# sdecoder/AVX-sort-merge-joins

Measured on AMD Instinct MI355X. Metric: join throughput Mtuples/s (R⋈S) + achieved HBM GB/s, 128M⋈128M at 1/2/4/8 GPU, higher is better.
Workload: dtype int64; 1 GPU; sortmergejoin_multiway R=128000000 S=128000000 per GPU, 16-byte tuples, uniform, PK/FK keys 1..|R|, row-id payloads (48-bit intermediates); tuples_per_relation_per_gpu=128000000, tuples_per_relation_total=128000000, tuple_bytes=16, payload=rowid, distribution=uniform, parallelism=range-partition x1

## Files before the change

### avx-sort-merge-joins_amd/csrc/capi.hip

```cpp
#include <atomic>
#include <math.h>
#include <string.h>
#include <sys/time.h>

#include <algorithm>
#include <vector>

#include "../../include/smj.h"
#include "smj_common.hpp"
#include "smj_internal.hpp"

__global__ void k_setplan(smj::RangePlan* p, smj::RangePlan v) { *p = v; }

__global__ void __launch_bounds__(256)
k_join_begin(smj::RangePlan* p, smj::RangePlan v, int set_plan, unsigned long long* count,
             unsigned int* status, unsigned int* zero, uint32_t nzero) {
    if (threadIdx.x == 0) {
        if (set_plan) *p = v;
        *count = 0;
    }
    if (threadIdx.x < 4) status[threadIdx.x] = 0;
    for (uint32_t i = threadIdx.x; i < nzero; i += 256) zero[i] = 0;
}

// ... 1357 lines not shown
        (unsigned long long*)c.ws.scratch("api_cnt", sizeof(unsigned long long));
    const uint32_t T = joincfg->NTHREADS > 0 ? (uint32_t)joincfg->NTHREADS : 1;
    const uint32_t fan = joincfg->PARTFANOUT > 1 ? (uint32_t)joincfg->PARTFANOUT : 2;
    const uint32_t D = ceil_log2(fan);
    const uint32_t F = (1u << D) >= T ? (1u << D) : T;
    const uint32_t bits = ceil_log2(F);
    int64_t* hist = (int64_t*)c.ws.scratch("mp_hist", (size_t)T * F * 8);
    int64_t* off = (int64_t*)c.ws.scratch("mp_off", (size_t)T * F * 8);
    const DevBuf* rels[2] = {&r, &s};
    Tup* sorted[2] = {sR, sS};
    const uint64_t ns[2] = {nR, nS};
    static const char* pn[2] = {"mp_partR", "mp_partS"};
    std::vector<uint64_t> toff[2], tlen[2];
    for (int q = 0; q < 2; q++) {
        toff[q].assign(T, 0);
        tlen[q].assign(T, 0);
        if (ns[q] == 0) continue;
        Tup* part = (Tup*)c.ws.scratch(pn[q], ns[q] * sizeof(Tup));
        const uint64_t chunk = ns[q] / T;
        std::vector<uint64_t> c0(T), cl(T);
        for (uint32_t t = 0; t < T; t++) {
            c0[t] = t * chunk;
            cl[t] = t + 1 == T ? ns[q] - c0[t] : chunk;
            if (!cl[t]) continue;
            const uint64_t rchunk = t + 1 == T ? nR - (uint64_t)t * (nR / T) : nR / T;
            const int64_t sh = rchunk ? (int64_t)ceil(log2((double)(rchunk * T))) - (int64_t)bits - 1
                                      : 0;
            const uint32_t shift = sh > 0 ? (uint32_t)(sh < 63 ? sh : 63) : 0u;
            const uint32_t mask =
                shift < 32 ? (uint32_t)((((1ull << bits) - 1) << shift) & 0xffffffffull) : 0u;
            const Digit32 dig{mask, shift};
            stable_partition(&c.ws, rels[q]->d + c0[t], cl[t], part + c0[t], dig, bits, 0,
                             hist + (size_t)t * F, off + (size_t)t * F, c.st);
        }
        std::vector<int64_t> hh((size_t)T * F, 0), ho((size_t)T * F, 0);
        for (uint32_t t = 0; t < T; t++) {
            if (!cl[t]) continue;
            SMJ_CHECK(hipMemcpyAsync(hh.data() + (size_t)t * F, hist + (size_t)t * F, F * 8,
                                     hipMemcpyDeviceToHost, c.st));
            SMJ_CHECK(hipMemcpyAsync(ho.data() + (size_t)t * F, off + (size_t)t * F, F * 8,
                                     hipMemcpyDeviceToHost, c.st));
        }
        sync();
        std::vector<uint64_t> so((size_t)T * F), sl((size_t)T * F);
        for (uint32_t t = 0; t < T; t++)
            for (uint32_t j = 0; j < F; j++) {
                so[(size_t)t * F + j] = c0[t] + (uint64_t)ho[(size_t)t * F + j];
                sl[(size_t)t * F + j] = (uint64_t)hh[(size_t)t * F + j];
            }
        segmented_sort(&c.ws, part, so.data(), sl.data(), T * F, c.st);
        const uint32_t per = F / T;
        uint64_t o = 0;
        for (uint32_t t = 0; t < T; t++) {
            std::vector<const Tup*> runs;
            std::vector<uint64_t> lens;
            for (uint32_t j = t * per; j < (t + 1) * per; j++)
                for (uint32_t i = 0; i < T; i++) {
                    runs.push_back(part + so[(size_t)i * F + j]);
                    lens.push_back(sl[(size_t)i * F + j]);
                }
            uint64_t tot = 0;
            for (uint64_t x : lens) tot += x;
            toff[q][t] = o;
            tlen[q][t] = tot;
            if (tot) multiway_merge_tree(&c.ws, runs.data(), lens.data(), (uint32_t)runs.size(),
                                         sorted[q] + o, c.st);
            o += tot;
        }
    }
    unsigned long long* tcnt =
        (unsigned long long*)c.ws.scratch("mp_cnt", (size_t)T * sizeof(unsigned long long));
    SMJ_CHECK(hipMemsetAsync(tcnt, 0, (size_t)T * 8, c.st));
    for (uint32_t t = 0; t < T; t++)
        merge_join_count(sR + toff[0][t], tlen[0][t], sS + toff[1][t], tlen[1][t], tcnt + t,
                         c.st);
    std::vector<unsigned long long> h(T, 0);
    SMJ_CHECK(hipMemcpyAsync(h.data(), tcnt, (size_t)T * 8, hipMemcpyDeviceToHost, c.st));
    sync();
    (void)cnt;
    gettimeofday(&t1, NULL);
    result_t* res = (result_t*)malloc(sizeof(result_t));
    res->totalresults = 0;
    res->nthreads = joincfg->NTHREADS;
    res->resultlist = (threadresult_t*)calloc(T, sizeof(threadresult_t));
    for (uint32_t t = 0; t < T; t++) {
        res->totalresults += (int64_t)h[t];
        res->resultlist[t].nresults = (int64_t)h[t];
        res->resultlist[t].threadid = t;
        if (mat < 0 ? materialize_on() : mat > 0) {
            chainedtuplebuffer_t* cb = chainedtuplebuffer_init();
            materialize_append(sR + toff[0][t], tlen[0][t], sS + toff[1][t], tlen[1][t], cb);
            res->resultlist[t].results = cb;
        }
    }
    if (!getenv("SMJ_QUIET")) {
        double us = (t1.tv_sec - t0.tv_sec) * 1e6 + (t1.tv_usec - t0.tv_usec);
        fprintf(stderr, "NUM-TUPLES = %lld TOTAL-TIME-USECS = %.4lf ", (long long)nS, us);
        fprintf(stderr, "TUPLES-PER-SECOND = %.4lf ", nS / (us / 1e6));
        fflush(stderr);
    }
    return res;
}

result_t* sortmergejoin_multipass(relation_t* relR, relation_t* relS,
                                  joinconfig_t* joincfg) {
    return multipass_api(relR, relS, joincfg, -1);
}

result_t* smj_join(relation_t* relR, relation_t* relS, joinconfig_t* joincfg, int algo,
                   int materialize) {
    const int mat = materialize < 0 ? -1 : (materialize ? 1 : 0);
    switch (algo) {
        case 0: return join_api(relR, relS, joincfg, "m-way", mat);
        case 1: return multipass_api(relR, relS, joincfg, mat);
        case 2: return mpsm_api(relR, relS, joincfg, mat);
        default:
            fprintf(stderr, "[ERROR] smj_join: unknown algorithm %d\n", algo);
            return 0;
    }
}

int smj_tuple_bytes(void) { return (int)sizeof(Tup); }

const char* smj_device_name(void) {
    static char name[256] = {0};
    if (!name[0]) {
        Ctx& c = ctx();
        hipDeviceProp_t p;
        SMJ_CHECK(hipGetDeviceProperties(&p, c.device));
        snprintf(name, sizeof(name), "%s (%s)", p.name, p.gcnArchName);
    }
    return name;
}

smj_workspace* smj_workspace_create(void) {
    ctx();
    return (smj_workspace*)new Workspace();
}
void smj_workspace_destroy(smj_workspace* ws) { delete (Workspace*)ws; }

void smj_workspace_set_layouts(smj_workspace* ws, uint32_t off) {
    ((Workspace*)(ws ? ws : smj_context_workspace()))->layouts_off = off;
}

int smj_workspace_last_layout(smj_workspace* ws) {
    return ((Workspace*)(ws ? ws : smj_context_workspace()))->last_layout;
}

int smj_tilepass_occupancy(int layout, uint32_t d2_bits) {
    if (layout != SMJ_LAYOUT_USED_P48 && layout != SMJ_LAYOUT_USED_P32) return -1;
    return tilepass_occupancy(layout == SMJ_LAYOUT_USED_P32, d2_bits);
}

void smj_dev_partition(smj_workspace* ws, const tuple_t* in, uint64_t n,
                       tuple_t* out, uint32_t nbits, uint32_t shiftbits,
                       int padded, int64_t* hist_out, int64_t* off_out,
                       smj_stream_t stream) {
    const uint32_t mask = (uint32_t)(((1ull << nbits) - 1) << shiftbits);
    Digit32 dig{mask, shiftbits};
    stable_partition((Workspace*)ws, (const Tup*)in, n, (Tup*)out, dig, nbits,
                     padded, hist_out, off_out, (hipStream_t)stream);
}

void smj_dev_sort(smj_workspace* ws, const tuple_t* in, uint64_t n,
                  tuple_t* out, smj_stream_t stream) {
    device_sort((Workspace*)ws, (const Tup*)in, n, (Tup*)out,
                (hipStream_t)stream);
}

void smj_dev_merge2(const tuple_t* a, uint64_t na, const tuple_t* b,
                    uint64_t nb, tuple_t* out, smj_stream_t stream) {
    merge2(&ctx().ws, (const Tup*)a, na, (const Tup*)b, nb, (Tup*)out, (hipStream_t)stream);
}

void smj_dev_multiway_merge_host(smj_workspace* ws, const tuple_t* const* runs,
                                 const uint64_t* lens, uint32_t k,
                                 tuple_t* out, smj_stream_t stream) {
    multiway_merge((Workspace*)ws, (const Tup* const*)runs, lens, k, (Tup*)out,
                   (hipStream_t)stream);
}

void smj_dev_merge_join_count(const tuple_t* r, uint64_t nr, const tuple_t* s,
                              uint64_t ns, unsigned long long* count_dev,
                              smj_stream_t stream) {
    merge_join_count((const Tup*)r, nr, (const Tup*)s, ns, count_dev,
                     (hipStream_t)stream);
}

uint64_t smj_dev_materialize(smj_workspace* ws, const tuple_t* sortedR, uint64_t nR,
                             const tuple_t* sortedS, uint64_t nS, tuple_t* out,
                             uint64_t out_cap, smj_stream_t stream) {
    return materialize((Workspace*)ws, (const Tup*)sortedR, nR, (const Tup*)sortedS,
                       nS, (Tup*)out, out_cap, (hipStream_t)stream);
}

uint64_t smj_dev_join_pairs(smj_workspace* ws, const tuple_t* sortedR, uint64_t nR,
                            const tuple_t* sortedS, uint64_t nS, value_t* r_payload_out,
                            value_t* s_payload_out, intkey_t* key_out, uint64_t out_cap,
                            smj_stream_t stream) {
    return join_pairs((Workspace*)ws, (const Tup*)sortedR, nR, (const Tup*)sortedS, nS,
                      r_payload_out, s_payload_out, key_out, out_cap, (hipStream_t)stream);
}

uint64_t smj_dev_semi_join(smj_workspace* ws, const tuple_t* sortedR, uint64_t nR,
                           const tuple_t* sortedS, uint64_t nS, tuple_t* out,
                           uint64_t out_cap, int anti, smj_stream_t stream) {
    return semi_join((Workspace*)ws, (const Tup*)sortedR, nR, (const Tup*)sortedS, nS,
                     (Tup*)out, out_cap, anti, (hipStream_t)stream);
}

uint64_t smj_dev_band_join(smj_workspace* ws, const tuple_t* sortedR, uint64_t nR,
                           const tuple_t* sortedS, uint64_t nS, int64_t lo, int64_t hi,
                           value_t* r_payload_out, value_t* s_payload_out,
                           intkey_t* r_key_out, intkey_t* s_key_out, uint64_t out_cap,
                           smj_stream_t stream) {
    return band_join((Workspace*)ws, (const Tup*)sortedR, nR, (const Tup*)sortedS, nS, lo, hi,
                     r_payload_out, s_payload_out, r_key_out, s_key_out, out_cap,
                     (hipStream_t)stream);
}

void smj_dev_band_join_count(smj_workspace* ws, const tuple_t* sortedR, uint64_t nR,
                             const tuple_t* sortedS, uint64_t nS, int64_t lo, int64_t hi,
                             unsigned long long* count_dev, smj_stream_t stream) {
    band_join_count((Workspace*)ws, (const Tup*)sortedR, nR, (const Tup*)sortedS, nS, lo, hi,
                    count_dev, (hipStream_t)stream);
}

void smj_dev_join(smj_workspace* ws, const tuple_t* R, uint64_t nR,
                  const tuple_t* S, uint64_t nS, tuple_t* sortedR,
                  tuple_t* sortedS, uint32_t fanout_bits, int64_t key_min,
                  int64_t key_max, unsigned long long* count_dev,
                  smj_stream_t stream) {
    device_join((Workspace*)ws, (const Tup*)R, nR, (const Tup*)S, nS,
                (Tup*)sortedR, (Tup*)sortedS, fanout_bits, key_min, key_max,
                count_dev, (hipStream_t)stream);
}

__global__ void __launch_bounds__(256)
k_seg_tables(const int64_t* __restrict__ cnt, uint32_t nseg, uint32_t nb,
             uint64_t* __restrict__ seg_start, int64_t* __restrict__ seg_cnt,
             int64_t* __restrict__ bcount, uint64_t* __restrict__ bstart) {
    __shared__ uint32_t scr[5];
    __shared__ unsigned long long base;
    if (threadIdx.x == 0) base = 0;
    for (uint32_t b = threadIdx.x; b < nb; b += 256) {
        bcount[b] = 0;
        bstart[b] = 0;
    }
    __syncthreads();
    for (uint32_t s = 0; s < nseg; s++) {
        for (uint32_t b0 = 0; b0 < nb; b0 += 256) {
            const uint32_t b = b0 + threadIdx.x;
            const int64_t c = b < nb ? cnt[(size_t)s * nb + b] : 0;
            uint32_t tot;
            const uint32_t ex = block_exclusive_scan((uint32_t)c, scr, &tot);
            if (b < nb) {
                seg_start[(size_t)b * nseg + s] = base + ex;
                seg_cnt[(size_t)b * nseg + s] = c;
                bcount[b] += c;
            }
            __syncthreads();
            if (threadIdx.x == 0) base += tot;
            __syncthreads();
        }
    }
}

__global__ void __launch_bounds__(256)
k_seg_totals(const int64_t* __restrict__ cnt0, const int64_t* __restrict__ cnt1,
             uint32_t nseg, uint32_t nb, int64_t* __restrict__ bcount0,
             int64_t* __restrict__ bcount1, uint64_t* __restrict__ bstart0,
             uint64_t* __restrict__ bstart1) {
    const int64_t* cnt = blockIdx.x ? cnt1 : cnt0;
    int64_t* bcount = blockIdx.x ? bcount1 : bcount0;
    uint64_t* bstart = blockIdx.x ? bstart1 : bstart0;
    for (uint32_t b = threadIdx.x; b < nb; b += 256) {
        int64_t t = 0;
        for (uint32_t j = 0; j < nseg; j++) t += cnt[(size_t)b * nseg + j];
        bcount[b] = t;
        bstart[b] = 0;
    }
}

static void join_segmented_core(Workspace* ws, void* R, uint64_t nR, void* S, uint64_t nS,
                                uint64_t* const* ss, int64_t* const* sc, uint32_t nseg,
                                uint32_t bucket_bits, int64_t key_lo, int64_t key_hi,
                                uint32_t flags, tuple_t* sortedR, tuple_t* sortedS,
                                unsigned long long* count_dev, hipStream_t st,
                                const uint64_t* pstride = nullptr) {
    if (!(flags & SMJ_SEG_STAGE_R))
        SMJ_CHECK(hipMemsetAsync(count_dev, 0, sizeof(unsigned long long), st));
    uint32_t D1, D2, D2cap;
    choose_levels(nR > nS ? nR : nS, bucket_bits, &D1, &D2, &D2cap);
    const uint32_t tot_bits = D1 + D2;
    D1 = bucket_bits;
    D2 = tot_bits > D1 ? tot_bits - D1 : 0;
    if (D2 > kMaxD2) D2 = kMaxD2;
    D2cap = D2 + 2 < kMaxD2 ? D2 + 2 : (D2 > kMaxD2 ? D2 : kMaxD2);
    RangePlan hplan = make_plan(key_lo, key_hi, D1, D2, D2cap, kGroupD3Max);
    const bool p48 = pstride != nullptr;
    const bool packed = (flags & SMJ_SEG_PACKED) != 0 || p48;
    if (p48 && !LayP48::usable(hplan)) {
        fprintf(stderr, "[ERROR] smj_dev_join_segmented_planes: 48-bit words need "
                "1 <= s1 <= 32 (s1 = %u)\n", hplan.s1);
        abort();
    }
// ... 417 lines not shown
```

### avx-sort-merge-joins_amd/csrc/partition.hip

```cpp
#include <stdlib.h>
#include <string.h>

#include "smj_common.hpp"
#include "smj_internal.hpp"

namespace smj {

template <int THREADS, int ITEMS, class Digit>
__global__ void __launch_bounds__(THREADS)
k_hist(const Tup* __restrict__ in, uint64_t n, uint64_t chunk, Digit dig_arg,
       uint32_t nbins, uint32_t* __restrict__ counts, uint32_t nwg) {
    const auto dig = dig_arg.load();
    constexpr int TILE = THREADS * ITEMS;
    extern __shared__ __attribute__((aligned(16))) uint32_t lds_hist[];
    for (uint32_t d = threadIdx.x; d < nbins; d += THREADS) lds_hist[d] = 0;
    __syncthreads();
    const uint64_t beg = (uint64_t)blockIdx.x * chunk;
    uint64_t end = beg + chunk;
    if (end > n) end = n;
    for (uint64_t base = beg; base < end; base += TILE) {
        Tup v[ITEMS];
#pragma unroll
        for (int j = 0; j < ITEMS; j++) {
            const uint64_t i = base + (uint64_t)j * THREADS + threadIdx.x;
// ... 997 lines not shown
        if (sh_hist[d]) atomicAdd(&hist[d], sh_hist[d]);
}


#ifndef SMJ_SC_SEG
#define SMJ_SC_SEG 16
#endif
constexpr uint32_t kSegBytes = SMJ_SC_SEG;
constexpr uint32_t kRegionAlign = 128;
static_assert(kRegionAlign % kSegBytes == 0, "regions hold whole segments");

struct RegionRel {
    const unsigned int* sample[2];
    uint64_t* base[2];
    uint64_t* seg_start[2];
    unsigned long long* cursor[2];
    uint64_t* cap_end[2];
    int64_t* hist_out[2];
    int64_t* seg_cnt[2];
};

__global__ void __launch_bounds__(256)
k_regions(RegionRel R, uint32_t nbins, uint32_t stride, uint64_t slack, uint32_t elem_bytes) {
    const int r = blockIdx.x;
    const unsigned int* __restrict__ sample = R.sample[r];
    uint64_t* __restrict__ base = R.base[r];
    uint64_t* __restrict__ seg_start = R.seg_start[r];
    unsigned long long* __restrict__ cursor = R.cursor[r];
    uint64_t* __restrict__ cap_end = R.cap_end[r];
    __shared__ uint64_t sh[256];
    const uint64_t ALIGN = kRegionAlign / elem_bytes;
    const uint32_t per = (nbins + 255) / 256;
    const uint32_t b = threadIdx.x * per;
    auto cap = [&](uint32_t d) {
        const uint64_t est = (uint64_t)sample[d] * stride / kShards;
        return (est + est / 8 + slack + ALIGN - 1) / ALIGN * ALIGN;
    };
    uint64_t loc = 0;
    for (uint32_t k = 0; k < per; k++)
        if (b + k < nbins) loc += kShards * cap(b + k);
    sh[threadIdx.x] = loc;
    __syncthreads();
    if (threadIdx.x == 0) {
        uint64_t run = 0;
        for (int t = 0; t < 256; t++) {
            const uint64_t x = sh[t];
            sh[t] = run;
            run += x;
        }
    }
    __syncthreads();
    uint64_t ex = sh[threadIdx.x];
    for (uint32_t k = 0; k < per; k++) {
        const uint32_t d = b + k;
        if (d < nbins) {
            base[d] = ex;
            const uint64_t c = cap(d);
            for (uint32_t q = 0; q < kShards; q++) {
                seg_start[d * kShards + q] = ex;
                cursor[d * kShards + q] = ex;
                ex += c;
                cap_end[d * kShards + q] = ex;
            }
        }
    }
}

__global__ void __launch_bounds__(256)
k_regions_done(RegionRel R, uint32_t nbins, unsigned int* __restrict__ flag) {
    const int r = blockIdx.x;
    const uint64_t* __restrict__ seg_start = R.seg_start[r];
    const unsigned long long* __restrict__ cursor = R.cursor[r];
    const uint64_t* __restrict__ cap_end = R.cap_end[r];
    for (uint32_t d = threadIdx.x; d < nbins; d += 256) {
        int64_t tot = 0;
        for (uint32_t q = 0; q < kShards; q++) {
            const uint32_t i = d * kShards + q;
            const uint64_t e = cursor[i] < cap_end[i] ? cursor[i] : cap_end[i];
            const int64_t c = (int64_t)(e - seg_start[i]);
            R.seg_cnt[r][i] = c;
            tot += c;
            if (cursor[i] > cap_end[i]) atomicOr(flag, 1u);
        }
        R.hist_out[r][d] = tot;
    }
}

template <int THREADS, int ITEMS, class Digit>
__global__ void __launch_bounds__(THREADS)
k_shard_hist(const Tup* __restrict__ in, uint64_t n, uint64_t chunk, uint32_t split,
             Digit dig_arg, uint32_t nbins, unsigned int* __restrict__ counts) {
    const auto dig = dig_arg.load();
    extern __shared__ unsigned int lh[];
    for (uint32_t d = threadIdx.x; d < nbins; d += THREADS) lh[d] = 0;
    __syncthreads();
    const uint32_t c = blockIdx.x / split, s = blockIdx.x % split;
    const uint64_t sub = (chunk + split - 1) / split;
    const uint64_t beg = (uint64_t)c * chunk + (uint64_t)s * sub;
    const uint64_t end = min(min(beg + sub, (uint64_t)(c + 1) * chunk), n);
    constexpr int TILE = THREADS * ITEMS;
    for (uint64_t base = beg; base < end; base += TILE) {
        Tup v[ITEMS];
#pragma unroll
        for (int j = 0; j < ITEMS; j++) {
            const uint64_t i = base + (uint64_t)j * THREADS + threadIdx.x;
            v[j] = ld_stream(in + (i < end ? i : end - 1));
        }
#pragma unroll
        for (int j = 0; j < ITEMS; j++)
            if (base + (uint64_t)j * THREADS + threadIdx.x < end) atomicAdd(&lh[dig(v[j])], 1u);
    }
    __syncthreads();
    const uint32_t q = c % kShards;
    for (uint32_t d = threadIdx.x; d < nbins; d += THREADS)
        if (lh[d]) atomicAdd(&counts[(size_t)d * kShards + q], lh[d]);
}

__global__ void __launch_bounds__(1024)
k_regions_exact(RegionRel R, uint32_t nbins) {
    const int r = blockIdx.x;
    const unsigned int* __restrict__ cnt = R.sample[r];
    __shared__ uint32_t scr[1024 / 64 + 1];
    const uint32_t per = (nbins + 1023) / 1024;
    const uint32_t b = threadIdx.x * per;
    uint32_t loc = 0;
    for (uint32_t k = 0; k < per; k++)
        if (b + k < nbins)
            for (uint32_t q = 0; q < kShards; q++) loc += cnt[(size_t)(b + k) * kShards + q];
    uint32_t tot;
    uint64_t e = block_exclusive_scan(loc, scr, &tot);
    for (uint32_t k = 0; k < per; k++) {
        const uint32_t d = b + k;
        if (d >= nbins) break;
        R.base[r][d] = e;
        for (uint32_t q = 0; q < kShards; q++) {
            const size_t i = (size_t)d * kShards + q;
            R.seg_start[r][i] = e;
            R.cursor[r][i] = e;
            e += cnt[i];
            R.cap_end[r][i] = e;
        }
    }
}

template <int THREADS, int ITEMS, class OutT, uint32_t SB = sizeof(OutT)>
struct ScatterGeom {
    static constexpr uint32_t SEG = kSegBytes >= SB ? kSegBytes / SB : 1;
    static constexpr uint32_t TILE = THREADS * ITEMS;
    static __host__ __device__ constexpr uint32_t max_segs(uint32_t nbins) {
        return (TILE + nbins * (SEG - 1)) / SEG;
    }
    static __host__ __device__ constexpr size_t lds_bytes(uint32_t nbins) {
        return (size_t)TILE * sizeof(OutT) + (size_t)nbins * SEG * sizeof(OutT) +
               (size_t)nbins * (8 + 4 * 4) + ((size_t)max_segs(nbins) * 2 + 15) / 16 * 16 +
               (THREADS / 64 + 1) * 4;
    }
};

template <class P, class = void>
struct requires_quads : std::false_type {};
template <class P>
struct requires_quads<P, std::void_t<decltype(P::kQuads)>> : std::true_type {};
template <class Pack>
constexpr bool pack_quads() {
    if constexpr (requires_quads<Pack>::value) return Pack::kQuads;
    else return false;
}

template <int THREADS, int ITEMS, class Digit, class Pack, bool VEC>
__global__ void __launch_bounds__(THREADS)
k_scatter_res(const Tup* __restrict__ in, uint64_t n, uint64_t chunk, Digit dig_arg,
              uint32_t nbins, unsigned long long* __restrict__ cursor_all,
              const uint64_t* __restrict__ cap_end_all,
              void* __restrict__ out, uint64_t ostride, Pack pk,
              unsigned int* __restrict__ bad_flag) {
    typedef typename Pack::OutT OutT;
    typedef ScatterGeom<THREADS, ITEMS, OutT, Pack::kStoreBytes> Geo;
    constexpr uint32_t SEG = Geo::SEG;
    constexpr int TILE = (int)Geo::TILE;
    uint32_t bad = 0;
    const auto dig = dig_arg.load();
    const uint32_t shard = blockIdx.x % kShards;
    unsigned long long* cursor = cursor_all + shard;
    const uint64_t* cap_end = cap_end_all + shard;
    extern __shared__ __attribute__((aligned(16))) unsigned char lds_raw[];
    OutT* stage = reinterpret_cast<OutT*>(lds_raw);
    OutT* carry = stage + TILE;
    uint64_t* pos = reinterpret_cast<uint64_t*>(carry + (size_t)nbins * SEG);
    uint32_t* tstart = reinterpret_cast<uint32_t*>(pos + nbins);
    uint32_t* tfill = tstart + nbins;
    uint32_t* kc = tfill + nbins;
    uint32_t* segpre = kc + nbins;
    uint16_t* segown = reinterpret_cast<uint16_t*>(segpre + nbins);
    uint32_t* scr = reinterpret_cast<uint32_t*>(
        reinterpret_cast<unsigned char*>(segown) + ((size_t)Geo::max_segs(nbins) * 2 + 15) / 16 * 16);

    for (uint32_t d = threadIdx.x; d < nbins; d += THREADS) {
        tfill[d] = 0;
        kc[d] = 0;
    }
    const uint64_t beg = (uint64_t)blockIdx.x * chunk;
    uint64_t end = beg + chunk;
    if (end > n) end = n;
    const uint32_t d0 = threadIdx.x;
    const bool own = d0 < nbins;
    const uint64_t my_cap = own ? cap_end[(size_t)d0 * kShards] : 0;
    uint32_t my_kc = 0;

    static_assert(!VEC || (sizeof(Tup) == 8 && ITEMS % 2 == 0), "VEC: 8-byte tuples, ITEMS even");
    auto item_pos = [](int j) -> uint32_t {
        return VEC ? 2u * ((uint32_t)(j / 2) * THREADS + threadIdx.x) + (uint32_t)(j & 1)
                   : (uint32_t)j * THREADS + threadIdx.x;
    };
    auto load_tile = [&](Tup (&x)[ITEMS], uint64_t b0) {
#ifndef KEY_8B
        typedef unsigned long long V2 __attribute__((ext_vector_type(2)));
        if constexpr (VEC) {
            const V2* __restrict__ vin = reinterpret_cast<const V2*>(in);
            const uint64_t vl = end / 2 - 1;
#pragma unroll
            for (int p = 0; p < ITEMS / 2; p++) {
                const uint64_t vi = b0 / 2 + (uint64_t)p * THREADS + threadIdx.x;
#if SMJ_NT_LOADS
                const V2 y = __builtin_nontemporal_load(vin + (vi < vl ? vi : vl));
#else
                const V2 y = vin[vi < vl ? vi : vl];
#endif
                x[2 * p] = (Tup)y.x;
                x[2 * p + 1] = (Tup)y.y;
            }
        } else
#endif
        {
#pragma unroll
            for (int j = 0; j < ITEMS; j++) {
                const uint64_t i = b0 + (uint64_t)j * THREADS + threadIdx.x;
                x[j] = ld_stream(in + (i < end ? i : end - 1));
            }
        }
    };
    Tup v[ITEMS], nv[ITEMS];
    if (beg < end) load_tile(v, beg);
    __syncthreads();
    for (uint64_t base = beg; base < end; base += TILE) {
        const uint32_t tcount =
            (uint32_t)((end - base) < (uint64_t)TILE ? (end - base) : TILE);
        const uint64_t nb = base + TILE;
        __builtin_amdgcn_s_waitcnt(0x0f70);
        uint32_t dg[ITEMS];
#pragma unroll
        for (int j = 0; j < ITEMS; j++) {
            const uint32_t li = item_pos(j);
            dg[j] = li < tcount ? dig(v[j]) : 0xffffffffu;
            if (dg[j] != 0xffffffffu) atomicAdd(&tfill[dg[j]], 1u);
        }
        __syncthreads();
        const uint32_t c = own ? tfill[d0] : 0;
        const uint32_t T = my_kc + c;
        uint32_t Eown = T / SEG * SEG;
        uint32_t tot;
        const uint32_t ex = block_exclusive_scan(own ? (c | ((Eown / SEG) << 16)) : 0u, scr, &tot);
        const uint32_t nseg = tot >> 16;
        unsigned long long Pown = 0;
        if (own) {
            tstart[d0] = ex & 0xffffu;
            tfill[d0] = ex & 0xffffu;
            segpre[d0] = ex >> 16;
            for (uint32_t k = 0; k < Eown / SEG; k++) segown[(ex >> 16) + k] = (uint16_t)d0;
            if (Eown) Pown = atomicAdd(&cursor[(size_t)d0 * kShards], (unsigned long long)Eown);
        }
        load_tile(nv, nb);
        __syncthreads();
#pragma unroll
        for (int j = 0; j < ITEMS; j++)
            if (dg[j] != 0xffffffffu) stage[atomicAdd(&tfill[dg[j]], 1u)] = pk(v[j], bad);
        if (own) {
            const bool ovf = Eown && Pown + Eown > my_cap;
            pos[d0] = ovf ? ~0ull : Pown;
            if (ovf) Eown = 0;
        }
        __syncthreads();
        if constexpr (pack_quads<Pack>() && SEG == 4) {
            for (uint32_t sg = threadIdx.x; sg < nseg; sg += THREADS) {
                const uint32_t d = segown[sg];
                const uint32_t e = (sg - segpre[d]) * SEG;
                const uint32_t k = kc[d];
                const uint64_t p = pos[d];
                OutT x[4];
#pragma unroll
                for (uint32_t i = 0; i < 4; i++)
                    x[i] = e + i < k ? carry[d * SEG + e + i] : stage[tstart[d] + e + i - k];
                if (p != ~0ull) {
                    if ((p & 3) == 0) {
                        Pack::store4(out, ostride, p + e, x);
                    } else {
#pragma unroll
                        for (uint32_t i = 0; i < 4; i++) Pack::store(out, ostride, p + e + i, x[i]);
                    }
                }
            }
        } else if constexpr (Pack::kPairs) {
            constexpr uint32_t PS = SEG / 2;
            for (uint32_t q = threadIdx.x; q < nseg * PS; q += THREADS) {
                const uint32_t sg = q / PS;
                const uint32_t d = segown[sg];
                const uint32_t e = (sg - segpre[d]) * SEG + 2 * (q % PS);
                const uint32_t k = kc[d];
                const uint64_t p = pos[d];
                const OutT x0 = e < k ? carry[d * SEG + e] : stage[tstart[d] + e - k];
                const OutT x1 = e + 1 < k ? carry[d * SEG + e + 1] : stage[tstart[d] + e + 1 - k];
                if (p != ~0ull) {
                    if ((p & 1) == 0) {
                        Pack::store2(out, ostride, p + e, x0, x1);
                    } else {
                        Pack::store(out, ostride, p + e, x0);
                        Pack::store(out, ostride, p + e + 1, x1);
                    }
                }
            }
        } else {
            for (uint32_t q = threadIdx.x; q < nseg * SEG; q += THREADS) {
                const uint32_t sg = q / SEG;
                const uint32_t d = segown[sg];
                const uint32_t e = (sg - segpre[d]) * SEG + q % SEG;
                const uint32_t k = kc[d];
                const uint64_t p = pos[d];
                const OutT x = e < k ? carry[d * SEG + e] : stage[tstart[d] + e - k];
                if (p != ~0ull) Pack::store(out, ostride, p + e, x);
            }
        }
        __syncthreads();
        if (own) {
            uint32_t left = T - Eown;
            if (left > SEG - 1) left = SEG - 1;
            for (uint32_t e = Eown; e < Eown + left; e++)
                carry[d0 * SEG + (e - Eown)] =
                    e < my_kc ? carry[d0 * SEG + e] : stage[tstart[d0] + e - my_kc];
            my_kc = left;
            kc[d0] = left;
            tfill[d0] = 0;
        }
#pragma unroll
        for (int j = 0; j < ITEMS; j++) v[j] = nv[j];
        __syncthreads();
    }
    if (own) {
        const uint32_t d = d0;
        pos[d] = 0;
        if (kc[d]) {
            const uint64_t p = atomicAdd(&cursor[(size_t)d * kShards], (unsigned long long)kc[d]);
            pos[d] = p + kc[d] <= my_cap ? p : ~0ull;
        }
    }
    __syncthreads();
    for (uint32_t q = threadIdx.x; q < nbins * SEG; q += THREADS) {
        const uint32_t d = q / SEG, j = q % SEG;
        if (j < kc[d] && pos[d] != ~0ull) Pack::store(out, ostride, pos[d] + j, carry[q]);
    }
    if (bad_flag && bad) atomicOr(bad_flag, bad);
}

template <class Digit>
__global__ void k_padcopy(const Tup* __restrict__ in, uint64_t n, Digit dig_arg,
                          const uint64_t* __restrict__ ustart,
                          const uint64_t* __restrict__ pstart,
                          Tup* __restrict__ out) {
    const auto dig = dig_arg.load();
    uint64_t i = (uint64_t)blockIdx.x * blockDim.x + threadIdx.x;
    const uint64_t stride = (uint64_t)gridDim.x * blockDim.x;
    for (; i < n; i += stride) {
        Tup t = in[i];
        uint32_t d = dig(t);
        out[pstart[d] + (i - ustart[d])] = t;
    }
}

template <class Digit>
__global__ void k_hist_global(const Tup* __restrict__ in, uint64_t n, Digit dig_arg,
                              unsigned long long* __restrict__ hist) {
    const auto dig = dig_arg.load();
    uint64_t i = (uint64_t)blockIdx.x * blockDim.x + threadIdx.x;
    const uint64_t stride = (uint64_t)gridDim.x * blockDim.x;
    for (; i < n; i += stride) atomicAdd(&hist[dig(in[i])], 1ull);
}

struct LowBits {
    Digit32 inner;
    uint32_t lowbits;
    __device__ __forceinline__ LowBits load() const { return *this; }
    __device__ __forceinline__ uint32_t operator()(const Tup& t) const {
        return inner(t) & ((1u << lowbits) - 1u);
    }
};
struct HighBits {
    Digit32 inner;
    uint32_t lowbits;
    __device__ __forceinline__ HighBits load() const { return *this; }
    __device__ __forceinline__ uint32_t operator()(const Tup& t) const {
        return inner(t) >> lowbits;
    }
};

template <int THREADS, int ITEMS, bool STABLE, class Digit, class Pack = PackNone>
static void partition_hist_scatter(Workspace* ws, const Tup* in, uint64_t n,
                                   typename Pack::OutT* out, const Digit& dig, uint32_t dbits,
                                   int padded, uint64_t* starts_dev,
                                   int64_t* hist_out, int64_t* off_out,
                                   hipStream_t st, const Pack& pk = Pack(),
                                   unsigned int* bad_flag = nullptr) {
    constexpr int TILE = THREADS * ITEMS;
    const uint32_t nbins = 1u << dbits;
    uint64_t ntiles = (n + TILE - 1) / TILE;
    if (ntiles == 0) ntiles = 1;
    const uint32_t maxwg = 256 * 8;
    uint32_t nwg = (uint32_t)(ntiles < maxwg ? ntiles : maxwg);
    const uint64_t tiles_per_wg = (ntiles + nwg - 1) / nwg;
    const uint64_t chunk = tiles_per_wg * TILE;
    nwg = (uint32_t)((ntiles + tiles_per_wg - 1) / tiles_per_wg);

    uint32_t* counts = (uint32_t*)ws->scratch("pt_counts", (size_t)nbins * nwg * 4);
    uint64_t* totals = (uint64_t*)ws->scratch("pt_totals", (size_t)nbins * 8);
    {
        TraceScope ts(ws, "k_hist", st);
        hipLaunchKernelGGL((k_hist<THREADS, ITEMS, Digit>), dim3(nwg), dim3(THREADS),
                           nbins * sizeof(uint32_t), st, in, n, chunk, dig, nbins,
                           counts, nwg);
    }
    {
        TraceScope ts(ws, "k_scan", st);
        hipLaunchKernelGGL(k_scanrow, dim3(nbins), dim3(256), 0, st, counts, nwg,
                           totals);
        hipLaunchKernelGGL(k_scandig, dim3(1), dim3(256), 0, st, totals, nbins,
                           padded, starts_dev, hist_out, off_out);
    }
    if (n == 0) return;
    if constexpr (!STABLE) {
        const size_t ldsu = scatter_u_lds<THREADS, ITEMS>(nbins);
        set_lds_attr((const void*)k_scatter_u<THREADS, ITEMS, Digit, Pack>, 160 * 1024);
        if (ldsu > 160 * 1024) {
            fprintf(stderr, "[ERROR] smj: scatter LDS %zu > 160 KiB\n", ldsu);
            abort();
        }
        TraceScope ts(ws, "k_scatter", st);
        hipLaunchKernelGGL((k_scatter_u<THREADS, ITEMS, Digit, Pack>), dim3(nwg),
                           dim3(THREADS), ldsu, st, in, n, chunk, dig, nbins,
                           counts, nwg, starts_dev, out, pk, bad_flag);
        SMJ_CHECK(hipGetLastError());
        return;
    } else {
        typedef SwcGeom<512, 8> SG;
        if (nbins <= 4 * 512 && SG::lds_bytes(nbins) <= 160 * 1024) {
            set_lds_attr((const void*)k_scatter_swc<512, 8, Digit>, 160 * 1024);
            TraceScope ts(ws, "k_scatter", st);
            hipLaunchKernelGGL((k_scatter_swc<512, 8, Digit>), dim3(nwg), dim3(512),
                               SG::lds_bytes(nbins), st, in, n, chunk, dig, nbins, dbits,
                               counts, nwg, starts_dev, out);
            SMJ_CHECK(hipGetLastError());
            return;
        }
        const size_t lds = scatter_lds<THREADS, ITEMS>(nbins);
        set_lds_attr((const void*)k_scatter<THREADS, ITEMS, Digit>, 160 * 1024);
        if (lds > 160 * 1024) {
            fprintf(stderr, "[ERROR] smj: scatter LDS %zu > 160 KiB\n", lds);
            abort();
        }
        {
            TraceScope ts(ws, "k_scatter", st);
            hipLaunchKernelGGL((k_scatter<THREADS, ITEMS, Digit>), dim3(nwg),
                               dim3(THREADS), lds, st, in, n, chunk, dig, nbins, dbits,
                               counts, nwg, starts_dev, out);
        }
    }
    SMJ_CHECK(hipGetLastError());
}

static bool lds_order_ok(Workspace* ws, hipStream_t st) {
    static const bool ok = [&] {
        const uint64_t bad = lds_order_selfcheck(ws, st);
        if (bad)
            fprintf(stderr, "[WARN] smj: LDS atomics return %llu values out of lane order: "
                            "the stable partition uses ballot ranks\n",
                    (unsigned long long)bad);
        return bad == 0;
    }();
    return ok;
}

template <class Digit>
static void stable_partition_swp(Workspace* ws, const Tup* in, uint64_t n, Tup* out,
                                 const Digit& dig, uint32_t dbits, int padded,
                                 uint64_t* starts_dev, int64_t* hist_out, int64_t* off_out,
                                 hipStream_t st) {
    constexpr int THREADS = 512;
    constexpr int ITEMS = sizeof(Tup) == 16 ? 8 : 16;
    typedef SwaGeom<THREADS, ITEMS> G;
    const uint32_t nbins = 1u << dbits;
    uint64_t ntiles = (n + G::TILE - 1) / G::TILE;
    if (ntiles == 0) ntiles = 1;
    uint32_t nwg = (uint32_t)(ntiles < 256 ? ntiles : 256);
    const uint64_t tiles_per_wg = (ntiles + nwg - 1) / nwg;
    const uint64_t chunk = tiles_per_wg * G::TILE;
    nwg = (uint32_t)((ntiles + tiles_per_wg - 1) / tiles_per_wg);
    uint32_t* counts = (uint32_t*)ws->scratch("pt_counts", (size_t)nbins * nwg * 4);
    uint64_t* totals = (uint64_t*)ws->scratch("pt_totals", (size_t)nbins * 8);
    {
        TraceScope ts(ws, "k_hist", st);
        bool vec = false;
        if constexpr (sizeof(Tup) == 8) {
            vec = ((uintptr_t)in & 15) == 0 && (chunk & 1) == 0;
            if (vec)
                hipLaunchKernelGGL((k_hist_v<512, 8, Digit>), dim3(nwg), dim3(512),
                                   nbins * sizeof(uint32_t), st, in, n, chunk, dig, nbins,
                                   counts, nwg);
// ... 46 lines not shown
                               hipStream_t st) {
    if (dbits <= 10)
        partition_hist_scatter<512, 16, false>(ws, in, n, out, dig, dbits, 0, starts_dev,
                                               hist_out, nullptr, st);
    else
        partition_hist_scatter<256, 8, false>(ws, in, n, out, dig, dbits, 0, starts_dev,
                                              hist_out, nullptr, st);
}

void stable_partition(Workspace* ws, const Tup* in, uint64_t n, Tup* out,
                      const Digit32& dig, uint32_t dbits, int padded,
                      int64_t* hist_out, int64_t* off_out, hipStream_t st) {
    const uint32_t nbins = 1u << dbits;
    if (dbits <= kNarrowDigitBits) {
        uint64_t* starts = (uint64_t*)ws->scratch("pt_starts", (size_t)nbins * 8);
        stable_partition_narrow(ws, in, n, out, dig, dbits, padded, starts,
                                hist_out, off_out, st);
        return;
    }
    const uint32_t lowb = dbits / 2, highb = dbits - lowb;
    Tup* t1 = (Tup*)ws->scratch("pt_wide1", (n ? n : 1) * sizeof(Tup));
    Tup* t2 = (Tup*)ws->scratch("pt_wide2", (n ? n : 1) * sizeof(Tup));
    uint64_t* st1 = (uint64_t*)ws->scratch("pt_wst1", (1u << lowb) * 8);
    uint64_t* st2 = (uint64_t*)ws->scratch("pt_wst2", (1u << highb) * 8);
    LowBits lo{dig, lowb};
    HighBits hi{dig, lowb};
    stable_partition_narrow(ws, in, n, t1, lo, lowb, 0, st1, nullptr, nullptr, st);
    stable_partition_narrow(ws, t1, n, t2, hi, highb, 0, st2, nullptr, nullptr, st);
    unsigned long long* h = (unsigned long long*)ws->scratch("pt_whist", (size_t)nbins * 8);
    SMJ_CHECK(hipMemsetAsync(h, 0, (size_t)nbins * 8, st));
    if (n) hipLaunchKernelGGL(k_hist_global<Digit32>, dim3(1024), dim3(256), 0,
                              st, in, n, dig, h);
    uint64_t* ust = (uint64_t*)ws->scratch("pt_wust", (size_t)nbins * 8);
    uint64_t* pst = (uint64_t*)ws->scratch("pt_wpst", (size_t)nbins * 8);
    hipLaunchKernelGGL(k_scandig, dim3(1), dim3(256), 0, st,
                       (const uint64_t*)h, nbins, 0, ust, nullptr, nullptr);
    hipLaunchKernelGGL(k_scandig, dim3(1), dim3(256), 0, st,
                       (const uint64_t*)h, nbins, padded, pst, hist_out, off_out);
    if (n) hipLaunchKernelGGL(k_padcopy<Digit32>, dim3(2048), dim3(256), 0, st,
                              t2, n, dig, ust, pst, out);
    SMJ_CHECK(hipGetLastError());
}

void plan_partition(Workspace* ws, const Tup* in, uint64_t n, Tup* out,
                    const RangePlan* plan_dev, uint32_t dbits,
                    uint64_t* starts_dev, int64_t* hist_out, hipStream_t st) {
    PlanDigit1 dig{plan_dev};
    const uint32_t nbins = 1u << dbits;
    constexpr int THREADS = 512;
    constexpr int ITEMS = sizeof(Tup) == 16 ? 8 : 16;
    constexpr int TILE = THREADS * ITEMS;
    const size_t lds = scatter_wc_lds<THREADS, ITEMS>(nbins);
    if (sizeof(Tup) != 16 || dbits > 10 || lds > 160 * 1024) {
        unstable_partition(ws, in, n, out, dig, dbits, starts_dev, hist_out, st);
        return;
    }
    uint64_t ntiles = (n + TILE - 1) / TILE;
    if (ntiles == 0) ntiles = 1;
    const uint32_t maxwg = 256;
    uint32_t nwg = (uint32_t)(ntiles < maxwg ? ntiles : maxwg);
    const uint64_t tiles_per_wg = (ntiles + nwg - 1) / nwg;
    const uint64_t chunk = tiles_per_wg * TILE;
    nwg = (uint32_t)((ntiles + tiles_per_wg - 1) / tiles_per_wg);
    uint32_t* counts = (uint32_t*)ws->scratch("pt_counts", (size_t)nbins * nwg * 4);
    uint64_t* totals = (uint64_t*)ws->scratch("pt_totals", (size_t)nbins * 8);
    {
        TraceScope ts(ws, "k_hist", st);
        hipLaunchKernelGGL((k_hist<1024, 8, PlanDigit1>), dim3(nwg), dim3(1024),
                           nbins * sizeof(uint32_t), st, in, n, chunk, dig, nbins,
                           counts, nwg);
    }
    {
        TraceScope ts(ws, "k_scan", st);
        hipLaunchKernelGGL(k_scanrow, dim3(nbins), dim3(256), 0, st, counts, nwg,
                           totals);
        hipLaunchKernelGGL(k_scandig, dim3(1), dim3(256), 0, st, totals, nbins, 0,
                           starts_dev, hist_out, (int64_t*)nullptr);
    }
    if (n == 0) return;
    set_lds_attr((const void*)k_scatter_wc<THREADS, ITEMS, PlanDigit1>, 160 * 1024);
    TraceScope ts(ws, "k_scatter", st);
    hipLaunchKernelGGL((k_scatter_wc<THREADS, ITEMS, PlanDigit1>), dim3(nwg),
                       dim3(THREADS), lds, st, in, n, chunk, dig, nbins, counts,
                       nwg, starts_dev, out);
    SMJ_CHECK(hipGetLastError());
}

#ifdef KEY_8B
void plan_partition_packed(Workspace* ws, const Tup* in, uint64_t n, uint64_t* out,
                           const RangePlan* plan_dev, const RangePlan& pack_plan,
                           uint32_t dbits, uint64_t* starts_dev, int64_t* hist_out,
                           unsigned int* pack_bad, hipStream_t st) {
    PlanDigit1 dig{plan_dev};
    LayPacked::Pack pk;
    pk.bu = key_u(pack_plan.base);
    pk.span = pack_plan.span;
    pk.s1 = pack_plan.s1;
    if (dbits > 10)
        partition_hist_scatter<256, 8, false, PlanDigit1, LayPacked::Pack>(
            ws, in, n, out, dig, dbits, 0, starts_dev, hist_out, nullptr, st, pk, pack_bad);
    else
        partition_hist_scatter<512, 16, false, PlanDigit1, LayPacked::Pack>(
            ws, in, n, out, dig, dbits, 0, starts_dev, hist_out, nullptr, st, pk, pack_bad);
}
#endif

#ifndef SMJ_SC_THREADS
#define SMJ_SC_THREADS 1024
#endif
#ifndef SMJ_SC_ITEMS16
#define SMJ_SC_ITEMS16 4
#endif
#ifndef SMJ_SC_ITEMS16Q
#define SMJ_SC_ITEMS16Q 6
#endif
#ifndef SMJ_SC_ITEMS16P
#define SMJ_SC_ITEMS16P 8
#endif
#ifndef SMJ_SC_ITEMS8
#define SMJ_SC_ITEMS8 12
#endif
#ifndef SMJ_SC_ITEMS8W
#define SMJ_SC_ITEMS8W 16
#endif
#ifndef SMJ_SC_WG_PER_CU
#define SMJ_SC_WG_PER_CU 1
#endif
#ifndef SMJ_SAMPLE_STRIDE
#define SMJ_SAMPLE_STRIDE 128
#endif
static constexpr uint32_t kSampleStride = SMJ_SAMPLE_STRIDE;
#ifndef SMJ_SAMPLE_WG
#define SMJ_SAMPLE_WG 128
#endif
static constexpr uint32_t kSampleWg = SMJ_SAMPLE_WG;
static constexpr uint64_t kRegionSlack = 1024;

uint64_t sampled_capacity(uint64_t n, uint32_t dbits) {
    const uint64_t ALIGN = kRegionAlign / 4;
    return n + n / 8 + 5 * kSampleStride + 1 +
           ((uint64_t)1 << dbits) * kShards * (kRegionSlack + ALIGN);
}

static uint64_t scatter_chunk(uint64_t n, uint64_t tile, uint32_t* nwg_out) {
    const uint64_t ntiles = (n + tile - 1) / tile;
    const uint32_t maxwg = 256 * SMJ_SC_WG_PER_CU;
    uint32_t nwg = (uint32_t)(ntiles < maxwg ? ntiles : maxwg);
    const uint64_t tiles_per_wg = (ntiles + nwg - 1) / nwg;
    *nwg_out = (uint32_t)((ntiles + tiles_per_wg - 1) / tiles_per_wg);
    return tiles_per_wg * tile;
}

template <class Pack>
static int sampled_items(uint32_t nbins) {
    constexpr int THREADS = SMJ_SC_THREADS;
    constexpr int BIG = sizeof(Tup) == 16
        ? (sizeof(typename Pack::OutT) <= 8    ? SMJ_SC_ITEMS16P
           : sizeof(typename Pack::OutT) <= 12 ? SMJ_SC_ITEMS16Q
                                               : SMJ_SC_ITEMS16)
        : (sizeof(typename Pack::OutT) <= 4 ? SMJ_SC_ITEMS8W : SMJ_SC_ITEMS8);
    constexpr int SMALL = sizeof(Tup) == 16 ? 4 : 8;
    typedef typename Pack::OutT O;
    if (ScatterGeom<THREADS, BIG, O, Pack::kStoreBytes>::lds_bytes(nbins) <= 160 * 1024) return BIG;
    if (ScatterGeom<THREADS, SMALL, O, Pack::kStoreBytes>::lds_bytes(nbins) <= 160 * 1024)
        return SMALL;
    return 0;
}

template <int ITEMS, class Pack>
static bool sampled_scatter_t(Workspace* ws, const Tup* in, uint64_t n, void* out,
                              uint64_t ostride, const PlanDigit1& dig, uint32_t nbins,
                              unsigned long long* cursor, const uint64_t* cap_end,
                              const Pack& pk, unsigned int* bad_flag, hipStream_t st) {
    constexpr int THREADS = SMJ_SC_THREADS;
    constexpr int TILE = THREADS * ITEMS;
    const size_t lds = ScatterGeom<THREADS, ITEMS, typename Pack::OutT,
                                   Pack::kStoreBytes>::lds_bytes(nbins);
    if (lds > 160 * 1024) return false;
    uint32_t nwg = 0;
    const uint64_t chunk = scatter_chunk(n, TILE, &nwg);
    constexpr bool VEC_OK = sizeof(Tup) == 8 && ITEMS % 2 == 0;
    set_lds_attr((const void*)k_scatter_res<THREADS, ITEMS, PlanDigit1, Pack, false>, 160 * 1024);
    if constexpr (VEC_OK)
        set_lds_attr((const void*)k_scatter_res<THREADS, ITEMS, PlanDigit1, Pack, true>,
                     160 * 1024);
    TraceScope ts(ws, "k_scatter", st);
    bool vec = false;
    if constexpr (VEC_OK) {
        vec = n % 2 == 0 && chunk % 2 == 0 && ((uintptr_t)in & 15) == 0;
        if (vec)
            hipLaunchKernelGGL((k_scatter_res<THREADS, ITEMS, PlanDigit1, Pack, true>), dim3(nwg),
                               dim3(THREADS), lds, st, in, n, chunk, dig, nbins, cursor,
                               cap_end, out, ostride, pk, bad_flag);
    }
    if (!vec)
        hipLaunchKernelGGL((k_scatter_res<THREADS, ITEMS, PlanDigit1, Pack, false>), dim3(nwg),
                           dim3(THREADS), lds, st, in, n, chunk, dig, nbins, cursor,
                           cap_end, out, ostride, pk, bad_flag);
    return true;
}

template <class Pack>
static void sampled_scatter(Workspace* ws, const Tup* in, uint64_t n, void* out,
                            uint64_t ostride, const PlanDigit1& dig, uint32_t nbins,
                            unsigned long long* cursor, const uint64_t* cap_end,
                            const Pack& pk, unsigned int* bad_flag, hipStream_t st) {
    constexpr int THREADS = SMJ_SC_THREADS;
    if (nbins > (uint32_t)THREADS) {
        fprintf(stderr, "[ERROR] smj: sampled scatter needs <= %d partitions\n", THREADS);
        abort();
    }
    constexpr int BIG = sizeof(Tup) == 16
        ? (sizeof(typename Pack::OutT) <= 8    ? SMJ_SC_ITEMS16P
           : sizeof(typename Pack::OutT) <= 12 ? SMJ_SC_ITEMS16Q
                                               : SMJ_SC_ITEMS16)
        : (sizeof(typename Pack::OutT) <= 4 ? SMJ_SC_ITEMS8W : SMJ_SC_ITEMS8);
    constexpr int SMALL = sizeof(Tup) == 16 ? 4 : 8;
    const int items = sampled_items<Pack>(nbins);
    if (items == BIG && sampled_scatter_t<BIG>(ws, in, n, out, ostride, dig, nbins, cursor,
                                               cap_end, pk, bad_flag, st))
        return;
    if (items == SMALL && sampled_scatter_t<SMALL>(ws, in, n, out, ostride, dig, nbins,
                                                   cursor, cap_end, pk, bad_flag, st))
        return;
    fprintf(stderr, "[ERROR] smj: sampled scatter LDS exceeds 160 KiB (%u partitions)\n", nbins);
    abort();
}

void sampled_partition(Workspace* ws, int nrel, const Tup* const* in, const uint64_t* n,
                       void* const* out, const RangePlan* plan_dev, uint32_t dbits,
                       unsigned int* sample, uint64_t* const* starts_dev,
                       int64_t* const* hist_out, uint64_t* const* seg_start,
                       int64_t* const* seg_cnt, unsigned int* flag_dev, hipStream_t st,
                       const RangePlan* host_plan, bool packed, unsigned int* bad,
                       uint64_t p48_stride, bool p32, bool exact, bool p96) {
    PlanDigit1 dig{plan_dev};
    const uint32_t nbins = 1u << dbits;
    if (p96 && (sizeof(Tup) != 16 || !host_plan || !p48_stride || p32 || exact)) {
        fprintf(stderr, "[ERROR] smj: the 96-bit layout needs 16-byte tuples, the host plan "
                        "and a plane stride\n");
        abort();
    }
    if (exact && (p48_stride || p32)) {
        fprintf(stderr, "[ERROR] smj: exact shard regions take tuples or 64-bit words\n");
        abort();
    }
#ifndef KEY_8B
    packed = p48_stride != 0 || p32;
#endif
    if (p32 && (p48_stride || !packed)) {
        fprintf(stderr, "[ERROR] smj: the 32-bit layout is a packed one-plane layout\n");
        abort();
    }
    if (p48_stride && !packed) {
        fprintf(stderr, "[ERROR] smj: the 48-bit layout is a packed layout\n");
        abort();
    }
    if (packed && !host_plan) {
        fprintf(stderr, "[ERROR] smj: packed partition needs the host plan\n");
        abort();
    }
    static const char* cn[2] = {"sp_cursor0", "sp_cursor1"};
    static const char* en[2] = {"sp_capend0", "sp_capend1"};
    SampleRel S;
    RegionRel R;
    uint64_t nmax = 0;
    for (int r = 0; r < 2; r++) {
        const int rr = r < nrel ? r : 0;
        S.in[r] = in[rr];
        S.n[r] = n[rr];
        S.hist[r] = sample + (size_t)rr * nbins * (exact ? kShards : 1);
        R.sample[r] = S.hist[r];
        R.base[r] = starts_dev[rr];
        R.seg_start[r] = seg_start[rr];
        R.hist_out[r] = hist_out[rr];
        R.seg_cnt[r] = seg_cnt[rr];
        if (r < nrel) {
            R.cursor[r] = (unsigned long long*)ws->scratch(cn[r], (size_t)nbins * kShards * 8);
            R.cap_end[r] = (uint64_t*)ws->scratch(en[r], (size_t)nbins * kShards * 8);
            nmax = n[r] > nmax ? n[r] : nmax;
        } else {
            R.cursor[r] = R.cursor[0];
            R.cap_end[r] = R.cap_end[0];
        }
    }
    if (exact) {
        TraceScope ts(ws, "k_hist", st);
        for (int r = 0; r < nrel; r++) {
            if (!n[r]) continue;
            int items = 0;
#ifdef KEY_8B
            if (packed)
                items = sampled_items<LayPacked::Pack>(nbins);
            else
#endif
                items = sampled_items<PackRange>(nbins);
            if (!items) {
                fprintf(stderr, "[ERROR] smj: sampled scatter LDS exceeds 160 KiB (%u "
                        "partitions)\n", nbins);
                abort();
            }
            uint32_t nwg = 0;
            const uint64_t chunk = scatter_chunk(n[r], (uint64_t)SMJ_SC_THREADS * items, &nwg);
            constexpr int HI = sizeof(Tup) == 16 ? 8 : 16;
            const uint32_t split = 4;
            hipLaunchKernelGGL((k_shard_hist<1024, HI, PlanDigit1>), dim3(nwg * split),
                               dim3(1024), nbins * sizeof(unsigned int), st, in[r], n[r], chunk,
                               split, dig, nbins, S.hist[r]);
        }
        hipLaunchKernelGGL(k_regions_exact, dim3(nrel), dim3(1024), 0, st, R, nbins);
    } else {
        TraceScope ts(ws, "k_sample", st);
        const uint64_t npts = (nmax + 4 * kSampleStride - 1) / (4 * kSampleStride);
        uint32_t g = (uint32_t)((npts + 255) / 256);
        if (g > kSampleWg) g = kSampleWg;
        if (g == 0) g = 1;
        hipLaunchKernelGGL((k_sample_hist<PlanDigit1>), dim3(g, nrel), dim3(256),
                           nbins * sizeof(unsigned int), st, S, kSampleStride, dig, nbins);
        hipLaunchKernelGGL(k_regions, dim3(nrel), dim3(256), 0, st, R, nbins, kSampleStride,
                           kRegionSlack,
                           p96 ? (uint32_t)SMJ_P96_SEGB : p48_stride || p32 ? 4u : packed ? 8u
                                                                     : (uint32_t)sizeof(Tup));
    }
    for (int r = 0; r < nrel; r++) {
        if (!n[r]) continue;
        if (p32) {
            LayP32::Pack pk;
            pk.bu = key_u(host_plan->base);
            pk.span = host_plan->span;
            pk.s1 = host_plan->s1;
            sampled_scatter(ws, in[r], n[r], out[r], 0, dig, nbins, R.cursor[r], R.cap_end[r],
                            pk, bad, st);
            continue;
        }
#ifdef KEY_8B
        if (p96) {
            LayP96::Pack pk;
            pk.bu = key_u(host_plan->base);
            pk.span = host_plan->span;
            sampled_scatter(ws, in[r], n[r], out[r], p48_stride, dig, nbins, R.cursor[r],
                            R.cap_end[r], pk, bad, st);
            continue;
        }
#endif
        if (p48_stride) {
            LayP48::Pack pk;
            pk.bu = key_u(host_plan->base);
            pk.span = host_plan->span;
            pk.s1 = host_plan->s1;
            sampled_scatter(ws, in[r], n[r], out[r], p48_stride, dig, nbins, R.cursor[r],
                            R.cap_end[r], pk, bad, st);
            continue;
        }
#ifdef KEY_8B
        if (packed) {
            LayPacked::Pack pk;
            pk.bu = key_u(host_plan->base);
            pk.span = host_plan->span;
            pk.s1 = host_plan->s1;
            sampled_scatter(ws, in[r], n[r], out[r], 0, dig, nbins, R.cursor[r], R.cap_end[r],
                            pk, bad, st);
            continue;
        }
#endif
        PackRange pk{0ull, ~0ull};
        if (bad && host_plan) {
            pk.bu = key_u(host_plan->base);
            pk.span = host_plan->span;
        }
        sampled_scatter(ws, in[r], n[r], out[r], 0, dig, nbins, R.cursor[r], R.cap_end[r], pk,
                        bad && host_plan ? bad : (unsigned int*)nullptr, st);
    }
    hipLaunchKernelGGL(k_regions_done, dim3(nrel), dim3(256), 0, st, R, nbins, flag_dev);
    SMJ_CHECK(hipGetLastError());
}

__global__ void __launch_bounds__(1024)
k_lds_order(uint32_t K, uint32_t iters, unsigned long long* bad) {
    __shared__ uint32_t ctr[16][64];
// ... 63 lines not shown
```

### avx-sort-merge-joins_amd/csrc/smj_common.hpp

```cpp
#pragma once
#include <hip/hip_runtime.h>
#include <stdint.h>
#include <stdio.h>
#include <stdlib.h>

#define SMJ_CHECK(call)                                                        \
    do {                                                                       \
        hipError_t e_ = (call);                                                \
        if (e_ != hipSuccess) {                                                \
            fprintf(stderr, "[ERROR] smj: %s failed at %s:%d: %s\n", #call,    \
                    __FILE__, __LINE__, hipGetErrorString(e_));                \
            abort();                                                           \
        }                                                                      \
    } while (0)

#include <mutex>
#include <set>
#include <utility>

namespace smj {

inline void set_lds_attr(const void* kernel, int bytes) {
    static std::mutex mu;
    static std::set<std::pair<int, const void*>> done;
// ... 13 lines not shown
typedef uint64_t Tup;
#endif

constexpr int kTupBytes = sizeof(Tup);

#ifndef SMJ_NT_STORES
#define SMJ_NT_STORES 1
#endif
#ifndef SMJ_NT_LOADS
#define SMJ_NT_LOADS 0
#endif
#ifdef KEY_8B
typedef long long TupVec __attribute__((ext_vector_type(2)));
#endif
__device__ __forceinline__ void st_stream(Tup* p, const Tup& v) {
#if SMJ_NT_STORES
#ifdef KEY_8B
    TupVec x = {v.payload, v.key};
    __builtin_nontemporal_store(x, reinterpret_cast<TupVec*>(p));
#else
    __builtin_nontemporal_store(v, p);
#endif
#else
    *p = v;
#endif
}
__device__ __forceinline__ Tup ld_stream(const Tup* p) {
#if SMJ_NT_LOADS
#ifdef KEY_8B
    const TupVec x = __builtin_nontemporal_load(reinterpret_cast<const TupVec*>(p));
    Tup t;
    t.payload = x.x;
    t.key = x.y;
    return t;
#else
    return __builtin_nontemporal_load(p);
#endif
#else
    return *p;
#endif
}

__device__ __forceinline__ void st_w(uint64_t* p, uint64_t v) {
#if SMJ_NT_STORES
    __builtin_nontemporal_store(v, p);
#else
    *p = v;
#endif
}
#ifdef KEY_8B
__device__ __forceinline__ void st_w(Tup* p, const Tup& v) { st_stream(p, v); }
#endif

__device__ __forceinline__ Tup ld_nt(const Tup* p) {
#ifdef KEY_8B
    const TupVec x = __builtin_nontemporal_load(reinterpret_cast<const TupVec*>(p));
    Tup t;
    t.payload = x.x;
    t.key = x.y;
    return t;
#else
    return __builtin_nontemporal_load(p);
#endif
}

typedef const __attribute__((address_space(1))) uint64_t* GlobalU64Ptr;
__device__ __forceinline__ Tup ld_g(const Tup* p) {
#ifdef KEY_8B
    typedef const __attribute__((address_space(1))) TupVec* GV;
    const TupVec x = *(GV)p;
    Tup t;
    t.payload = x.x;
    t.key = x.y;
    return t;
#else
    return *(GlobalU64Ptr)p;
#endif
}

__device__ __forceinline__ void st_g(Tup* p, const Tup& v) {
#ifdef KEY_8B
    typedef __attribute__((address_space(1))) TupVec* GV;
    TupVec x = {v.payload, v.key};
    *(GV)p = x;
#else
    *(__attribute__((address_space(1))) uint64_t*)p = v;
#endif
}

__host__ __device__ __forceinline__ int64_t tup_key(const Tup& t) {
#ifdef KEY_8B
    return t.key;
#else
    return (int64_t)(int32_t)(uint32_t)(t >> 32);
#endif
}

__host__ __device__ __forceinline__ bool tup_less(const Tup& a, const Tup& b) {
#ifdef KEY_8B
    return (a.key < b.key) || (a.key == b.key && a.payload < b.payload);
#else
    return (int64_t)a < (int64_t)b;
#endif
}

__host__ __device__ __forceinline__ Tup tup_sel(bool c, const Tup& a, const Tup& b) {
#ifdef KEY_8B
    Tup r;
    r.payload = c ? a.payload : b.payload;
    r.key = c ? a.key : b.key;
    return r;
#else
    return c ? a : b;
#endif
}

__host__ __device__ __forceinline__ bool tup_eq(const Tup& a, const Tup& b) {
#ifdef KEY_8B
    return a.key == b.key && a.payload == b.payload;
#else
    return a == b;
#endif
}

__host__ __device__ __forceinline__ Tup tup_max_sentinel() {
#ifdef KEY_8B
    Tup t;
    t.payload = INT64_MAX;
    t.key = INT64_MAX;
    return t;
#else
    return (uint64_t)INT64_MAX;
#endif
}

__host__ __device__ __forceinline__ uint64_t key_u(int64_t k) {
    return (uint64_t)k ^ 0x8000000000000000ull;
}

struct RefDigit {
    uint32_t mask;
    uint32_t shift;
    __host__ __device__ __forceinline__ RefDigit load() const { return *this; }
    __device__ __forceinline__ uint32_t operator()(const Tup& t) const {
        uint64_t km1 = (uint64_t)(tup_key(t) - 1);
        return (uint32_t)((km1 & (uint64_t)mask) >> shift);
    }
};

constexpr uint32_t kBadPayload = 1;
constexpr uint32_t kBadRange = 2;
constexpr uint32_t kBadPayload48 = 4;
constexpr uint32_t kBadPayload32 = 8;

struct RangePlan {
    int64_t base;
    uint64_t span;
    uint32_t D1, D2, D3;
    uint32_t s1, s2, s3;
};

__host__ __device__ __forceinline__ uint64_t plan_rel(const RangePlan& p,
                                                      int64_t k) {
    uint64_t ku = key_u(k), bu = key_u(p.base);
    if (ku < bu) return 0;
    uint64_t r = ku - bu;
    return r > p.span ? p.span : r;
}

__host__ __device__ __forceinline__ uint32_t plan_d1(const RangePlan& p,
                                                     uint64_t rel) {
    uint64_t d = rel >> p.s1;
    uint64_t lim = (1ull << p.D1) - 1;
    return (uint32_t)(d > lim ? lim : d);
}

struct LayTup {
    typedef Tup W;
    static constexpr bool packed = false;
    typedef const W* CView;
    typedef W* View;
    __device__ static __forceinline__ CView cview(const void* b, uint64_t) {
        return static_cast<const W*>(b);
    }
    __device__ static __forceinline__ View view(void* b, uint64_t) { return static_cast<W*>(b); }
    __device__ static __forceinline__ uint64_t rel(const RangePlan& P, const W& w, uint32_t) {
        return plan_rel(P, tup_key(w));
    }
    __device__ static __forceinline__ bool clamped(const RangePlan& P, const W& w) {
        const uint64_t ku = key_u(tup_key(w)), bu = key_u(P.base);
        return ku < bu || ku - bu > P.span;
    }
    __device__ static __forceinline__ bool less(const W& a, const W& b) { return tup_less(a, b); }
    __device__ static __forceinline__ Tup unpack(const RangePlan&, const W& w, uint32_t) {
        return w;
    }
    __device__ static __forceinline__ uint32_t digit_fast(const W& w, uint32_t base_lo,
                                                          uint32_t, uint32_t sh, uint32_t mask) {
        return (((uint32_t)tup_key(w) - base_lo) >> sh) & mask;
    }
    __host__ static bool fast_ok(const RangePlan& P, uint32_t sh, uint32_t width) {
        return sh + width <= 32;
    }
    struct FastDigit {
        uint32_t base_lo, sh, mask;
        __device__ FastDigit(const RangePlan& P, uint32_t s, uint32_t width)
            : base_lo((uint32_t)P.base), sh(s), mask((1u << width) - 1) {}
        __device__ __forceinline__ uint32_t operator()(const W& w) const {
            return (((uint32_t)tup_key(w) - base_lo) >> sh) & mask;
        }
    };
    struct Unpack {
        __device__ Unpack(const RangePlan&, uint32_t) {}
        __device__ __forceinline__ Tup operator()(const W& w) const { return w; }
    };
    __device__ static __forceinline__ uint64_t same_key_id(const W& w) {
#ifdef KEY_8B
        return (uint64_t)w.payload;
#else
        return w;
#endif
    }
};

#ifdef KEY_8B
struct LayPacked {
    typedef uint64_t W;
    static constexpr bool packed = true;
    typedef const W* CView;
    typedef W* View;
    __device__ static __forceinline__ CView cview(const void* b, uint64_t) {
        return static_cast<const W*>(b);
    }
    __device__ static __forceinline__ View view(void* b, uint64_t) { return static_cast<W*>(b); }
    __device__ static __forceinline__ uint64_t rel(const RangePlan& P, const W& w, uint32_t b) {
        return ((uint64_t)b << P.s1) | (w >> (64 - P.s1));
    }
    __device__ static __forceinline__ bool clamped(const RangePlan&, const W&) { return false; }
    __device__ static __forceinline__ bool less(const W& a, const W& b) { return a < b; }
    __device__ static __forceinline__ uint64_t same_key_id(const W& w) { return w; }
    __device__ static __forceinline__ uint32_t digit_fast(const W& w, uint32_t, uint32_t s1,
                                                          uint32_t sh, uint32_t mask) {
        return (uint32_t)(w >> (64 - s1 + sh)) & mask;
    }
    __host__ static bool fast_ok(const RangePlan& P, uint32_t sh, uint32_t width) {
        return sh + width <= P.s1;
    }
    __device__ static __forceinline__ Tup unpack(const RangePlan& P, const W& w, uint32_t b) {
        Tup t;
        t.payload = (int64_t)(w & (~0ull >> P.s1));
        t.key = (int64_t)((key_u(P.base) + rel(P, w, b)) ^ 0x8000000000000000ull);
        return t;
    }
    struct FastDigit {
        uint32_t tsh, mask;
        __device__ FastDigit(const RangePlan& P, uint32_t s, uint32_t width)
            : tsh(64 - P.s1 + s), mask((1u << width) - 1) {}
        __device__ __forceinline__ uint32_t operator()(const W& w) const {
            return (uint32_t)(w >> tsh) & mask;
        }
    };
    struct Unpack {
        uint64_t kbu, pmask;
        uint32_t sh;
        __device__ Unpack(const RangePlan& P, uint32_t b)
            : kbu(key_u(P.base) + ((uint64_t)b << P.s1)), pmask(~0ull >> P.s1), sh(64 - P.s1) {}
        __device__ __forceinline__ Tup operator()(const W& w) const {
            Tup t;
            t.payload = (int64_t)(w & pmask);
            t.key = (int64_t)((kbu + (w >> sh)) ^ 0x8000000000000000ull);
            return t;
        }
    };
    struct Pack {
        typedef uint64_t OutT;
        uint64_t bu, span;
        uint32_t s1;
        __device__ __forceinline__ uint64_t operator()(const Tup& t, uint32_t& bad) const {
            const uint64_t ku = key_u(t.key);
            const uint64_t r = ku - bu;
            const uint32_t pb = 64 - s1;
            bad |= (ku < bu || r > span) ? kBadRange : 0u;
            bad |= ((uint64_t)t.payload >> pb) != 0 ? kBadPayload : 0u;
            return ((r & ((1ull << s1) - 1)) << pb) | (uint64_t)t.payload;
        }
        static constexpr uint32_t kStoreBytes = 8;
        __device__ static __forceinline__ void store(void* out, uint64_t, uint64_t i,
                                                     uint64_t x) {
            static_cast<uint64_t*>(out)[i] = x;
        }
        static constexpr bool kPairs = false;
        template <class X>
        __device__ static __forceinline__ void store2(void*, uint64_t, uint64_t, const X&,
                                                      const X&) {}
    };
    __host__ static bool usable(const RangePlan& P) { return P.s1 >= 1 && P.s1 <= 32; }
};
#endif

#ifndef SMJ_P96_SEGB
#define SMJ_P96_SEGB 8
#endif
#ifdef KEY_8B
struct __attribute__((packed, aligned(4))) P96W {
    int64_t pay;
    uint32_t rel;
};
static_assert(sizeof(P96W) == 12, "12-byte element");
typedef const __attribute__((address_space(1))) int64_t* G64c;
typedef __attribute__((address_space(1))) int64_t* G64;
typedef const __attribute__((address_space(1))) uint32_t* G32c96;
typedef __attribute__((address_space(1))) uint32_t* G32w96;
struct P96CView {
    G64c pay;
    G32c96 rel;
    __device__ __forceinline__ P96W operator[](uint64_t i) const {
        P96W w;
        w.pay = pay[i];
        w.rel = rel[i];
        return w;
    }
    __device__ __forceinline__ P96CView operator+(uint64_t k) const {
        return P96CView{pay + k, rel + k};
    }
};
struct P96View {
    G64 pay;
    G32w96 rel;
    __device__ __forceinline__ P96View operator+(uint64_t k) const {
        return P96View{pay + k, rel + k};
    }
};
__device__ __forceinline__ void st_w(const P96View& p, const P96W& w) {
#if SMJ_NT_STORES
    __builtin_nontemporal_store(w.pay, (int64_t*)p.pay);
    __builtin_nontemporal_store(w.rel, (uint32_t*)p.rel);
#else
    p.pay[0] = w.pay;
    p.rel[0] = w.rel;
#endif
}

struct LayP96 {
    typedef P96W W;
    static constexpr bool packed = true;
    typedef P96CView CView;
    typedef P96View View;
    __device__ static __forceinline__ CView cview(const void* b, uint64_t stride) {
        const int64_t* pay = static_cast<const int64_t*>(b);
        return CView{(G64c)pay, (G32c96)(const uint32_t*)(pay + stride)};
    }
    __device__ static __forceinline__ View view(void* b, uint64_t stride) {
        int64_t* pay = static_cast<int64_t*>(b);
        return View{(G64)pay, (G32w96)(uint32_t*)(pay + stride)};
    }
    __device__ static __forceinline__ uint64_t rel(const RangePlan&, const W& w, uint32_t) {
        return w.rel;
    }
    __device__ static __forceinline__ bool clamped(const RangePlan&, const W&) { return false; }
    __device__ static __forceinline__ bool less(const W& a, const W& b) {
        return a.rel < b.rel || (a.rel == b.rel && a.pay < b.pay);
    }
    __device__ static __forceinline__ uint64_t same_key_id(const W& w) {
        return (uint64_t)w.pay;
    }
    __device__ static __forceinline__ uint32_t digit_fast(const W& w, uint32_t, uint32_t,
                                                          uint32_t sh, uint32_t mask) {
        return (w.rel >> sh) & mask;
    }
    __host__ static bool fast_ok(const RangePlan&, uint32_t sh, uint32_t width) {
        return sh + width <= 32;
    }
    __device__ static __forceinline__ Tup unpack(const RangePlan& P, const W& w, uint32_t) {
        Tup t;
        t.payload = w.pay;
        t.key = (int64_t)((key_u(P.base) + w.rel) ^ 0x8000000000000000ull);
        return t;
    }
    struct FastDigit {
        uint32_t sh, mask;
        __device__ FastDigit(const RangePlan&, uint32_t s, uint32_t width)
            : sh(s), mask((1u << width) - 1) {}
        __device__ __forceinline__ uint32_t operator()(const W& w) const {
            return (w.rel >> sh) & mask;
        }
    };
    struct Unpack {
        uint64_t kbu;
        __device__ Unpack(const RangePlan& P, uint32_t) : kbu(key_u(P.base)) {}
        __device__ __forceinline__ Tup operator()(const W& w) const {
            Tup t;
            t.payload = w.pay;
            t.key = (int64_t)((kbu + w.rel) ^ 0x8000000000000000ull);
            return t;
        }
    };
    struct Pack {
        typedef P96W OutT;
        uint64_t bu, span;
        __device__ __forceinline__ P96W operator()(const Tup& t, uint32_t& bad) const {
            const uint64_t ku = key_u(t.key);
            const uint64_t r = ku - bu;
            bad |= (ku < bu || r > span) ? kBadRange : 0u;
            P96W w;
            w.pay = t.payload;
            w.rel = (uint32_t)r;
            return w;
        }
        static constexpr uint32_t kStoreBytes = SMJ_P96_SEGB;
        __device__ static __forceinline__ void store(void* out, uint64_t stride, uint64_t i,
                                                     const P96W& x) {
            int64_t* pay = static_cast<int64_t*>(out);
            ((G64)pay)[i] = x.pay;
            ((G32w96)(uint32_t*)(pay + stride))[i] = x.rel;
        }
        static constexpr bool kPairs = true;
        __device__ static __forceinline__ void store2(void* out, uint64_t stride, uint64_t i,
                                                      const P96W& x0, const P96W& x1) {
            typedef long long L2 __attribute__((ext_vector_type(2)));
            typedef uint32_t U2 __attribute__((ext_vector_type(2)));
            int64_t* pay = static_cast<int64_t*>(out);
            L2 p = {x0.pay, x1.pay};
            U2 r = {x0.rel, x1.rel};
            *(__attribute__((address_space(1))) L2*)(pay + i) = p;
            *(__attribute__((address_space(1))) U2*)((uint32_t*)(pay + stride) + i) = r;
        }
    };
    __host__ static bool usable(const RangePlan& P) { return P.span < (1ull << 32); }
};
#endif

typedef const __attribute__((address_space(1))) uint32_t* G32c;
typedef const __attribute__((address_space(1))) uint16_t* G16c;
typedef __attribute__((address_space(1))) uint32_t* G32;
typedef __attribute__((address_space(1))) uint16_t* G16;

struct P48CView {
    G32c lo;
    G16c hi;
    __device__ __forceinline__ uint64_t operator[](uint64_t i) const {
        return (uint64_t)lo[i] | ((uint64_t)hi[i] << 32);
    }
    __device__ __forceinline__ P48CView operator+(uint64_t k) const {
        return P48CView{lo + k, hi + k};
    }
};

struct P48View {
    G32 lo;
    G16 hi;
    __device__ __forceinline__ uint64_t operator[](uint64_t i) const {
        return (uint64_t)lo[i] | ((uint64_t)hi[i] << 32);
    }
    __device__ __forceinline__ P48View operator+(uint64_t k) const {
        return P48View{lo + k, hi + k};
    }
};

__device__ __forceinline__ void st_w(const P48View& p, uint64_t v) {
#if SMJ_NT_STORES
    __builtin_nontemporal_store((uint32_t)v, p.lo);
    __builtin_nontemporal_store((uint16_t)(v >> 32), p.hi);
#else
    p.lo[0] = (uint32_t)v;
    p.hi[0] = (uint16_t)(v >> 32);
#endif
}

struct LayP48 {
    typedef uint64_t W;
    static constexpr bool packed = true;
    typedef P48CView CView;
    typedef P48View View;
    __device__ static __forceinline__ CView cview(const void* b, uint64_t stride) {
        const uint32_t* lo = static_cast<const uint32_t*>(b);
        return CView{(G32c)lo, (G16c)(const uint16_t*)(lo + stride)};
    }
    __device__ static __forceinline__ View view(void* b, uint64_t stride) {
        uint32_t* lo = static_cast<uint32_t*>(b);
        return View{(G32)lo, (G16)(uint16_t*)(lo + stride)};
    }
    __device__ static __forceinline__ uint64_t rel(const RangePlan& P, const W& w, uint32_t b) {
        return ((uint64_t)b << P.s1) | (w >> (48 - P.s1));
    }
    __device__ static __forceinline__ bool clamped(const RangePlan&, const W&) { return false; }
    __device__ static __forceinline__ bool less(const W& a, const W& b) { return a < b; }
    __device__ static __forceinline__ uint64_t same_key_id(const W& w) { return w; }
    __device__ static __forceinline__ uint32_t digit_fast(const W& w, uint32_t, uint32_t s1,
                                                          uint32_t sh, uint32_t mask) {
        return (uint32_t)(w >> (48 - s1 + sh)) & mask;
    }
    __host__ static bool fast_ok(const RangePlan& P, uint32_t sh, uint32_t width) {
        return sh + width <= P.s1;
    }
    __device__ static __forceinline__ Tup unpack(const RangePlan& P, const W& w, uint32_t b) {
        const uint64_t pay = w & (~0ull >> (16 + P.s1));
        const int64_t key = (int64_t)((key_u(P.base) + rel(P, w, b)) ^ 0x8000000000000000ull);
#ifdef KEY_8B
        Tup t;
        t.payload = (int64_t)pay;
        t.key = key;
        return t;
#else
        return ((uint64_t)(uint32_t)key << 32) | pay;
#endif
    }
    struct FastDigit {
        uint32_t tsh, mask;
        __device__ FastDigit(const RangePlan& P, uint32_t s, uint32_t width)
            : tsh(48 - P.s1 + s), mask((1u << width) - 1) {}
        __device__ __forceinline__ uint32_t operator()(const W& w) const {
            return (uint32_t)(w >> tsh) & mask;
        }
    };
    struct Unpack {
        uint64_t kbu, pmask;
        uint32_t sh;
        __device__ Unpack(const RangePlan& P, uint32_t b)
            : kbu(key_u(P.base) + ((uint64_t)b << P.s1)), pmask(~0ull >> (16 + P.s1)),
              sh(48 - P.s1) {}
        __device__ __forceinline__ Tup operator()(const W& w) const {
#ifdef KEY_8B
            Tup t;
            t.payload = (int64_t)(w & pmask);
            t.key = (int64_t)((kbu + (w >> sh)) ^ 0x8000000000000000ull);
            return t;
#else
            const uint32_t key = (uint32_t)kbu + (uint32_t)(w >> sh);
            return ((uint64_t)key << 32) | (uint32_t)(w & pmask);
#endif
        }
    };
    struct Pack {
        typedef uint64_t OutT;
        uint64_t bu, span;
        uint32_t s1;
        __device__ __forceinline__ uint64_t operator()(const Tup& t, uint32_t& bad) const {
            const uint64_t ku = key_u(tup_key(t));
            const uint64_t r = ku - bu;
            const uint32_t pb = 48 - s1;
#ifdef KEY_8B
            const uint64_t pay = (uint64_t)t.payload;
#else
            const uint64_t pay = (uint32_t)t;
#endif
            bad |= (ku < bu || r > span) ? kBadRange : 0u;
            bad |= (pay >> (64 - s1)) != 0 ? kBadPayload : 0u;
            bad |= (pay >> pb) != 0 ? kBadPayload48 : 0u;
            return ((r & ((1ull << s1) - 1)) << pb) | (pay & ((1ull << pb) - 1));
        }
        static constexpr uint32_t kStoreBytes = 4;
        __device__ static __forceinline__ void store(void* out, uint64_t stride, uint64_t i,
                                                     uint64_t x) {
            uint32_t* lo = static_cast<uint32_t*>(out);
            ((G32)lo)[i] = (uint32_t)x;
            ((G16)(uint16_t*)(lo + stride))[i] = (uint16_t)(x >> 32);
        }
        static constexpr bool kPairs = true;
        __device__ static __forceinline__ void store2(void* out, uint64_t stride, uint64_t i,
                                                      uint64_t x0, uint64_t x1) {
            typedef uint32_t U2 __attribute__((ext_vector_type(2)));
            typedef uint16_t H2 __attribute__((ext_vector_type(2)));
            uint32_t* lo = static_cast<uint32_t*>(out);
            const U2 l = {(uint32_t)x0, (uint32_t)x1};
            const H2 h = {(uint16_t)(x0 >> 32), (uint16_t)(x1 >> 32)};
            *(__attribute__((address_space(1))) U2*)(lo + i) = l;
            *(__attribute__((address_space(1))) H2*)((uint16_t*)(lo + stride) + i) = h;
        }
    };
    __host__ static bool usable(const RangePlan& P) { return P.s1 >= 1 && P.s1 <= 32; }
};

struct P32CView {
    G32c p;
    __device__ __forceinline__ uint32_t operator[](uint64_t i) const { return p[i]; }
    __device__ __forceinline__ P32CView operator+(uint64_t k) const { return P32CView{p + k}; }
};
struct P32View {
    G32 p;
    __device__ __forceinline__ uint32_t operator[](uint64_t i) const { return p[i]; }
    __device__ __forceinline__ P32View operator+(uint64_t k) const { return P32View{p + k}; }
};
__device__ __forceinline__ void st_w(const P32View& v, uint32_t x) {
#if SMJ_NT_STORES
    __builtin_nontemporal_store(x, v.p);
#else
    v.p[0] = x;
#endif
}

struct LayP32 {
    typedef uint32_t W;
    static constexpr bool packed = true;
    typedef P32CView CView;
    typedef P32View View;
    __device__ static __forceinline__ CView cview(const void* b, uint64_t) {
        return CView{(G32c) static_cast<const uint32_t*>(b)};
    }
    __device__ static __forceinline__ View view(void* b, uint64_t) {
        return View{(G32) static_cast<uint32_t*>(b)};
    }
    __device__ static __forceinline__ uint64_t rel(const RangePlan& P, const W& w, uint32_t b) {
        return ((uint64_t)b << P.s1) | (uint64_t)(w >> (32 - P.s1));
    }
    __device__ static __forceinline__ bool clamped(const RangePlan&, const W&) { return false; }
    __device__ static __forceinline__ bool less(const W& a, const W& b) { return a < b; }
    __device__ static __forceinline__ uint64_t same_key_id(const W& w) { return w; }
    __device__ static __forceinline__ uint32_t digit_fast(const W& w, uint32_t, uint32_t s1,
                                                          uint32_t sh, uint32_t mask) {
        return (w >> (32 - s1 + sh)) & mask;
    }
    __host__ static bool fast_ok(const RangePlan& P, uint32_t sh, uint32_t width) {
        return sh + width <= P.s1;
    }
    __device__ static __forceinline__ Tup unpack(const RangePlan& P, const W& w, uint32_t b) {
        const uint32_t pay = w & (0xffffffffu >> P.s1);
        const int64_t key = (int64_t)((key_u(P.base) + rel(P, w, b)) ^ 0x8000000000000000ull);
#ifdef KEY_8B
        Tup t;
        t.payload = (int64_t)pay;
        t.key = key;
        return t;
#else
        return ((uint64_t)(uint32_t)key << 32) | pay;
#endif
    }
    struct FastDigit {
        uint32_t tsh, mask;
        __device__ FastDigit(const RangePlan& P, uint32_t s, uint32_t width)
            : tsh(32 - P.s1 + s), mask((1u << width) - 1) {}
        __device__ __forceinline__ uint32_t operator()(const W& w) const {
            return (w >> tsh) & mask;
        }
    };
    struct Unpack {
        uint64_t kbu;
        uint32_t pmask, sh;
        __device__ Unpack(const RangePlan& P, uint32_t b)
            : kbu(key_u(P.base) + ((uint64_t)b << P.s1)), pmask(0xffffffffu >> P.s1),
              sh(32 - P.s1) {}
        __device__ __forceinline__ Tup operator()(const W& w) const {
#ifdef KEY_8B
            Tup t;
            t.payload = (int64_t)(w & pmask);
            t.key = (int64_t)((kbu + (w >> sh)) ^ 0x8000000000000000ull);
            return t;
#else
            const uint32_t key = (uint32_t)kbu + (w >> sh);
            return ((uint64_t)key << 32) | (w & pmask);
#endif
        }
    };
    struct Pack {
        typedef uint32_t OutT;
        uint64_t bu, span;
        uint32_t s1;
        __device__ __forceinline__ uint32_t operator()(const Tup& t, uint32_t& bad) const {
            const uint64_t ku = key_u(tup_key(t));
            const uint64_t r = ku - bu;
#ifdef KEY_8B
            const uint64_t pay = (uint64_t)t.payload;
#else
            const uint64_t pay = (uint32_t)t;
#endif
            bad |= (ku < bu || r > span) ? kBadRange : 0u;
            bad |= (pay >> (64 - s1)) != 0 ? kBadPayload : 0u;
            bad |= (pay >> (48 - s1)) != 0 ? kBadPayload48 : 0u;
            bad |= (pay >> (32 - s1)) != 0 ? kBadPayload32 : 0u;
            return ((uint32_t)r << (32 - s1)) | ((uint32_t)pay & (0xffffffffu >> s1));
        }
        static constexpr uint32_t kStoreBytes = 4;
        __device__ static __forceinline__ void store(void* out, uint64_t, uint64_t i, uint32_t x) {
#if SMJ_NT_STORES
            __builtin_nontemporal_store(x, (G32) static_cast<uint32_t*>(out) + i);
#else
            ((G32) static_cast<uint32_t*>(out))[i] = x;
#endif
        }
#ifndef SMJ_P32_QUADS
#define SMJ_P32_QUADS 1
#endif
        static constexpr bool kQuads = SMJ_P32_QUADS;
        __device__ static __forceinline__ void store4(void* out, uint64_t, uint64_t i,
                                                      const uint32_t (&x)[4]) {
            typedef uint32_t U4 __attribute__((ext_vector_type(4)));
            const U4 v = {x[0], x[1], x[2], x[3]};
            __attribute__((address_space(1))) U4* p =
                (__attribute__((address_space(1))) U4*)(static_cast<uint32_t*>(out) + i);
#if SMJ_NT_STORES
            __builtin_nontemporal_store(v, p);
#else
            *p = v;
#endif
        }
        static constexpr bool kPairs = true;
        __device__ static __forceinline__ void store2(void* out, uint64_t, uint64_t i, uint32_t x0,
                                                      uint32_t x1) {
            typedef uint32_t U2 __attribute__((ext_vector_type(2)));
            const U2 v = {x0, x1};
            __attribute__((address_space(1))) U2* p =
                (__attribute__((address_space(1))) U2*)(static_cast<uint32_t*>(out) + i);
#if SMJ_NT_STORES
            __builtin_nontemporal_store(v, p);
#else
            *p = v;
#endif
        }
    };
    __host__ static bool usable(const RangePlan& P) { return P.s1 >= 1 && P.s1 <= 31; }
};

typedef const __attribute__((address_space(1))) uint8_t* G8c;
typedef __attribute__((address_space(1))) uint8_t* G8;
struct P40CView {
    G32c lo;
    G8c hi;
    uint64_t gbits;
    __device__ __forceinline__ uint64_t operator[](uint64_t i) const {
        return (uint64_t)lo[i] | ((uint64_t)hi[i] << 32) | gbits;
    }
    __device__ __forceinline__ P40CView operator+(uint64_t k) const {
        return P40CView{lo + k, hi + k, gbits};
    }
};
struct P40View {
    G32 lo;
    G8 hi;
    __device__ __forceinline__ P40View operator+(uint64_t k) const { return P40View{lo + k, hi + k}; }
};
__device__ __forceinline__ void st_w(const P40View& p, uint64_t v) {
#if SMJ_NT_STORES
    __builtin_nontemporal_store((uint32_t)v, p.lo);
    __builtin_nontemporal_store((uint8_t)(v >> 32), p.hi);
#else
    p.lo[0] = (uint32_t)v;
    p.hi[0] = (uint8_t)(v >> 32);
#endif
}
struct LayP40 : LayP48 {
    typedef P40CView CView;
    typedef P40View View;
    __device__ static __forceinline__ CView cview(const void* b, uint64_t hoff) {
        return CView{(G32c) static_cast<const uint32_t*>(b),
                     (G8c)(static_cast<const uint8_t*>(b) + hoff), 0ull};
    }
    __device__ static __forceinline__ View view(void* b, uint64_t hoff) {
        return View{(G32) static_cast<uint32_t*>(b), (G8)(static_cast<uint8_t*>(b) + hoff)};
    }
    __host__ static bool holds(const RangePlan& P) { return P.D2 >= 8; }
};
template <class V>
__device__ __forceinline__ V with_group(const V& v, uint32_t, const RangePlan&) {
    return v;
}
__device__ __forceinline__ P40CView with_group(const P40CView& v, uint32_t g, const RangePlan& P) {
    return P40CView{v.lo, v.hi, (uint64_t)g << (48 - P.D2)};
}

struct PackNone {
    typedef Tup OutT;
    __device__ __forceinline__ Tup operator()(const Tup& t, uint32_t&) const { return t; }
    static constexpr uint32_t kStoreBytes = sizeof(Tup);
    __device__ static __forceinline__ void store(void* out, uint64_t, uint64_t i, const Tup& x) {
        static_cast<Tup*>(out)[i] = x;
    }
    static constexpr bool kPairs = false;
    template <class X>
    __device__ static __forceinline__ void store2(void*, uint64_t, uint64_t, const X&,
                              const X&) {}
};

struct PackRange {
    typedef Tup OutT;
    uint64_t bu, span;
    __device__ __forceinline__ Tup operator()(const Tup& t, uint32_t& bad) const {
        const uint64_t ku = key_u(tup_key(t));
        bad |= (ku < bu || ku - bu > span) ? kBadRange : 0u;
        return t;
    }
    static constexpr uint32_t kStoreBytes = sizeof(Tup);
    __device__ static __forceinline__ void store(void* out, uint64_t, uint64_t i, const Tup& x) {
        static_cast<Tup*>(out)[i] = x;
    }
    static constexpr bool kPairs = false;
    template <class X>
    __device__ static __forceinline__ void store2(void*, uint64_t, uint64_t, const X&,
                              const X&) {}
};

__host__ __device__ __forceinline__ uint32_t plan_d2(const RangePlan& p,
                                                     uint64_t rel,
                                                     uint32_t d1) {
    uint64_t v = rel >> p.s2;
    uint64_t lo = (uint64_t)d1 << p.D2;
    uint64_t lim = (1ull << p.D2) - 1;
    if (v < lo) return 0;
    v -= lo;
    return (uint32_t)(v > lim ? lim : v);
}

__host__ __device__ __forceinline__ uint32_t plan_d3(const RangePlan& p,
                                                     uint64_t rel,
                                                     uint32_t d12) {
    uint64_t v = rel >> p.s3;
    uint64_t lo = (uint64_t)d12 << p.D3;
    uint64_t lim = (1ull << p.D3) - 1;
    if (v < lo) return 0;
    v -= lo;
    return (uint32_t)(v > lim ? lim : v);
}

__host__ __device__ inline RangePlan make_plan(int64_t kmin, int64_t kmax,
                                               uint32_t D1, uint32_t D2,
                                               uint32_t D2cap, uint32_t D3max) {
    RangePlan p;
    p.base = kmin;
    uint64_t width = (kmax >= kmin) ? (key_u(kmax) - key_u(kmin)) : 0;
    uint32_t L = 0;
    while (L < 64 && (width >> L) != 0) L++;
    p.span = (L >= 64) ? ~0ull : ((1ull << L) - 1);
    p.D1 = D1;
    p.s1 = L > D1 ? L - D1 : 0;
    p.D2 = D2 < p.s1 ? D2 : p.s1;
    uint32_t s2 = p.s1 - p.D2;
    if (s2 > D3max && p.D2 < D2cap) {
        uint32_t extra = s2 - D3max;
        if (extra > D2cap - p.D2) extra = D2cap - p.D2;
        p.D2 += extra;
        s2 -= extra;
    }
    p.s2 = s2;
    p.D3 = s2 < D3max ? s2 : D3max;
    p.s3 = s2 - p.D3;
    return p;
}

__device__ __forceinline__ int lane_id() { return threadIdx.x & 63; }

__device__ __forceinline__ uint64_t lanemask_lt() {
    int l = lane_id();
    return l == 0 ? 0ull : (~0ull >> (64 - l));
}

template <typename T>
__device__ __forceinline__ T wave_sum(T v) {
#pragma unroll
    for (int o = 32; o > 0; o >>= 1) v += __shfl_xor(v, o, 64);
    return v;
}

__device__ __forceinline__ uint32_t block_exclusive_scan(uint32_t v,
                                                         uint32_t* scratch,
                                                         uint32_t* total) {
    const int lane = lane_id();
    const int wid = threadIdx.x >> 6;
    const int nw = blockDim.x >> 6;
    uint32_t x = v;
#pragma unroll
    for (int o = 1; o < 64; o <<= 1) {
        uint32_t y = __shfl_up(x, o, 64);
        if (lane >= o) x += y;
    }
    if (lane == 63) scratch[wid] = x;
    __syncthreads();
    if (threadIdx.x == 0) {
        uint32_t run = 0;
        for (int w = 0; w < nw; w++) {
            uint32_t t = scratch[w];
            scratch[w] = run;
            run += t;
        }
        scratch[nw] = run;
    }
    __syncthreads();
    uint32_t res = scratch[wid] + x - v;
    if (total) *total = scratch[nw];
    __syncthreads();
    return res;
}

__host__ __device__ __forceinline__ uint64_t align_tuples(uint64_t n) {
    const uint64_t tpl = 64 / sizeof(Tup);
    return (n + tpl - 1) & ~(tpl - 1);
}

}
```

### avx-sort-merge-joins_amd/csrc/smj_internal.hpp

```cpp
#pragma once
#include <sched.h>

#include <chrono>
#include <map>
#include <mutex>
#include <string>
#include <vector>

#include <hip/hip_ext.h>

#include "smj_common.hpp"

namespace smj {

constexpr uint32_t kNarrowDigitBits = 12;
constexpr uint32_t kMaxD2 = 10;

typedef RefDigit Digit32;

__device__ __forceinline__ uint32_t uniform32(uint32_t x) {
    return __builtin_amdgcn_readfirstlane(x);
}
__device__ __forceinline__ uint64_t uniform64(uint64_t x) {
    return ((uint64_t)__builtin_amdgcn_readfirstlane((uint32_t)(x >> 32)) << 32) |
// ... 142 lines not shown
    struct TraceRec {
        const char* name;
        hipEvent_t a, b;
    };
    bool trace_on = false;
    std::string trace_only;
    std::vector<TraceRec> trace;
    size_t trace_n = 0;
    bool traced(const char* name) const {
        return trace_on && (trace_only.empty() || trace_only == name);
    }
    int trace_begin(const char* name, hipStream_t st) {
        if (!traced(name)) return -1;
        if (trace_n == trace.size()) {
            TraceRec r;
            SMJ_CHECK(hipEventCreate(&r.a));
            SMJ_CHECK(hipEventCreate(&r.b));
            trace.push_back(r);
        }
        trace[trace_n].name = name;
        SMJ_CHECK(hipEventRecord(trace[trace_n].a, st));
        return (int)trace_n++;
    }
    void trace_end(int idx, hipStream_t st) {
        if (idx >= 0) SMJ_CHECK(hipEventRecord(trace[idx].b, st));
    }
    bool trace_ext(const char* name, hipEvent_t* a, hipEvent_t* b) {
        if (!traced(name)) return false;
        if (trace_n == trace.size()) {
            TraceRec r;
            SMJ_CHECK(hipEventCreate(&r.a));
            SMJ_CHECK(hipEventCreate(&r.b));
            trace.push_back(r);
        }
        trace[trace_n].name = name;
        *a = trace[trace_n].a;
        *b = trace[trace_n].b;
        trace_n++;
        return true;
    }

    ~Workspace() {
        for (auto& r : trace) {
            (void)hipEventDestroy(r.a);
            (void)hipEventDestroy(r.b);
        }
        for (auto& kv : bufs) (void)hipFree(kv.second.first);
        for (auto& kv : pinned) (void)hipHostFree(kv.second.first);
        if (ev_init)
            for (auto& e : ev) (void)hipEventDestroy(e);
    }
};

struct TraceScope {
    Workspace* ws;
    hipStream_t st;
    int idx;
    TraceScope(Workspace* w, const char* name, hipStream_t s)
        : ws(w), st(s), idx(w ? w->trace_begin(name, s) : -1) {}
    ~TraceScope() {
        if (ws) ws->trace_end(idx, st);
    }
};

template <typename... KArgs, typename... Args>
inline void traced_launch(Workspace* ws, const char* name, void (*kernel)(KArgs...),
                          dim3 grid, dim3 block, uint32_t shmem, hipStream_t st,
                          Args... args) {
    hipEvent_t a, b;
    if (ws && ws->trace_ext(name, &a, &b))
        hipExtLaunchKernelGGL(kernel, grid, block, shmem, st, a, b, 0u, (KArgs)args...);
    else
        hipLaunchKernelGGL(kernel, grid, block, shmem, st, (KArgs)args...);
}

uint32_t glibc_rand_at(uint32_t seed, uint64_t k);
void gen_nonunique_ref(Workspace* ws, Tup* out, uint64_t n, uint64_t first, uint64_t total,
                       int64_t maxid, uint32_t seed, uint64_t skip, hipStream_t st);
void gen_zipf_ref(Workspace* ws, Tup* out, uint64_t n, uint64_t first, uint64_t maxid,
                  double theta, uint32_t seed, uint64_t skip, hipStream_t st);

void xsend(const int64_t* start, const int64_t* cnt, const unsigned int* flags, uint32_t F,
           uint32_t K, uint32_t G, uint32_t U, int64_t* msg, int64_t* chunk, hipStream_t st);
void xrecv(const int64_t* msg, const int64_t* chunk, uint32_t G, uint32_t rank, uint32_t mine,
           uint32_t K, uint32_t nb, uint64_t cap, int64_t* tstart, int64_t* tcnt,
           int64_t* summary, hipStream_t st);
void hist_tables(const int64_t* hist, uint32_t F, uint32_t K, int64_t* start, int64_t* cnt,
                 hipStream_t st);

void stable_partition(Workspace* ws, const Tup* in, uint64_t n, Tup* out,
                      const Digit32& dig, uint32_t dbits, int padded,
                      int64_t* hist_out, int64_t* off_out, hipStream_t st);
void plan_partition(Workspace* ws, const Tup* in, uint64_t n, Tup* out,
                    const RangePlan* plan_dev, uint32_t dbits,
                    uint64_t* starts_dev, int64_t* hist_out, hipStream_t st);
#ifdef KEY_8B
void plan_partition_packed(Workspace* ws, const Tup* in, uint64_t n, uint64_t* out,
                           const RangePlan* plan_dev, const RangePlan& pack_plan,
                           uint32_t dbits, uint64_t* starts_dev, int64_t* hist_out,
                           unsigned int* pack_bad, hipStream_t st);
#endif
uint64_t sampled_capacity(uint64_t n, uint32_t dbits);
#ifndef SMJ_SHARDS
#define SMJ_SHARDS 8
#endif
constexpr uint32_t kShards = SMJ_SHARDS;
void sampled_partition(Workspace* ws, int nrel, const Tup* const* in, const uint64_t* n,
                       void* const* out, const RangePlan* plan_dev, uint32_t dbits,
                       unsigned int* sample, uint64_t* const* starts_dev,
                       int64_t* const* hist_out, uint64_t* const* seg_start,
                       int64_t* const* seg_cnt, unsigned int* flag_dev, hipStream_t st,
                       const RangePlan* host_plan = nullptr, bool packed = false,
                       unsigned int* bad = nullptr, uint64_t p48_stride = 0,
                       bool p32 = false, bool exact = false, bool p96 = false);
void hist_memcpy(Workspace* ws, const Tup* in, uint64_t n, Tup* out,
                 uint32_t dbits, hipStream_t st);
uint64_t lds_order_selfcheck(Workspace* ws, hipStream_t st);

extern const uint32_t kGroupTarget;
extern const uint32_t kTileTuples;
extern const uint32_t kGroupD3Max;
struct BucketSortArgs {
    const void* part[2];
    const uint64_t* bstart[2];
    const int64_t* bcount[2];
    const uint64_t* seg_start[2] = {nullptr, nullptr};
    const int64_t* seg_cnt[2] = {nullptr, nullptr};
    uint32_t nseg = kShards;
    void* tmp[2];
    Tup* out[2];
    uint64_t n[2];
    int nrel;
    uint32_t nbuckets;
    const RangePlan* plan_dev;
    unsigned long long* count_dev;
    const unsigned int* part_flag = nullptr;
    const RangePlan* host_plan = nullptr;
    bool packed = false;
    bool p48 = false;
    uint64_t pstride[2] = {0, 0};
    bool p32 = false;
    bool p96 = false;
    unsigned int* status = nullptr;
    const unsigned int* pack_bad = nullptr;
    uint32_t* status_out = nullptr;
    bool digit_fast = true;
    uint32_t stage = 7;
    hipEvent_t ev_tile = nullptr;
    hipEvent_t ev_bucket = nullptr;
    hipEvent_t ev_ovf = nullptr;
};
bool bucket_sort(Workspace* ws, const BucketSortArgs& a, hipStream_t st);
int tilepass_occupancy(bool p32, uint32_t d2);

void plan_from_sample(Workspace* ws, const Tup* const* rels,
                      const uint64_t* ns, int nrel, uint32_t D1, uint32_t D2,
                      uint32_t D2cap, int64_t hint_min, int64_t hint_max,
                      RangePlan* plan_dev, hipStream_t st);

void segmented_sort(Workspace* ws, Tup* data, const uint64_t* seg_off_host,
                    const uint64_t* seg_len_host, uint32_t nseg, hipStream_t st);
void merge2(Workspace* ws, const Tup* a, uint64_t na, const Tup* b, uint64_t nb, Tup* out,
            hipStream_t st);
void merge_join_count(const Tup* r, uint64_t nr, const Tup* s, uint64_t ns,
                      unsigned long long* count_dev, hipStream_t st);
void merge_join_count_batch(Workspace* ws, const Tup* const* r, const uint64_t* nr,
                            const Tup* const* s, const uint64_t* ns, uint32_t k,
                            unsigned long long* count_dev, hipStream_t st);
void multiway_merge(Workspace* ws, const Tup* const* runs_host,
                    const uint64_t* lens_host, uint32_t k, Tup* out,
                    hipStream_t st);
void multiway_merge_tree(Workspace* ws, const Tup* const* runs_host,
                         const uint64_t* lens_host, uint32_t k, Tup* out,
                         hipStream_t st);

uint64_t materialize(Workspace* ws, const Tup* R, uint64_t nR, const Tup* S,
                     uint64_t nS, Tup* out, uint64_t out_cap, hipStream_t st);
uint64_t join_pairs(Workspace* ws, const Tup* R, uint64_t nR, const Tup* S, uint64_t nS,
                    void* r_out, void* s_out, void* key_out, uint64_t out_cap,
                    hipStream_t st);
uint64_t semi_join(Workspace* ws, const Tup* R, uint64_t nR, const Tup* S, uint64_t nS,
                   Tup* out, uint64_t out_cap, int anti, hipStream_t st);
void mat_scan(Workspace* ws, const uint64_t* cnt, uint64_t ntiles, uint64_t* base,
              uint64_t* ibase, uint64_t* tot, hipStream_t st);

uint64_t band_join(Workspace* ws, const Tup* R, uint64_t nR, const Tup* S, uint64_t nS,
                   int64_t lo, int64_t hi, void* r_out, void* s_out, void* r_key_out,
                   void* s_key_out, uint64_t out_cap, hipStream_t st);
void band_join_count(Workspace* ws, const Tup* R, uint64_t nR, const Tup* S, uint64_t nS,
                     int64_t lo, int64_t hi, unsigned long long* count_dev, hipStream_t st);

void gen_pk(Tup* out, uint64_t n, uint64_t first, uint64_t total,
            uint64_t seed, hipStream_t st);
void gen_fk(Tup* out, uint64_t n, uint64_t first, uint64_t total,
            uint64_t maxid, uint64_t seed, hipStream_t st);
void gen_zipf(Workspace* ws, Tup* out, uint64_t n, uint64_t first,
              uint64_t maxid, double theta, uint64_t seed, hipStream_t st);

}
```

### avx-sort-merge-joins_amd/smj/__init__.py

```python
from __future__ import annotations

import ctypes as C
import os

import numpy as np

try:
    import torch
except Exception:
    torch = None

PKG = os.path.dirname(os.path.abspath(__file__))
ROOT = os.path.dirname(PKG)
LIBDIR = os.environ.get("SMJ_LIB_DIR") or os.path.join(ROOT, "lib")
TUPLE8 = np.dtype([("payload", "<i4"), ("key", "<i4")])
TUPLE16 = np.dtype([("payload", "<i8"), ("key", "<i8")])

REFERENCE_SYMBOLS = [
    "partition_relation", "partition_relation_optimized",
    "partition_relation_optimized_V2", "histogram_memcpy_bench",
    "avxsort_tuples", "avxsort_int64", "avxsort_int32",
    "avxsortmultiway_tuples", "avxsortmultiway_int64",
    "scalarsort_tuples", "scalarsort_int64", "scalarsort_int32",
    "avx_merge_tuples", "avx_merge_int64", "scalar_merge_tuples",
    "scalar_merge_int64", "avx_multiway_merge", "scalar_multiway_merge",
    "scalar_multiway_merge_modulo", "scalar_multiway_merge_bitand",
    "merge_join", "merge_join_interpolation", "print_timing", "sortmergejoin_multiway",
    "sortmergejoin_multipass", "sortmergejoin_mpsm", "sortmergejoin_initrun",
    "chainedtuplebuffer_init", "chainedtuplebuffer_free", "chainedtuplebuffer_tuples",
    "cb_next_writepos", "write_result_relation", "radix_cluster", "is_sorted_helper",
    "check_sorted",
]
DEVICE_SYMBOLS = [
    "smj_tuple_bytes", "smj_device_name", "smj_workspace_create",
    "smj_workspace_destroy", "smj_dev_partition", "smj_dev_sort",
    "smj_dev_merge2", "smj_dev_multiway_merge_host", "smj_dev_merge_join_count",
    "smj_dev_join", "smj_join_phase_ms", "smj_dev_gen_pk", "smj_dev_gen_fk",
    "smj_dev_gen_zipf", "smj_dev_synchronize", "smj_dev_partition_range",
    "smj_trace_enable", "smj_trace_reset", "smj_trace_only", "smj_trace_read", "smj_dev_join_segmented",
    "smj_dev_partition_range_packed", "smj_dev_materialize", "smj_selfcheck_lds_order",
    "smj_set_materialize", "smj_dev_join_segmented_tables", "smj_dev_partition_range_sampled",
    "smj_sampled_capacity", "smj_sampled_shards", "smj_context_workspace",
    "smj_dev_gen_nonunique", "smj_dev_gen_zipf_ref", "smj_glibc_rand",
    "smj_dev_xsend", "smj_dev_xrecv", "smj_join", "smj_dev_partition_range_planes",
    "smj_dev_join_segmented_planes", "smj_mgpu_join", "smj_mgpu_release",
    "smj_inregister_sort_keyval32", "smj_workspace_set_layouts", "smj_mgpu_unique_id",
    "smj_mgpu_comm_init", "smj_mgpu_rank_join", "smj_mgpu_comm_destroy", "smj_mgpu_rank_sorted",
    "smj_mgpu_comm_workspace", "smj_workspace_last_layout", "smj_mgpu_join_slices",
    "smj_mgpu_last_stats", "smj_mgpu_last_sorted", "smj_mgpu_group_workspace",
    "smj_dev_partition_range_shards", "smj_tilepass_occupancy",
    "smj_dev_join_pairs", "smj_dev_semi_join",
    "smj_dev_band_join", "smj_dev_band_join_count",
]


def lib_path(width: int) -> str:
    return os.path.join(LIBDIR, "libsmj_hip.so" if width == 8 else "libsmj_hip_k8.so")


def build(jobs: int = 8) -> None:
    import subprocess
    subprocess.check_call(["make", "-C", ROOT, f"-j{jobs}"])


class Relation(C.Structure):
    _fields_ = [("tuples", C.c_void_p), ("num_tuples", C.c_uint64)]


class JoinConfig(C.Structure):
    _fields_ = [("NTHREADS", C.c_int), ("PARTFANOUT", C.c_int),
                ("SCALARSORT", C.c_int), ("SCALARMERGE", C.c_int),
                ("MWAYMERGEBUFFERSIZE", C.c_int), ("NUMASTRATEGY", C.c_int)]


class ThreadResult(C.Structure):
    _fields_ = [("nresults", C.c_int64), ("results", C.c_void_p),
                ("threadid", C.c_uint32)]


class Result(C.Structure):
    _fields_ = [("totalresults", C.c_int64),
                ("resultlist", C.POINTER(ThreadResult)), ("nthreads", C.c_int)]


class MgpuStats(C.Structure):
    _fields_ = [("layout", C.c_int), ("pbits", C.c_uint32), ("attempts", C.c_int),
                ("replans", C.c_int), ("sent_bytes", C.c_uint64), ("recv_bytes", C.c_uint64),
                ("key_min", C.c_int64), ("key_max", C.c_int64), ("ms", C.c_double),
                ("partition_ms", C.c_double), ("tables_ms", C.c_double),
                ("wait_ms", C.c_double), ("join_ms", C.c_double), ("reduce_ms", C.c_double),
                ("busy_ms", C.c_double), ("rows_ms", C.c_double)]

    def as_dict(self):
        d = {f: getattr(self, f) for f, _ in self._fields_}
        d["layout"] = MG_LAYOUTS[d["layout"]]
        return d


LAYOUT_NO_P48, LAYOUT_NO_PACKED, LAYOUT_NO_SAMPLED, LAYOUT_SAMPLE_PLAN = 1, 2, 4, 8
LAYOUT_NO_P32, LAYOUT_NO_P96 = 16, 32
LAYOUTS_USED = ("tuples", "words", "p48", "p32", "p96")
MG_COPY, MG_NOPLANES, MG_ONECALL, MG_SAMPLED, MG_EXACT = 1, 2, 4, 8, 16
MG_LAYOUTS = ("tuples", "words", "planes")


class MgpuComm:

    def __init__(self, lib, handle):
        self.lib, self.h = lib, handle

    def join(self, R, S, flags=0, key_range=None, guess_max=0):
        L = self.lib
        nR, nS = C.c_uint64(), C.c_uint64()
        st = MgpuStats()
        kmin, kmax = key_range if key_range is not None else (1, 0)
        torch.cuda.current_stream(R.device).synchronize()
        c = L.lib.smj_mgpu_rank_join(self.h, R.data_ptr(), R.shape[0], S.data_ptr(),
                                     S.shape[0], flags, kmin, kmax, guess_max, None,
                                     C.byref(nR), None, C.byref(nS), C.byref(st))
        stats = st.as_dict()
        self.n = (nR.value, nS.value)
        return int(c), nR.value, nS.value, stats

    def sorted(self):
        sR, sS = self.lib.empty(self.n[0]), self.lib.empty(self.n[1])
        self.lib.lib.smj_mgpu_rank_sorted(self.h, sR.data_ptr() if self.n[0] else None,
                                          sS.data_ptr() if self.n[1] else None)
        return sR, sS

    def close(self):
        if self.h:
            self.lib.lib.smj_mgpu_comm_destroy(self.h)
            self.h = None


class ChainedTupleBuffer(C.Structure):
    _fields_ = [("tuples", C.c_void_p), ("numtuples", C.c_uint64),
                ("capacity", C.c_uint64)]


_P = C.c_void_p
_U64 = C.c_uint64
_I64 = C.c_int64
_U32 = C.c_uint32


_HIP = None


def _hip_copy(dst: int, src: int, nbytes: int) -> None:
    global _HIP
    if _HIP is None:
        _HIP = C.CDLL("libamdhip64.so")
        _HIP.hipMemcpy.argtypes = [C.c_void_p, C.c_void_p, C.c_size_t, C.c_int]
        _HIP.hipMemcpy.restype = C.c_int
    rc = _HIP.hipMemcpy(dst, src, nbytes, 4)
    if rc != 0:
        raise RuntimeError(f"hipMemcpy failed: {rc}")


def _ptr(a):
    return a.ctypes.data


class Library:
    def __init__(self, width: int = 16, path: str | None = None):
        assert width in (8, 16)
        self.width = width
        self.dtype = TUPLE8 if width == 8 else TUPLE16
        self.path = path or lib_path(width)
        if not os.path.exists(self.path):
            raise FileNotFoundError(
                f"{self.path} missing: build it with `make -C {ROOT}` "
                "(there is no CPU fallback)")
        self.lib = C.CDLL(self.path)
        L = self.lib
        sig = {
            "partition_relation": (None, [_P, _P, _P, C.c_int, C.c_int]),
            "partition_relation_optimized": (None, [_P, _P, _P, _U32, _U32]),
            "partition_relation_optimized_V2": (None, [_P, _P, _P, _U32, _U32]),
            "histogram_memcpy_bench": (None, [_P, _P, _P, _U32]),
            "avxsort_tuples": (None, [_P, _P, _U64]),
            "avxsort_int64": (None, [_P, _P, _U64]),
            "avxsort_int32": (None, [_P, _P, _U64]),
            "avxsortmultiway_tuples": (None, [_P, _P, _U64]),
            "avxsortmultiway_int64": (None, [_P, _P, _U64]),
            "scalarsort_tuples": (None, [_P, _P, _U64]),
            "scalarsort_int64": (None, [_P, _P, _U64]),
            "scalarsort_int32": (None, [_P, _P, _U64]),
            "avx_merge_tuples": (_U64, [_P, _P, _P, _U64, _U64]),
            "avx_merge_int64": (_U64, [_P, _P, _P, _U64, _U64]),
            "scalar_merge_tuples": (_U64, [_P, _P, _P, _U64, _U64]),
            "scalar_merge_int64": (_U64, [_P, _P, _P, _U64, _U64]),
            "avx_multiway_merge": (_U64, [_P, _P, _U32, _P, _U32]),
            "scalar_multiway_merge": (_U64, [_P, _P, _U32, _P, _U32]),
            "merge_join": (_U64, [_P, _P, _U64, _U64, _P]),
            "sortmergejoin_multiway": (C.POINTER(Result), [_P, _P, _P]),
            "sortmergejoin_multipass": (C.POINTER(Result), [_P, _P, _P]),
            "sortmergejoin_mpsm": (C.POINTER(Result), [_P, _P, _P]),
            "chainedtuplebuffer_init": (C.POINTER(ChainedTupleBuffer), []),
            "chainedtuplebuffer_free": (None, [_P]),
            "chainedtuplebuffer_tuples": (_U64, [_P]),
            "cb_next_writepos": (_P, [_P]),
            "write_result_relation": (None, [_P, C.c_char_p]),
            "smj_set_materialize": (None, [C.c_int]),
            "smj_join": (C.POINTER(Result), [_P, _P, _P, C.c_int, C.c_int]),
            "radix_cluster": (None, [_P, _P, _P, C.c_int, C.c_int]),
            "is_sorted_helper": (C.c_int, [_P, _U64]),
            "check_sorted": (None, [_P, _P, _U64, _U64, C.c_int]),
            "smj_tuple_bytes": (C.c_int, []),
            "smj_device_name": (C.c_char_p, []),
            "smj_workspace_create": (_P, []),
            "smj_workspace_destroy": (None, [_P]),
            "smj_dev_partition": (None, [_P, _P, _U64, _P, _U32, _U32, C.c_int, _P, _P, _P]),
            "smj_dev_sort": (None, [_P, _P, _U64, _P, _P]),
            "smj_dev_merge2": (None, [_P, _U64, _P, _U64, _P, _P]),
            "smj_dev_multiway_merge_host": (None, [_P, _P, _P, _U32, _P, _P]),
            "smj_dev_merge_join_count": (None, [_P, _U64, _P, _U64, _P, _P]),
            "smj_dev_join": (None, [_P, _P, _U64, _P, _U64, _P, _P, _U32, _I64, _I64, _P, _P]),
            "smj_join_phase_ms": (None, [_P, _P]),
            "smj_dev_gen_pk": (None, [_P, _U64, _U64, _U64, _U64, C.c_int, _P]),
            "smj_dev_gen_fk": (None, [_P, _U64, _U64, _U64, _U64, _U64, _P]),
            "smj_dev_gen_zipf": (None, [_P, _P, _U64, _U64, _U64, C.c_double, _U64, _P]),
            "smj_dev_synchronize": (None, [_P]),
            "smj_dev_partition_range": (None, [_P, _P, _U64, _P, _U32, _I64, _I64, _P, _P]),
            "smj_dev_join_segmented": (None, [_P, _P, _U64, _P, _P, _U64, _P, _U32, _U32,
                                              _I64, _I64, _U32, _P, _P, _P, _P]),
            "smj_dev_partition_range_packed": (C.c_int, [_P, _P, _U64, _P, _U32, _I64, _I64,
                                                         _P, _P, _P]),
            "smj_dev_join_segmented_tables": (None, [_P, _P, _U64, _P, _P, _P, _U64, _P, _P,
                                                     _U32, _U32, _I64, _I64, _U32, _P, _P,
                                                     _P, _P]),
            "smj_dev_partition_range_sampled": (C.c_int, [_P, _P, _U64, _P, _U32, _I64, _I64,
                                                          C.c_int, _P, _P, _P, _P]),
            "smj_dev_partition_range_shards": (C.c_int, [_P, _P, _U64, _P, _U32, _I64, _I64,
                                                         C.c_int, _P, _P, _P, _P]),
            "smj_dev_partition_range_planes": (C.c_int, [_P, _P, _U64, _P, _U64, _U32, _I64,
                                                         _I64, _P, _P, _P, _P]),
            "smj_dev_join_segmented_planes": (None, [_P, _P, _U64, _U64, _P, _P, _P, _U64,
                                                     _U64, _P, _P, _U32, _U32, _I64, _I64,
                                                     _U32, _P, _P, _P, _P]),
            "smj_sampled_capacity": (_U64, [_U64, _U32]),
            "smj_sampled_shards": (_U32, []),
            "smj_dev_materialize": (_U64, [_P, _P, _U64, _P, _U64, _P, _U64, _P]),
            "smj_dev_join_pairs": (_U64, [_P, _P, _U64, _P, _U64, _P, _P, _P, _U64, _P]),
            "smj_dev_semi_join": (_U64, [_P, _P, _U64, _P, _U64, _P, _U64, C.c_int, _P]),
            "smj_dev_band_join": (_U64, [_P, _P, _U64, _P, _U64, _I64, _I64, _P, _P, _P, _P,
                                         _U64, _P]),
            "smj_dev_band_join_count": (None, [_P, _P, _U64, _P, _U64, _I64, _I64, _P, _P]),
            "smj_selfcheck_lds_order": (_U64, [_P, _P]),
            "smj_context_workspace": (_P, []),
            "smj_dev_gen_nonunique": (None, [_P, _P, _U64, _U64, _U64, _I64, _U32, _U64, _P]),
            "smj_dev_gen_zipf_ref": (None, [_P, _P, _U64, _U64, _U64, C.c_double, _U32, _U64,
                                            _P]),
            "smj_glibc_rand": (_U32, [_U32, _U64]),
            "smj_dev_xsend": (None, [_P, _P, _P, _U32, _U32, _U32, _U32, _P, _P, _P]),
            "smj_dev_xrecv": (None, [_P, _P, _U32, _U32, _U32, _U32, _U32, _U64, _P, _P, _P,
                                     _P]),
            "smj_mgpu_join": (_I64, [_P, _U64, _P, _U64, C.c_int, _U32, _I64, _I64, _P, _P,
                                     _P, _P]),
            "smj_mgpu_release": (None, []),
            "smj_mgpu_join_slices": (_I64, [_P, _P, _P, _P, C.c_int, _U32, _I64, _I64, _P, _P]),
            "smj_mgpu_last_stats": (C.c_int, [C.c_int, _P]),
            "smj_mgpu_group_workspace": (_P, [C.c_int]),
            "smj_mgpu_last_sorted": (C.c_int, [C.c_int, _P, _P, _P, _P]),
            "smj_mgpu_unique_id": (C.c_int, [_P, C.c_int]),
            "smj_mgpu_comm_init": (_P, [_P, C.c_int, C.c_int]),
            "smj_mgpu_rank_join": (_I64, [_P, _P, _U64, _P, _U64, _U32, _I64, _I64, _U64,
                                          _P, _P, _P, _P, _P]),
            "smj_mgpu_comm_destroy": (None, [_P]),
            "smj_mgpu_rank_sorted": (None, [_P, _P, _P]),
            "smj_mgpu_comm_workspace": (_P, [_P]),
            "smj_inregister_sort_keyval32": (None, [_P, _P, _U64]),
            "smj_workspace_set_layouts": (None, [_P, _U32]),
            "smj_workspace_last_layout": (C.c_int, [_P]),
            "smj_tilepass_occupancy": (C.c_int, [C.c_int, _U32]),
            "smj_trace_enable": (None, [_P, C.c_int]),
            "smj_trace_reset": (None, [_P]),
            "smj_trace_only": (None, [_P, C.c_char_p]),
            "smj_trace_read": (C.c_int, [_P, C.c_char_p, C.c_int, _P, _P, C.c_int]),
        }
        for name, (res, args) in sig.items():
            try:
                f = getattr(L, name)
            except AttributeError:
                if os.environ.get("SMJ_LIB_DIR"):
                    continue
                raise
            f.restype = res
            f.argtypes = args
        got = L.smj_tuple_bytes()
        assert got == width, f"{self.path} built for {got}-byte tuples"
        self._ws = None

    def _rel(self, a: np.ndarray) -> Relation:
        return Relation(a.ctypes.data, len(a))

    def _parts(self, fan: int):
        rels = (Relation * fan)()
        ptrs = (C.POINTER(Relation) * fan)(*[C.pointer(rels[i]) for i in range(fan)])
        return rels, ptrs

    def partition(self, t: np.ndarray, nbits: int, shift: int, variant: int = 1):
        fan = 1 << nbits
        t = np.ascontiguousarray(t, dtype=self.dtype)
        out = np.zeros(len(t) + fan * 64 // self.width, self.dtype)
        rin, rout = self._rel(t), self._rel(out)
        rout.num_tuples = len(t)
        rels, ptrs = self._parts(fan)
        fn = [self.lib.partition_relation, self.lib.partition_relation_optimized,
              self.lib.partition_relation_optimized_V2][variant]
        fn(C.cast(ptrs, _P), C.byref(rin), C.byref(rout), nbits, shift)
        base = out.ctypes.data
        cnt = np.array([rels[i].num_tuples for i in range(fan)], np.int64)
        off = np.array([(rels[i].tuples - base) // self.width for i in range(fan)], np.int64)
        return out, cnt, off

    def radix_cluster(self, t: np.ndarray, shift: int, bits: int, hist=None):
        t = np.ascontiguousarray(t, dtype=self.dtype)
        h = np.zeros(1 << bits, np.int32) if hist is None else \
            np.ascontiguousarray(hist, dtype=np.int32).copy()
        out = np.zeros(len(t) + int(h.sum()), self.dtype)
        rin, rout = self._rel(t), self._rel(out)
        self.lib.radix_cluster(C.byref(rout), C.byref(rin), _ptr(h), shift, bits)
        return out, h

    def is_sorted_helper(self, t: np.ndarray) -> int:
        t = np.ascontiguousarray(t, dtype=self.dtype)
        return int(self.lib.is_sorted_helper(_ptr(t) if len(t) else None, len(t)))

    def avxsort_tuples(self, t: np.ndarray, fn: str = "avxsort_tuples") -> np.ndarray:
        a = np.ascontiguousarray(t, dtype=self.dtype).copy()
        b = np.zeros_like(a)
        pa, pb = C.c_void_p(a.ctypes.data), C.c_void_p(b.ctypes.data)
        getattr(self.lib, fn)(C.byref(pa), C.byref(pb), len(a))
        res = b if pb.value == b.ctypes.data else a
        return res.copy()

    def sort_int(self, v: np.ndarray, fn: str = "avxsort_int64") -> np.ndarray:
        dt = np.int32 if fn.endswith("int32") else np.int64
        a = np.ascontiguousarray(v, dtype=dt).copy()
        b = np.zeros_like(a)
        pa, pb = C.c_void_p(a.ctypes.data), C.c_void_p(b.ctypes.data)
        getattr(self.lib, fn)(C.byref(pa), C.byref(pb), len(a))
        return (b if pb.value == b.ctypes.data else a).copy()

    def inregister_sort_keyval32(self, items: np.ndarray) -> np.ndarray:
        a = np.ascontiguousarray(items, dtype=np.int64)
        out = np.zeros_like(a)
        self.lib.smj_inregister_sort_keyval32(_ptr(a), _ptr(out), len(a) // 16)
        return out

    def merge_int64(self, a, b, fn="avx_merge_int64") -> np.ndarray:
        a = np.ascontiguousarray(a, dtype=np.int64)
        b = np.ascontiguousarray(b, dtype=np.int64)
        out = np.zeros(len(a) + len(b), np.int64)
        n = getattr(self.lib, fn)(_ptr(a), _ptr(b), _ptr(out), len(a), len(b))
        assert n == len(out)
        return out

    def avx_merge_tuples(self, a, b, fn="avx_merge_tuples") -> np.ndarray:
        a = np.ascontiguousarray(a, dtype=self.dtype)
        b = np.ascontiguousarray(b, dtype=self.dtype)
        out = np.zeros(len(a) + len(b), self.dtype)
        n = getattr(self.lib, fn)(_ptr(a), _ptr(b), _ptr(out), len(a), len(b))
        assert n == len(out)
        return out

    def avx_multiway_merge(self, runs, fn="avx_multiway_merge"):
        runs = [np.ascontiguousarray(r, dtype=self.dtype) for r in runs]
        k = len(runs)
        total = sum(len(r) for r in runs)
        out = np.zeros(total, self.dtype)
        rels = (Relation * k)(*[Relation(r.ctypes.data, len(r)) for r in runs])
        ptrs = (C.POINTER(Relation) * k)(*[C.pointer(rels[i]) for i in range(k)])
        fifo = np.zeros(1 << 16, self.dtype)
        n = getattr(self.lib, fn)(_ptr(out), C.cast(ptrs, _P), k, _ptr(fifo), len(fifo))
        consumed = all(rels[i].num_tuples == 0 and
                       rels[i].tuples == runs[i].ctypes.data + len(runs[i]) * self.width
                       for i in range(k))
        return out, int(n), consumed

    def merge_join(self, r, s) -> int:
        r = np.ascontiguousarray(r, dtype=self.dtype)
        s = np.ascontiguousarray(s, dtype=self.dtype)
        return int(self.lib.merge_join(_ptr(r), _ptr(s), len(r), len(s), None))

    def _take_buffer(self, cb) -> np.ndarray:
        n = int(self.lib.chainedtuplebuffer_tuples(cb))
        if n == 0:
            return np.zeros(0, self.dtype)
        b = C.cast(cb, C.POINTER(ChainedTupleBuffer)).contents
        raw = C.string_at(b.tuples, n * self.width)
        return np.frombuffer(raw, dtype=self.dtype).copy()

    def merge_join_materialize(self, r, s, prefix=None):
        r = np.ascontiguousarray(r, dtype=self.dtype)
        s = np.ascontiguousarray(s, dtype=self.dtype)
        cb = self.lib.chainedtuplebuffer_init()
        try:
            for t in (prefix if prefix is not None else []):
                p = self.lib.cb_next_writepos(cb)
                C.memmove(p, np.array([t], self.dtype).ctypes.data, self.width)
            n = int(self.lib.merge_join(_ptr(r), _ptr(s), len(r), len(s), cb))
            return n, self._take_buffer(cb)
        finally:
            self.lib.chainedtuplebuffer_free(cb)

    def mgpu_join(self, R, S, nranks=0, flags=0, key_range=None, sorted_out=True):
        dev = not isinstance(R, np.ndarray)
        if dev:
            for t in (R, S):
                torch.cuda.current_stream(t.device).synchronize()
            nR, nS = R.shape[0], S.shape[0]
            pR, pS = R.data_ptr(), S.data_ptr()
            sR = R.new_empty(R.shape) if sorted_out else None
            sS = S.new_empty(S.shape) if sorted_out else None
            qR = sR.data_ptr() if sorted_out else None
            qS = sS.data_ptr() if sorted_out else None
        else:
            R = np.ascontiguousarray(R, dtype=self.dtype)
            S = np.ascontiguousarray(S, dtype=self.dtype)
            nR, nS = len(R), len(S)
            pR, pS = (_ptr(R) if nR else None), (_ptr(S) if nS else None)
            sR = np.zeros(nR, self.dtype) if sorted_out else None
            sS = np.zeros(nS, self.dtype) if sorted_out else None
            qR = _ptr(sR) if sorted_out and nR else None
            qS = _ptr(sS) if sorted_out and nS else None
        G = nranks
        if G <= 0:
            import torch as _t
            G = _t.cuda.device_count()
        counts = np.zeros(2 * G, np.uint64)
        st = MgpuStats()
        kmin, kmax = key_range if key_range is not None else (1, 0)
        c = self.lib.smj_mgpu_join(pR, nR, pS, nS, G, flags, kmin, kmax, qR, qS,
                                   _ptr(counts), C.byref(st))
        return int(c), sR, sS, counts.reshape(G, 2), st.as_dict()

    def mgpu_join_slices(self, Rs, Ss, flags=0, key_range=None):
        G = len(Rs)
        assert G == len(Ss) and G >= 1
        for t in list(Rs) + list(Ss):
            torch.cuda.current_stream(t.device).synchronize()
        P, U = C.c_void_p * G, C.c_uint64 * G
        pR = P(*[t.data_ptr() if t.shape[0] else None for t in Rs])
        pS = P(*[t.data_ptr() if t.shape[0] else None for t in Ss])
        nR = U(*[t.shape[0] for t in Rs])
        nS = U(*[t.shape[0] for t in Ss])
        counts = np.zeros(2 * G, np.uint64)
        st = MgpuStats()
        kmin, kmax = key_range if key_range is not None else (1, 0)
        c = self.lib.smj_mgpu_join_slices(pR, nR, pS, nS, G, flags, kmin, kmax, _ptr(counts),
                                          C.byref(st))
        return int(c), counts.reshape(G, 2), [self.mgpu_last_stats(g) for g in range(G)]

    def mgpu_last_stats(self, rank):
        st = MgpuStats()
        if self.lib.smj_mgpu_last_stats(rank, C.byref(st)) != 0:
            raise IndexError(f"no rank {rank} in the last multi-GPU join")
        return st.as_dict()

    def mgpu_last_sorted(self, rank, device):
        pR, pS = C.c_void_p(), C.c_void_p()
        nR, nS = C.c_uint64(), C.c_uint64()
        if self.lib.smj_mgpu_last_sorted(rank, C.byref(pR), C.byref(nR), C.byref(pS),
                                         C.byref(nS)) != 0:
            raise IndexError(f"no rank {rank} in the last multi-GPU join")
        out = []
        for p, n in ((pR, nR.value), (pS, nS.value)):
            t = self.empty(n, device=device)
            if n:
                _hip_copy(t.data_ptr(), p.value, n * self.width)
            out.append(t)
        return tuple(out)

    def mgpu_comm(self, nranks, rank, group=None):
        import torch.distributed as dist
        idb = np.zeros(128, np.uint8)
        if rank == 0:
            n = self.lib.smj_mgpu_unique_id(_ptr(idb), len(idb))
            assert n == 128, n
        if nranks > 1:
            t = torch.from_numpy(idb.astype(np.int64))
            if dist.get_backend(group) == "nccl":
                t = t.cuda()
            dist.broadcast(t, src=dist.get_global_rank(group, 0) if group is not None else 0,
                           group=group)
            idb = t.cpu().numpy().astype(np.uint8)
        c = self.lib.smj_mgpu_comm_init(_ptr(idb), nranks, rank)
        return MgpuComm(self, c)

    def sortmergejoin_multiway(self, R, S, nthreads=1, fanout=128, mpsm=False,
                               algo=None, materialize=False, persist=None):
        R = np.ascontiguousarray(R, dtype=self.dtype)
        S = np.ascontiguousarray(S, dtype=self.dtype)
        cfg = JoinConfig(nthreads, fanout, int(self.width == 16), int(self.width == 16),
                         20 << 20, 2)
        rr, rs = self._rel(R), self._rel(S)
        algo = algo or ("mpsm" if mpsm else "m-way")
        code = {"m-way": 0, "m-pass": 1, "mpsm": 2}[algo]
        res = self.lib.smj_join(C.byref(rr), C.byref(rs), C.byref(cfg), code,
                                1 if (materialize or persist) else 0)
        if not res:
            return None
        total = int(res.contents.totalresults)
        out = None
        if materialize or persist:
            if persist:
                self.lib.write_result_relation(C.cast(res, _P), os.fsencode(persist))
            lists = [res.contents.resultlist[i].results for i in range(max(nthreads, 1))]
            out = np.concatenate([self._take_buffer(cb) for cb in lists if cb] or
                                 [np.zeros(0, self.dtype)])
            for cb in lists:
                self.lib.chainedtuplebuffer_free(cb)
        libc = C.CDLL(None)
        libc.free.argtypes = [C.c_void_p]
        libc.free(res.contents.resultlist)
        libc.free(C.cast(res, C.c_void_p))
        return total if out is None else (total, out)

    @property
    def ws(self):
        if self._ws is None:
            self._ws = self.lib.smj_workspace_create()
        return self._ws

    def set_layouts(self, off: int = 0):
        self.lib.smj_workspace_set_layouts(self.ws, off)

    def reset_workspace(self):
        if self._ws is not None:
            import torch
            torch.cuda.synchronize()
            self.lib.smj_workspace_destroy(self._ws)
            self._ws = None

    def last_layout(self, api: bool = False) -> str:
        f = getattr(self.lib, "smj_workspace_last_layout", None)
        if f is None or f.restype is not C.c_int:
            return "unknown"
        k = f(None if api else self.ws)
        return LAYOUTS_USED[k] if k >= 0 else "none"

    def tilepass_occupancy(self, layout: str = "p48", d2_bits: int = 10) -> int:
        return int(self.lib.smj_tilepass_occupancy(LAYOUTS_USED.index(layout), d2_bits))

    @staticmethod
    def stream_ptr():
        return torch.cuda.current_stream().cuda_stream

    def empty(self, n: int, device="cuda"):
        dt = torch.int32 if self.width == 8 else torch.int64
        return torch.empty((max(n, 1), 2), dtype=dt, device=device)[:n]

    def to_device(self, a: np.ndarray):
        v = np.ascontiguousarray(a, dtype=self.dtype).view(
            np.int32 if self.width == 8 else np.int64).reshape(-1, 2)
        return torch.from_numpy(v.copy()).cuda()

    def to_host(self, t) -> np.ndarray:
        return t.cpu().numpy().reshape(-1).view(self.dtype).copy()

    def dev_gen_pk(self, out, first, total, seed, with_payload=True):
        self.lib.smj_dev_gen_pk(out.data_ptr(), out.shape[0], first, total, seed,
                                int(with_payload), self.stream_ptr())

    def dev_gen_fk(self, out, first, total, maxid, seed):
        self.lib.smj_dev_gen_fk(out.data_ptr(), out.shape[0], first, total, maxid,
                                seed, self.stream_ptr())

    def dev_gen_zipf(self, out, first, maxid, theta, seed):
        self.lib.smj_dev_gen_zipf(self.ws, out.data_ptr(), out.shape[0], first, maxid,
                                  theta, seed, self.stream_ptr())

    def dev_gen_nonunique(self, out, first, total, maxid, seed, skip=0):
        self.lib.smj_dev_gen_nonunique(self.ws, out.data_ptr(), out.shape[0], first, total,
                                       maxid, seed, skip, self.stream_ptr())

    def dev_gen_zipf_ref(self, out, first, maxid, theta, seed, skip=0):
        self.lib.smj_dev_gen_zipf_ref(self.ws, out.data_ptr(), out.shape[0], first, maxid,
                                      theta, seed, skip, self.stream_ptr())

    def dev_xsend(self, start, cnt, flags, world, msg, chunk, used=0):
        F, K = start.shape
        self.lib.smj_dev_xsend(start.data_ptr(), cnt.data_ptr(), flags.data_ptr(), F, K, world,
                               used, msg.data_ptr(), chunk.data_ptr(), self.stream_ptr())

    def dev_xrecv(self, msg, chunk, world, rank, mine, K, tstart, tcnt, cap, summary):
        self.lib.smj_dev_xrecv(msg.data_ptr(), chunk.data_ptr(), world, rank, mine, K,
                               tstart.shape[0], cap, tstart.data_ptr(), tcnt.data_ptr(),
                               summary.data_ptr(), self.stream_ptr())

    def glibc_rand(self, seed, k):
        return int(self.lib.smj_glibc_rand(seed, k))

    def dev_sort(self, inp, out):
        self.lib.smj_dev_sort(self.ws, inp.data_ptr(), inp.shape[0], out.data_ptr(),
                              self.stream_ptr())

    def dev_partition(self, inp, out, nbits, shift, padded, hist, off):
        self.lib.smj_dev_partition(self.ws, inp.data_ptr(), inp.shape[0], out.data_ptr(),
                                   nbits, shift, int(padded), hist.data_ptr(),
                                   off.data_ptr(), self.stream_ptr())

    def dev_merge2(self, a, b, out):
        self.lib.smj_dev_merge2(a.data_ptr(), a.shape[0], b.data_ptr(), b.shape[0],
                                out.data_ptr(), self.stream_ptr())

    def dev_merge_join_count(self, r, s, count):
        self.lib.smj_dev_merge_join_count(r.data_ptr(), r.shape[0], s.data_ptr(),
                                          s.shape[0], count.data_ptr(), self.stream_ptr())

    @staticmethod
    def run_table(runs):
        k = len(runs)
        ptrs = (C.c_void_p * k)(*[r.data_ptr() for r in runs])
        lens = (C.c_uint64 * k)(*[r.shape[0] for r in runs])
        return C.cast(ptrs, _P), C.cast(lens, _P), k, (ptrs, lens)

    def dev_multiway_merge(self, runs, out):
        ptrs, lens, k, _keep = runs if isinstance(runs, tuple) else self.run_table(runs)
        self.lib.smj_dev_multiway_merge_host(self.ws, ptrs, lens, k, out.data_ptr(),
                                             self.stream_ptr())

    def dev_materialize(self, sortedR, sortedS, out=None):
        cap = 0 if out is None else out.shape[0]
        return int(self.lib.smj_dev_materialize(
            self.ws, sortedR.data_ptr(), sortedR.shape[0], sortedS.data_ptr(),
            sortedS.shape[0], out.data_ptr() if cap else None, cap, self.stream_ptr()))

    def _column(self, t, cap, what):
        dt = torch.int32 if self.width == 8 else torch.int64
        assert t.dim() == 1 and t.dtype == dt and t.is_contiguous() and t.is_cuda, what
        assert t.shape[0] >= cap, f"{what} holds fewer than the {cap} of r_out"
        return t.data_ptr() if cap else None

    def dev_join_pairs(self, sortedR, sortedS, r_out=None, s_out=None, key_out=None):
        cap = 0 if r_out is None else r_out.shape[0]
        assert (s_out is None) == (r_out is None), "r_out and s_out go together"
        assert r_out is not None or key_out is None, "key_out needs r_out and s_out"
        rp = self._column(r_out, cap, "r_out") if r_out is not None else None
        sp = self._column(s_out, cap, "s_out") if s_out is not None else None
        kp = self._column(key_out, cap, "key_out") if key_out is not None else None
        return int(self.lib.smj_dev_join_pairs(
            self.ws, sortedR.data_ptr(), sortedR.shape[0], sortedS.data_ptr(),
            sortedS.shape[0], rp, sp, kp, cap, self.stream_ptr()))

    def dev_semi_join(self, sortedR, sortedS, out=None, anti=False):
        cap = 0 if out is None else out.shape[0]
        return int(self.lib.smj_dev_semi_join(
            self.ws, sortedR.data_ptr(), sortedR.shape[0], sortedS.data_ptr(),
            sortedS.shape[0], out.data_ptr() if cap else None, cap, int(bool(anti)),
            self.stream_ptr()))

    def join_index(self, R, S, key_range=None, with_keys=False):
        dt = torch.int32 if self.width == 8 else torch.int64
        sR, sS = self.empty(R.shape[0]), self.empty(S.shape[0])
        count = torch.zeros(1, dtype=torch.int64, device=R.device)
        kmin, kmax = key_range if key_range is not None else (1, 0)
        self.dev_join(R, S, sR, sS, count, 10, kmin, kmax)
        total = int(count.item())
        cols = [torch.empty(total, dtype=dt, device=R.device)
                for _ in range(3 if with_keys else 2)]
        if total:
            got = self.dev_join_pairs(sR, sS, *cols)
            assert got == total, (got, total)
        return tuple(cols)

    @staticmethod
    def _band(lo, hi):
        lo, hi = int(lo), int(hi)
        for v in (lo, hi):
            assert -(1 << 63) <= v < (1 << 63), "lo and hi are int64"
        return lo, hi

    def dev_band_join(self, sortedR, sortedS, lo, hi, r_out=None, s_out=None,
                      r_key_out=None, s_key_out=None):
        lo, hi = self._band(lo, hi)
        cap = 0 if r_out is None else r_out.shape[0]
        assert (s_out is None) == (r_out is None), "r_out and s_out go together"
        assert r_out is not None or (r_key_out is None and s_key_out is None), \
            "key columns need r_out and s_out"
        ptrs = [self._column(t, cap, what) if t is not None else None
                for t, what in ((r_out, "r_out"), (s_out, "s_out"),
                                (r_key_out, "r_key_out"), (s_key_out, "s_key_out"))]
        return int(self.lib.smj_dev_band_join(
            self.ws, sortedR.data_ptr(), sortedR.shape[0], sortedS.data_ptr(),
            sortedS.shape[0], lo, hi, *ptrs, cap, self.stream_ptr()))

    def dev_band_join_count(self, sortedR, sortedS, lo, hi, count):
        lo, hi = self._band(lo, hi)
        self.lib.smj_dev_band_join_count(
            self.ws, sortedR.data_ptr(), sortedR.shape[0], sortedS.data_ptr(),
            sortedS.shape[0], lo, hi, count.data_ptr(), self.stream_ptr())

    def band_join(self, R, S, lo, hi, with_keys=False):
        dt = torch.int32 if self.width == 8 else torch.int64
        total = 0
        if R.shape[0] and S.shape[0]:
# ... 124 lines not shown
```

### include/smj.h

```cpp
#ifndef SMJ_H
#define SMJ_H

#include <stdint.h>
#include <stddef.h>
#include <stdio.h>
#include <inttypes.h>
#include <sys/time.h>
#include <pthread.h>

#ifdef __cplusplus
extern "C" {
#endif

#ifndef TYPES_H
#define TYPES_H
#ifdef KEY_8B
typedef int64_t intkey_t;
typedef int64_t value_t;
#else
typedef int32_t intkey_t;
typedef int32_t value_t;
#endif

typedef struct tuple_t        tuple_t;
// ... 136 lines not shown
    tuple_t * tuples;
    uint64_t  numtuples;
    uint64_t  capacity;
} chainedtuplebuffer_t;
chainedtuplebuffer_t * chainedtuplebuffer_init(void);
void chainedtuplebuffer_free(chainedtuplebuffer_t * cb);
uint64_t chainedtuplebuffer_tuples(chainedtuplebuffer_t * cb);
tuple_t * cb_next_writepos(chainedtuplebuffer_t * cb);
#endif

uint64_t merge_join(tuple_t * rtuples, tuple_t * stuples, const uint64_t numR,
                    const uint64_t numS, void * output);

void smj_set_materialize(int on);

result_t * smj_join(relation_t * relR, relation_t * relS, joinconfig_t * joincfg,
                    int algo, int materialize);

void write_result_relation(result_t * result, const char * filename);

#ifndef SMJ_COMPAT_HIDE_PRINT_TIMING
void print_timing(uint64_t numtuples, struct timeval * start,
                  struct timeval * end, FILE * out);
#endif

int is_sorted_helper(int64_t * items, uint64_t nitems);

void check_sorted(int64_t * R, int64_t * S, uint64_t nR, uint64_t nS, int my_tid);

uint64_t merge_join_interpolation(tuple_t * rtuples, tuple_t * stuples,
                                  const uint64_t numR, const uint64_t numS,
                                  void * output);

#ifndef SMJ_ARG_T
#define SMJ_ARG_T
typedef struct arg_t arg_t;
typedef struct relationpair_t relationpair_t;
struct arg_t {
    tuple_t *  relR;
    tuple_t *  relS;
    tuple_t *  tmp_partR;
    tuple_t *  tmp_partS;
    tuple_t *  tmp_sortR;
    tuple_t *  tmp_sortS;
    int32_t numR;
    int32_t numS;
    int32_t my_tid;
    int     nthreads;
    joinconfig_t * joincfg;
    pthread_barrier_t * barrier;
    int64_t result;
    relationpair_t ** threadrelchunks;
    tuple_t ** sharedmergebuffer;
    uint32_t ** histR;
    tuple_t * tmpRglobal;
    uint64_t totalR;
#ifdef JOIN_MATERIALIZE
    threadresult_t * threadresult;
#endif
    struct timeval start, end;
    uint64_t part, sort, mergedelta, merge, join;
} __attribute__((aligned(CACHE_LINE_SIZE)));
struct relationpair_t {
    relation_t R;
    relation_t S;
};
#endif

result_t * sortmergejoin_initrun(relation_t * relR, relation_t * relS,
                                 joinconfig_t * joincfg,
                                 void * (*jointhread)(void *));

result_t * sortmergejoin_multiway(relation_t * relR, relation_t * relS,
                                  joinconfig_t * joincfg);

result_t * sortmergejoin_multipass(relation_t * relR, relation_t * relS,
                                   joinconfig_t * joincfg);

result_t * sortmergejoin_mpsm(relation_t * relR, relation_t * relS,
                              joinconfig_t * joincfg);

#define SMJ_MG_COPY     1u
#define SMJ_MG_NOPLANES 2u
#define SMJ_MG_ONECALL  4u
#define SMJ_MG_SAMPLED  8u
#define SMJ_MG_EXACT   16u
typedef struct smj_mgpu_stats {
    int      layout;
    uint32_t pbits;
    int      attempts;
    int      replans;
    uint64_t sent_bytes;
    uint64_t recv_bytes;
    int64_t  key_min;
    int64_t  key_max;
    double   ms;
    double   partition_ms;
    double   tables_ms;
    double   wait_ms;
    double   join_ms;
    double   reduce_ms;
    double   busy_ms;
    double   rows_ms;
} smj_mgpu_stats;
int64_t smj_mgpu_join(const tuple_t * R, uint64_t nR, const tuple_t * S, uint64_t nS,
                      int nranks, uint32_t flags, int64_t key_min, int64_t key_max,
                      tuple_t * sortedR, tuple_t * sortedS, uint64_t * rank_counts,
                      smj_mgpu_stats * stats);
int64_t smj_mgpu_join_slices(const tuple_t * const * R, const uint64_t * nR,
                             const tuple_t * const * S, const uint64_t * nS, int nranks,
                             uint32_t flags, int64_t key_min, int64_t key_max,
                             uint64_t * rank_counts, smj_mgpu_stats * stats);
int smj_mgpu_last_stats(int rank, smj_mgpu_stats * out);
int smj_mgpu_last_sorted(int rank, tuple_t ** sortedR, uint64_t * nR, tuple_t ** sortedS,
                         uint64_t * nS);
struct smj_workspace * smj_mgpu_group_workspace(int rank);
void smj_mgpu_release(void);

typedef struct smj_mgpu_comm smj_mgpu_comm;
int smj_mgpu_unique_id(void * out, int cap);
smj_mgpu_comm * smj_mgpu_comm_init(const void * id, int nranks, int rank);
int64_t smj_mgpu_rank_join(smj_mgpu_comm * comm, const tuple_t * R, uint64_t nR,
                           const tuple_t * S, uint64_t nS, uint32_t flags,
                           int64_t key_min, int64_t key_max, uint64_t guess_max,
                           tuple_t ** sortedR, uint64_t * nR_out, tuple_t ** sortedS,
                           uint64_t * nS_out, smj_mgpu_stats * stats);
void smj_mgpu_rank_sorted(smj_mgpu_comm * comm, tuple_t * outR, tuple_t * outS);
struct smj_workspace * smj_mgpu_comm_workspace(smj_mgpu_comm * comm);
void smj_mgpu_comm_destroy(smj_mgpu_comm * comm);

typedef void * smj_stream_t;

int smj_tuple_bytes(void);
const char * smj_device_name(void);

typedef struct smj_workspace smj_workspace;
smj_workspace * smj_workspace_create(void);
void smj_workspace_destroy(smj_workspace * ws);

#define SMJ_LAYOUT_NO_P48      1u
#define SMJ_LAYOUT_NO_PACKED   2u
#define SMJ_LAYOUT_NO_SAMPLED  4u
#define SMJ_LAYOUT_SAMPLE_PLAN 8u
#define SMJ_LAYOUT_NO_P32     16u
#define SMJ_LAYOUT_NO_P96     32u
void smj_workspace_set_layouts(smj_workspace * ws, uint32_t off);
#define SMJ_LAYOUT_USED_TUPLES 0
#define SMJ_LAYOUT_USED_WORDS  1
#define SMJ_LAYOUT_USED_P48    2
#define SMJ_LAYOUT_USED_P32    3
#define SMJ_LAYOUT_USED_P96    4
int smj_workspace_last_layout(smj_workspace * ws);
int smj_tilepass_occupancy(int layout, uint32_t d2_bits);

void smj_dev_partition(smj_workspace * ws, const tuple_t * in, uint64_t n,
                       tuple_t * out, uint32_t nbits, uint32_t shiftbits,
                       int padded, int64_t * hist_out, int64_t * off_out,
                       smj_stream_t stream);

void smj_dev_sort(smj_workspace * ws, const tuple_t * in, uint64_t n,
                  tuple_t * out, smj_stream_t stream);

void smj_dev_merge2(const tuple_t * a, uint64_t na, const tuple_t * b,
                    uint64_t nb, tuple_t * out, smj_stream_t stream);

void smj_dev_multiway_merge_host(smj_workspace * ws,
                                 const tuple_t * const * runs,
                                 const uint64_t * lens, uint32_t k,
                                 tuple_t * out, smj_stream_t stream);

void smj_dev_merge_join_count(const tuple_t * r, uint64_t nr,
                              const tuple_t * s, uint64_t ns,
                              unsigned long long * count_dev,
                              smj_stream_t stream);

uint64_t smj_dev_materialize(smj_workspace * ws, const tuple_t * sortedR,
                             uint64_t nR, const tuple_t * sortedS, uint64_t nS,
                             tuple_t * out, uint64_t out_cap, smj_stream_t stream);

uint64_t smj_dev_join_pairs(smj_workspace * ws, const tuple_t * sortedR, uint64_t nR,
                            const tuple_t * sortedS, uint64_t nS, value_t * r_payload_out,
                            value_t * s_payload_out, intkey_t * key_out ,
                            uint64_t out_cap, smj_stream_t stream);

uint64_t smj_dev_semi_join(smj_workspace * ws, const tuple_t * sortedR, uint64_t nR,
                           const tuple_t * sortedS, uint64_t nS, tuple_t * out,
                           uint64_t out_cap, int anti, smj_stream_t stream);

uint64_t smj_dev_band_join(smj_workspace * ws, const tuple_t * sortedR, uint64_t nR,
                           const tuple_t * sortedS, uint64_t nS, int64_t lo, int64_t hi,
                           value_t * r_payload_out, value_t * s_payload_out,
                           intkey_t * r_key_out ,
                           intkey_t * s_key_out ,
                           uint64_t out_cap, smj_stream_t stream);

void smj_dev_band_join_count(smj_workspace * ws, const tuple_t * sortedR, uint64_t nR,
                             const tuple_t * sortedS, uint64_t nS, int64_t lo, int64_t hi,
                             unsigned long long * count_dev, smj_stream_t stream);

void smj_dev_join(smj_workspace * ws, const tuple_t * R, uint64_t nR,
                  const tuple_t * S, uint64_t nS, tuple_t * sortedR,
                  tuple_t * sortedS, uint32_t fanout_bits, int64_t key_min,
                  int64_t key_max, unsigned long long * count_dev,
                  smj_stream_t stream);

void smj_join_phase_ms(smj_workspace * ws, float * ms5);

void smj_dev_gen_pk(tuple_t * out, uint64_t n, uint64_t first, uint64_t total,
                    uint64_t seed, int with_payload, smj_stream_t stream);
void smj_dev_gen_fk(tuple_t * out, uint64_t n, uint64_t first, uint64_t total,
                    uint64_t maxid, uint64_t seed, smj_stream_t stream);
void smj_dev_gen_zipf(smj_workspace * ws, tuple_t * out, uint64_t n,
                      uint64_t first, uint64_t maxid, double theta,
                      uint64_t seed, smj_stream_t stream);

void smj_dev_gen_nonunique(smj_workspace * ws, tuple_t * out, uint64_t n, uint64_t first,
                           uint64_t total, int64_t maxid, uint32_t seed, uint64_t skip,
                           smj_stream_t stream);
void smj_dev_gen_zipf_ref(smj_workspace * ws, tuple_t * out, uint64_t n, uint64_t first,
                          uint64_t maxid, double theta, uint32_t seed, uint64_t skip,
                          smj_stream_t stream);
uint32_t smj_glibc_rand(uint32_t seed, uint64_t k);

void smj_dev_synchronize(smj_stream_t stream);

void smj_dev_partition_range(smj_workspace * ws, const tuple_t * in, uint64_t n,
                             tuple_t * out, uint32_t nbits, int64_t key_min,
                             int64_t key_max, int64_t * hist_out,
                             smj_stream_t stream);

int smj_dev_partition_range_packed(smj_workspace * ws, const tuple_t * in, uint64_t n,
                                   uint64_t * out, uint32_t nbits, int64_t key_min,
                                   int64_t key_max, int64_t * hist_out,
                                   unsigned int * bad_flag, smj_stream_t stream);

#define SMJ_SEG_PACKED 1u
#define SMJ_SEG_STAGE_R 2u
#define SMJ_SEG_STAGE_REST 4u
void smj_dev_join_segmented(smj_workspace * ws, void * R, uint64_t nR,
                            const int64_t * segR, void * S, uint64_t nS,
                            const int64_t * segS, uint32_t nseg,
                            uint32_t bucket_bits, int64_t key_lo, int64_t key_hi,
                            uint32_t flags, tuple_t * sortedR, tuple_t * sortedS,
                            unsigned long long * count_dev, smj_stream_t stream);

void smj_dev_join_segmented_tables(smj_workspace * ws, void * R, uint64_t nR,
                                   const int64_t * startR, const int64_t * cntR,
                                   void * S, uint64_t nS, const int64_t * startS,
                                   const int64_t * cntS, uint32_t nseg,
                                   uint32_t bucket_bits, int64_t key_lo, int64_t key_hi,
                                   uint32_t flags, tuple_t * sortedR, tuple_t * sortedS,
                                   unsigned long long * count_dev, smj_stream_t stream);

void smj_dev_join_segmented_planes(smj_workspace * ws, void * R, uint64_t strideR,
                                   uint64_t nR, const int64_t * startR,
                                   const int64_t * cntR, void * S, uint64_t strideS,
                                   uint64_t nS, const int64_t * startS,
                                   const int64_t * cntS, uint32_t nseg,
                                   uint32_t bucket_bits, int64_t key_lo, int64_t key_hi,
                                   uint32_t flags, tuple_t * sortedR, tuple_t * sortedS,
                                   unsigned long long * count_dev, smj_stream_t stream);

int smj_dev_partition_range_sampled(smj_workspace * ws, const tuple_t * in, uint64_t n,
                                    void * out, uint32_t nbits, int64_t key_min,
                                    int64_t key_max, int packed, int64_t * seg_start,
                                    int64_t * seg_cnt, unsigned int * flags,
                                    smj_stream_t stream);
int smj_dev_partition_range_planes(smj_workspace * ws, const tuple_t * in, uint64_t n,
                                   void * out, uint64_t stride, uint32_t nbits,
                                   int64_t key_min, int64_t key_max, int64_t * seg_start,
                                   int64_t * seg_cnt, unsigned int * flags,
                                   smj_stream_t stream);
int smj_dev_partition_range_shards(smj_workspace * ws, const tuple_t * in, uint64_t n,
                                   void * out, uint32_t nbits, int64_t key_min,
                                   int64_t key_max, int packed, int64_t * seg_start,
                                   int64_t * seg_cnt, unsigned int * flags,
                                   smj_stream_t stream);
uint64_t smj_sampled_capacity(uint64_t n, uint32_t nbits);
uint32_t smj_sampled_shards(void);

void smj_dev_xsend(const int64_t * start, const int64_t * cnt, const unsigned int * flags,
                   uint32_t F, uint32_t K, uint32_t world, uint32_t used, int64_t * msg,
                   int64_t * chunk, smj_stream_t stream);
void smj_dev_xrecv(const int64_t * msg, const int64_t * chunk, uint32_t world, uint32_t rank,
                   uint32_t mine, uint32_t K, uint32_t nbuckets, uint64_t cap,
                   int64_t * tstart, int64_t * tcnt, int64_t * summary, smj_stream_t stream);

uint64_t smj_selfcheck_lds_order(smj_workspace * ws, smj_stream_t stream);

smj_workspace * smj_context_workspace(void);

void smj_trace_enable(smj_workspace * ws, int on);
void smj_trace_reset(smj_workspace * ws);
void smj_trace_only(smj_workspace * ws, const char * name);
int smj_trace_read(smj_workspace * ws, char * names, int cap, float * ms_sum,
                   int * launches, int max);

#ifdef __cplusplus
}
#endif
#endif
```

Before: 88180 Mtuples/s.

## Software-pipeline range scatter kernel with prefetch, double-buffered fill counters and quad stores

Restructures the KEY_8B range-scatter kernel so the next tile's loads are issued while the current tile is histogrammed, staged and written out. Non-owner waves prefetch early and owner waves after their atomic reservation, with an explicit vmcnt wait. The per-bin fill counters are double-buffered so one barrier can be dropped, and digits are packed into 16-bit pairs to save registers. Pack error checks move into an accumulator reduced once at the end, and a 4-wide store path is added for the p48 layout. This adds register pressure, inline asm and more LDS, and a query API reports scatter tile size and resource use.

```diff
diff --git a/avx-sort-merge-joins_amd/csrc/capi.hip b/avx-sort-merge-joins_amd/csrc/capi.hip
--- a/avx-sort-merge-joins_amd/csrc/capi.hip
+++ b/avx-sort-merge-joins_amd/csrc/capi.hip
@@ -1533,6 +1533,17 @@
     return tilepass_occupancy(layout == SMJ_LAYOUT_USED_P32, d2_bits);
 }
 
+uint32_t smj_scatter_tile(int layout, uint32_t nbins) {
+    return (uint32_t)scatter_query(layout, nbins, 0, nullptr, nullptr);
+}
+
+int smj_scatter_resources(int layout, uint32_t nbins, int vec, int* num_regs,
+                          int* scratch_bytes) {
+    if (!num_regs || !scratch_bytes) return -1;
+    ctx();
+    return scatter_query(layout, nbins, vec, num_regs, scratch_bytes) ? 0 : -1;
+}
+
 void smj_dev_partition(smj_workspace* ws, const tuple_t* in, uint64_t n,
                        tuple_t* out, uint32_t nbits, uint32_t shiftbits,
                        int padded, int64_t* hist_out, int64_t* off_out,
diff --git a/avx-sort-merge-joins_amd/csrc/partition.hip b/avx-sort-merge-joins_amd/csrc/partition.hip
--- a/avx-sort-merge-joins_amd/csrc/partition.hip
+++ b/avx-sort-merge-joins_amd/csrc/partition.hip
@@ -1173,7 +1173,7 @@
     }
     static __host__ __device__ constexpr size_t lds_bytes(uint32_t nbins) {
         return (size_t)TILE * sizeof(OutT) + (size_t)nbins * SEG * sizeof(OutT) +
-               (size_t)nbins * (8 + 4 * 4) + ((size_t)max_segs(nbins) * 2 + 15) / 16 * 16 +
+               (size_t)nbins * (8 + 5 * 4) + ((size_t)max_segs(nbins) * 2 + 15) / 16 * 16 +
                (THREADS / 64 + 1) * 4;
     }
 };
@@ -1188,6 +1188,145 @@
     else return false;
 }
 
+template <class Geo, class OutT>
+struct ScatterLds {
+    OutT* stage;
+    OutT* carry;
+    uint64_t* pos;
+    uint32_t *tstart, *tfill_a, *tfill_b, *kc, *segpre, *scr;
+    uint16_t* segown;
+    __device__ __forceinline__ ScatterLds(unsigned char* raw, uint32_t nbins) {
+        stage = reinterpret_cast<OutT*>(raw);
+        carry = stage + Geo::TILE;
+        pos = reinterpret_cast<uint64_t*>(carry + (size_t)nbins * Geo::SEG);
+        tstart = reinterpret_cast<uint32_t*>(pos + nbins);
+        tfill_a = tstart + nbins;
+        tfill_b = tfill_a + nbins;
+        kc = tfill_b + nbins;
+        segpre = kc + nbins;
+        segown = reinterpret_cast<uint16_t*>(segpre + nbins);
+        scr = reinterpret_cast<uint32_t*>(reinterpret_cast<unsigned char*>(segown) +
+                                          ((size_t)Geo::max_segs(nbins) * 2 + 15) / 16 * 16);
+    }
+};
+
+template <int THREADS, int ITEMS, bool VEC>
+__device__ __forceinline__ void scatter_load_tile(Tup (&x)[ITEMS],
+                                                  const unsigned char* __restrict__ cin,
+                                                  uint32_t clen, uint32_t r0) {
+#ifndef KEY_8B
+    typedef unsigned long long V2 __attribute__((ext_vector_type(2)));
+    if constexpr (VEC) {
+        const uint32_t vl = clen / 2 - 1;
+#pragma unroll
+        for (int p = 0; p < ITEMS / 2; p++) {
+            const uint32_t vi = r0 / 2 + (uint32_t)p * THREADS + threadIdx.x;
+            const V2* q = reinterpret_cast<const V2*>(cin + (vi < vl ? vi : vl) * 16u);
+#if SMJ_NT_LOADS
+            const V2 y = __builtin_nontemporal_load(q);
+#else
+            const V2 y = *q;
+#endif
+            x[2 * p] = (Tup)y.x;
+            x[2 * p + 1] = (Tup)y.y;
+        }
+    } else
+#endif
+    {
+#pragma unroll
+        for (int j = 0; j < ITEMS; j++) {
+            const uint32_t i = r0 + (uint32_t)j * THREADS + threadIdx.x;
+            x[j] = ld_stream(reinterpret_cast<const Tup*>(
+                cin + (i < clen ? i : clen - 1) * (uint32_t)sizeof(Tup)));
+        }
+    }
+}
+
+template <int THREADS, class Pack, class Geo>
+__device__ __forceinline__ void scatter_store_segments(
+    const ScatterLds<Geo, typename Pack::OutT>& L, uint32_t nseg, void* __restrict__ out,
+    uint64_t ostride) {
+    typedef typename Pack::OutT OutT;
+    constexpr uint32_t SEG = Geo::SEG;
+    const OutT* stage = L.stage;
+    const OutT* carry = L.carry;
+    const uint64_t* pos = L.pos;
+    const uint32_t *tstart = L.tstart, *kc = L.kc, *segpre = L.segpre;
+    const uint16_t* segown = L.segown;
+    if constexpr (pack_quads<Pack>() && SEG == 4) {
+        for (uint32_t sg = threadIdx.x; sg < nseg; sg += THREADS) {
+            const uint32_t d = segown[sg];
+            const uint32_t e = (sg - segpre[d]) * SEG;
+            const uint32_t k = kc[d];
+            const uint64_t p = pos[d];
+            OutT x[4];
+#pragma unroll
+            for (uint32_t i = 0; i < 4; i++)
+                x[i] = e + i < k ? carry[d * SEG + e + i] : stage[tstart[d] + e + i - k];
+            if (p != ~0ull) {
+                if ((p & 3) == 0) {
+                    Pack::store4(out, ostride, p + e, x);
+                } else {
+#pragma unroll
+                    for (uint32_t i = 0; i < 4; i++) Pack::store(out, ostride, p + e + i, x[i]);
+                }
+            }
+        }
+    } else if constexpr (Pack::kPairs) {
+        constexpr uint32_t PS = SEG / 2;
+        for (uint32_t q = threadIdx.x; q < nseg * PS; q += THREADS) {
+            const uint32_t sg = q / PS;
+            const uint32_t d = segown[sg];
+            const uint32_t e = (sg - segpre[d]) * SEG + 2 * (q % PS);
+            const uint32_t k = kc[d];
+            const uint64_t p = pos[d];
+            const OutT x0 = e < k ? carry[d * SEG + e] : stage[tstart[d] + e - k];
+            const OutT x1 = e + 1 < k ? carry[d * SEG + e + 1] : stage[tstart[d] + e + 1 - k];
+            if (p != ~0ull) {
+                if ((p & 1) == 0) {
+                    Pack::store2(out, ostride, p + e, x0, x1);
+                } else {
+                    Pack::store(out, ostride, p + e, x0);
+                    Pack::store(out, ostride, p + e + 1, x1);
+                }
+            }
+        }
+    } else {
+        for (uint32_t q = threadIdx.x; q < nseg * SEG; q += THREADS) {
+            const uint32_t sg = q / SEG;
+            const uint32_t d = segown[sg];
+            const uint32_t e = (sg - segpre[d]) * SEG + q % SEG;
+            const uint32_t k = kc[d];
+            const uint64_t p = pos[d];
+            const OutT x = e < k ? carry[d * SEG + e] : stage[tstart[d] + e - k];
+            if (p != ~0ull) Pack::store(out, ostride, p + e, x);
+        }
+    }
+}
+
+template <int THREADS, class Pack, class Geo>
+__device__ __forceinline__ void scatter_flush(const ScatterLds<Geo, typename Pack::OutT>& L,
+                                              uint32_t nbins, bool own,
+                                              unsigned long long* cursor_d0, uint64_t cap,
+                                              void* __restrict__ out, uint64_t ostride) {
+    constexpr uint32_t SEG = Geo::SEG;
+    if (own) {
+        const uint32_t d = threadIdx.x;
+        L.pos[d] = 0;
+        if (L.kc[d]) {
+            const uint64_t p = atomicAdd(cursor_d0, (unsigned long long)L.kc[d]);
+            L.pos[d] = p + L.kc[d] <= cap ? p : ~0ull;
+        }
+    }
+    __syncthreads();
+    for (uint32_t q = threadIdx.x; q < nbins * SEG; q += THREADS) {
+        const uint32_t d = q / SEG, j = q % SEG;
+        if (j < L.kc[d] && L.pos[d] != ~0ull)
+            Pack::store(out, ostride, L.pos[d] + j, L.carry[q]);
+    }
+}
+
+#ifdef KEY_8B
 template <int THREADS, int ITEMS, class Digit, class Pack, bool VEC>
 __global__ void __launch_bounds__(THREADS)
 k_scatter_res(const Tup* __restrict__ in, uint64_t n, uint64_t chunk, Digit dig_arg,
@@ -1199,25 +1338,24 @@
     typedef ScatterGeom<THREADS, ITEMS, OutT, Pack::kStoreBytes> Geo;
     constexpr uint32_t SEG = Geo::SEG;
     constexpr int TILE = (int)Geo::TILE;
-    uint32_t bad = 0;
+    PackAcc acc;
     const auto dig = dig_arg.load();
     const uint32_t shard = blockIdx.x % kShards;
     unsigned long long* cursor = cursor_all + shard;
     const uint64_t* cap_end = cap_end_all + shard;
     extern __shared__ __attribute__((aligned(16))) unsigned char lds_raw[];
-    OutT* stage = reinterpret_cast<OutT*>(lds_raw);
-    OutT* carry = stage + TILE;
-    uint64_t* pos = reinterpret_cast<uint64_t*>(carry + (size_t)nbins * SEG);
-    uint32_t* tstart = reinterpret_cast<uint32_t*>(pos + nbins);
-    uint32_t* tfill = tstart + nbins;
-    uint32_t* kc = tfill + nbins;
-    uint32_t* segpre = kc + nbins;
-    uint16_t* segown = reinterpret_cast<uint16_t*>(segpre + nbins);
-    uint32_t* scr = reinterpret_cast<uint32_t*>(
-        reinterpret_cast<unsigned char*>(segown) + ((size_t)Geo::max_segs(nbins) * 2 + 15) / 16 * 16);
+    const ScatterLds<Geo, OutT> L(lds_raw, nbins);
+    OutT* const stage = L.stage;
+    OutT* const carry = L.carry;
+    uint64_t* const pos = L.pos;
+    uint32_t *const tstart = L.tstart, *const kc = L.kc, *const segpre = L.segpre;
+    uint32_t* const scr = L.scr;
+    uint16_t* const segown = L.segown;
+    uint32_t *const tfill_a = L.tfill_a, *const tfill_b = L.tfill_b;
 
     for (uint32_t d = threadIdx.x; d < nbins; d += THREADS) {
-        tfill[d] = 0;
+        tfill_a[d] = 0;
+        tfill_b[d] = 0;
         kc[d] = 0;
     }
     const uint64_t beg = (uint64_t)blockIdx.x * chunk;
@@ -1233,32 +1371,170 @@
         return VEC ? 2u * ((uint32_t)(j / 2) * THREADS + threadIdx.x) + (uint32_t)(j & 1)
                    : (uint32_t)j * THREADS + threadIdx.x;
     };
+    const unsigned char* __restrict__ cin = reinterpret_cast<const unsigned char*>(in + beg);
+    const uint32_t clen = beg < end ? (uint32_t)(end - beg) : 1u;
+    auto load_tile = [&](Tup (&x)[ITEMS], uint32_t r0) {
+        scatter_load_tile<THREADS, ITEMS, VEC>(x, cin, clen, r0);
+    };
+    const uint32_t wid = __builtin_amdgcn_readfirstlane(threadIdx.x >> 6);
+    const uint32_t own_waves = (nbins + 63) / 64;
+    const bool own_wave = wid < own_waves;
+    constexpr uint32_t NLOADS = VEC ? ITEMS / 2 : ITEMS;
+    static_assert(NLOADS < 64, "the vmcnt field holds 6 bits");
+    Tup v[ITEMS];
+    if (beg < end) load_tile(v, 0);
+    uint32_t pend_e = 0;
+    auto take_carry = [&]() {
+        const uint32_t okc = kc[d0], ots = tstart[d0];
+        for (uint32_t e = pend_e; e < pend_e + my_kc; e++)
+            carry[d0 * SEG + (e - pend_e)] =
+                e < okc ? carry[d0 * SEG + e] : stage[ots + e - okc];
+        kc[d0] = my_kc;
+    };
+    uint32_t tsel = 0;
+    __syncthreads();
+    for (uint32_t base = 0; beg < end && base < clen; base += TILE) {
+        const uint32_t tcount = clen - base < (uint32_t)TILE ? clen - base : (uint32_t)TILE;
+        const uint32_t nb = base + TILE;
+        uint32_t* const tfill = tsel ? tfill_b : tfill_a;
+        uint32_t* const tnext = tsel ? tfill_a : tfill_b;
+        __builtin_amdgcn_s_waitcnt(0x0f70);
+        constexpr uint32_t kNoDigit = 0xffffu;
+        uint32_t dgp[(ITEMS + 1) / 2];
+        OutT w[ITEMS];
+#pragma unroll
+        for (int j = 0; j < ITEMS; j++) {
+            const uint32_t d = item_pos(j) < tcount ? dig(v[j]) : kNoDigit;
+            dgp[j / 2] = (j & 1) ? (dgp[j / 2] | (d << 16)) : d;
+            w[j] = pk.pack(v[j], acc);
+        }
+        auto digit = [&](int j) -> uint32_t {
+            return (j & 1) ? dgp[j / 2] >> 16 : dgp[j / 2] & 0xffffu;
+        };
+        if (!own_wave) load_tile(v, nb);
+#pragma unroll
+        for (int j = 0; j < ITEMS; j++) {
+            const uint32_t d = digit(j);
+            if (d != kNoDigit) atomicAdd(&tfill[d], 1u);
+        }
+        __syncthreads();
+        const uint32_t c = own ? tfill[d0] : 0;
+        const uint32_t T = my_kc + c;
+        uint32_t Eown = T / SEG * SEG;
+        const uint32_t sv = own ? (c | ((Eown / SEG) << 16)) : 0u;
+        uint32_t sx = sv;
+        if (own_wave) {
+            const int lane = lane_id();
+#pragma unroll
+            for (int o = 1; o < 64; o <<= 1) {
+                const uint32_t y = __shfl_up(sx, o, 64);
+                if (lane >= o) sx += y;
+            }
+            if (lane == 63) scr[wid] = sx;
+        }
+        __syncthreads();
+        uint32_t ex = sx - sv, tot = 0;
+        for (uint32_t k = 0; k < own_waves; k++) {
+            const uint32_t t = scr[k];
+            ex += k < wid ? t : 0u;
+            tot += t;
+        }
+        const uint32_t nseg = tot >> 16;
+        unsigned long long Pown = 0;
+        auto owner_phase = [&]() {
+            take_carry();
+            tnext[d0] = 0;
+            tstart[d0] = ex & 0xffffu;
+            tfill[d0] = ex & 0xffffu;
+            segpre[d0] = ex >> 16;
+            for (uint32_t k = 0; k < Eown / SEG; k++) segown[(ex >> 16) + k] = (uint16_t)d0;
+            if (Eown)
+                asm volatile("global_atomic_add_x2 %0, %1, %2, off sc0"
+                             : "=&v"(Pown)
+                             : "v"(&cursor[(size_t)d0 * kShards]), "v"((unsigned long long)Eown)
+                             : "memory");
+        };
+        auto stage_items = [&]() {
+#pragma unroll
+            for (int j = 0; j < ITEMS; j++) {
+                const uint32_t d = digit(j);
+                if (d != kNoDigit) stage[atomicAdd(&tfill[d], 1u)] = w[j];
+            }
+        };
+        auto owner_close = [&]() {
+            const bool ovf = Eown && Pown + Eown > my_cap;
+            pos[d0] = ovf ? ~0ull : Pown;
+            if (ovf) Eown = 0;
+            uint32_t left = T - Eown;
+            if (left > SEG - 1) left = SEG - 1;
+            pend_e = Eown;
+            my_kc = left;
+        };
+        if (own) owner_phase();
+        if (own_wave) load_tile(v, nb);
+        __syncthreads();
+        stage_items();
+        asm volatile("s_waitcnt vmcnt(%1)" : "+v"(Pown) : "n"(NLOADS) : "memory");
+        if (own) owner_close();
+        __syncthreads();
+        scatter_store_segments<THREADS, Pack, Geo>(L, nseg, out, ostride);
+        tsel ^= 1u;
+    }
+    __syncthreads();
+    if (own) take_carry();
+    scatter_flush<THREADS, Pack, Geo>(L, nbins, own, &cursor[(size_t)d0 * kShards], my_cap, out,
+                                      ostride);
+    const uint32_t bad = pk.flags(acc);
+    if (bad_flag && bad) atomicOr(bad_flag, bad);
+}
+#else
+template <int THREADS, int ITEMS, class Digit, class Pack, bool VEC>
+__global__ void __launch_bounds__(THREADS)
+k_scatter_res(const Tup* __restrict__ in, uint64_t n, uint64_t chunk, Digit dig_arg,
+              uint32_t nbins, unsigned long long* __restrict__ cursor_all,
+              const uint64_t* __restrict__ cap_end_all,
+              void* __restrict__ out, uint64_t ostride, Pack pk,
+              unsigned int* __restrict__ bad_flag) {
+    typedef typename Pack::OutT OutT;
+    typedef ScatterGeom<THREADS, ITEMS, OutT, Pack::kStoreBytes> Geo;
+    constexpr uint32_t SEG = Geo::SEG;
+    constexpr int TILE = (int)Geo::TILE;
+    PackAcc acc;
+    const auto dig = dig_arg.load();
+    const uint32_t shard = blockIdx.x % kShards;
+    unsigned long long* cursor = cursor_all + shard;
+    const uint64_t* cap_end = cap_end_all + shard;
+    extern __shared__ __attribute__((aligned(16))) unsigned char lds_raw[];
+    const ScatterLds<Geo, OutT> L(lds_raw, nbins);
+    OutT* const stage = L.stage;
+    OutT* const carry = L.carry;
+    uint64_t* const pos = L.pos;
+    uint32_t *const tstart = L.tstart, *const kc = L.kc, *const segpre = L.segpre;
+    uint32_t* const scr = L.scr;
+    uint16_t* const segown = L.segown;
+    uint32_t* const tfill = L.tfill_a;
+
+    for (uint32_t d = threadIdx.x; d < nbins; d += THREADS) {
+        tfill[d] = 0;
+        kc[d] = 0;
+    }
+    const uint64_t beg = (uint64_t)blockIdx.x * chunk;
+    uint64_t end = beg + chunk;
+    if (end > n) end = n;
+    const uint32_t d0 = threadIdx.x;
+    const bool own = d0 < nbins;
+    const uint32_t coff = d0 * kShards;
+    uint32_t my_kc = 0;
+
+    static_assert(!VEC || (sizeof(Tup) == 8 && ITEMS % 2 == 0), "VEC: 8-byte tuples, ITEMS even");
+    auto item_pos = [](int j) -> uint32_t {
+        return VEC ? 2u * ((uint32_t)(j / 2) * THREADS + threadIdx.x) + (uint32_t)(j & 1)
+                   : (uint32_t)j * THREADS + threadIdx.x;
+    };
+    const unsigned char* __restrict__ cin = reinterpret_cast<const unsigned char*>(in + beg);
+    const uint32_t clen = beg < end ? (uint32_t)(end - beg) : 1u;
     auto load_tile = [&](Tup (&x)[ITEMS], uint64_t b0) {
-#ifndef KEY_8B
-        typedef unsigned long long V2 __attribute__((ext_vector_type(2)));
-        if constexpr (VEC) {
-            const V2* __restrict__ vin = reinterpret_cast<const V2*>(in);
-            const uint64_t vl = end / 2 - 1;
-#pragma unroll
-            for (int p = 0; p < ITEMS / 2; p++) {
-                const uint64_t vi = b0 / 2 + (uint64_t)p * THREADS + threadIdx.x;
-#if SMJ_NT_LOADS
-                const V2 y = __builtin_nontemporal_load(vin + (vi < vl ? vi : vl));
-#else
-                const V2 y = vin[vi < vl ? vi : vl];
-#endif
-                x[2 * p] = (Tup)y.x;
-                x[2 * p + 1] = (Tup)y.y;
-            }
-        } else
-#endif
-        {
-#pragma unroll
-            for (int j = 0; j < ITEMS; j++) {
-                const uint64_t i = b0 + (uint64_t)j * THREADS + threadIdx.x;
-                x[j] = ld_stream(in + (i < end ? i : end - 1));
-            }
-        }
+        scatter_load_tile<THREADS, ITEMS, VEC>(x, cin, clen, (uint32_t)(b0 - beg));
     };
     Tup v[ITEMS], nv[ITEMS];
     if (beg < end) load_tile(v, beg);
@@ -1268,13 +1544,17 @@
             (uint32_t)((end - base) < (uint64_t)TILE ? (end - base) : TILE);
         const uint64_t nb = base + TILE;
         __builtin_amdgcn_s_waitcnt(0x0f70);
-        uint32_t dg[ITEMS];
-#pragma unroll
-        for (int j = 0; j < ITEMS; j++) {
-            const uint32_t li = item_pos(j);
-            dg[j] = li < tcount ? dig(v[j]) : 0xffffffffu;
-            if (dg[j] != 0xffffffffu) atomicAdd(&tfill[dg[j]], 1u);
-        }
+        constexpr uint32_t kNoDigit = 0xffffu;
+        uint32_t dgp[(ITEMS + 1) / 2];
+#pragma unroll
+        for (int j = 0; j < ITEMS; j++) {
+            const uint32_t d = item_pos(j) < tcount ? dig(v[j]) : kNoDigit;
+            dgp[j / 2] = (j & 1) ? (dgp[j / 2] | (d << 16)) : d;
+            if (d != kNoDigit) atomicAdd(&tfill[d], 1u);
+        }
+        auto digit = [&](int j) -> uint32_t {
+            return (j & 1) ? dgp[j / 2] >> 16 : dgp[j / 2] & 0xffffu;
+        };
         __syncthreads();
         const uint32_t c = own ? tfill[d0] : 0;
         const uint32_t T = my_kc + c;
@@ -1283,73 +1563,33 @@
         const uint32_t ex = block_exclusive_scan(own ? (c | ((Eown / SEG) << 16)) : 0u, scr, &tot);
         const uint32_t nseg = tot >> 16;
         unsigned long long Pown = 0;
+        uint64_t my_cap = 0;
         if (own) {
+            my_cap = cap_end[coff];
             tstart[d0] = ex & 0xffffu;
             tfill[d0] = ex & 0xffffu;
             segpre[d0] = ex >> 16;
             for (uint32_t k = 0; k < Eown / SEG; k++) segown[(ex >> 16) + k] = (uint16_t)d0;
-            if (Eown) Pown = atomicAdd(&cursor[(size_t)d0 * kShards], (unsigned long long)Eown);
+            if (Eown) Pown = atomicAdd(&cursor[coff], (unsigned long long)Eown);
         }
         load_tile(nv, nb);
         __syncthreads();
 #pragma unroll
-        for (int j = 0; j < ITEMS; j++)
-            if (dg[j] != 0xffffffffu) stage[atomicAdd(&tfill[dg[j]], 1u)] = pk(v[j], bad);
+        for (int j = 0; j < ITEMS; j++) {
+            const uint32_t d = digit(j);
+            if (d != kNoDigit) {
+                Tup t = v[j];
+                asm volatile("" : "+v"(t));
+                stage[atomicAdd(&tfill[d], 1u)] = pk.pack(t, acc);
+            }
+        }
         if (own) {
             const bool ovf = Eown && Pown + Eown > my_cap;
             pos[d0] = ovf ? ~0ull : Pown;
             if (ovf) Eown = 0;
         }
         __syncthreads();
-        if constexpr (pack_quads<Pack>() && SEG == 4) {
-            for (uint32_t sg = threadIdx.x; sg < nseg; sg += THREADS) {
-                const uint32_t d = segown[sg];
-                const uint32_t e = (sg - segpre[d]) * SEG;
-                const uint32_t k = kc[d];
-                const uint64_t p = pos[d];
-                OutT x[4];
-#pragma unroll
-                for (uint32_t i = 0; i < 4; i++)
-                    x[i] = e + i < k ? carry[d * SEG + e + i] : stage[tstart[d] + e + i - k];
-                if (p != ~0ull) {
-                    if ((p & 3) == 0) {
-                        Pack::store4(out, ostride, p + e, x);
-                    } else {
-#pragma unroll
-                        for (uint32_t i = 0; i < 4; i++) Pack::store(out, ostride, p + e + i, x[i]);
-                    }
-                }
-            }
-        } else if constexpr (Pack::kPairs) {
-            constexpr uint32_t PS = SEG / 2;
-            for (uint32_t q = threadIdx.x; q < nseg * PS; q += THREADS) {
-                const uint32_t sg = q / PS;
-                const uint32_t d = segown[sg];
-                const uint32_t e = (sg - segpre[d]) * SEG + 2 * (q % PS);
-                const uint32_t k = kc[d];
-                const uint64_t p = pos[d];
-                const OutT x0 = e < k ? carry[d * SEG + e] : stage[tstart[d] + e - k];
-                const OutT x1 = e + 1 < k ? carry[d * SEG + e + 1] : stage[tstart[d] + e + 1 - k];
-                if (p != ~0ull) {
-                    if ((p & 1) == 0) {
-                        Pack::store2(out, ostride, p + e, x0, x1);
-                    } else {
-                        Pack::store(out, ostride, p + e, x0);
-                        Pack::store(out, ostride, p + e + 1, x1);
-                    }
-                }
-            }
-        } else {
-            for (uint32_t q = threadIdx.x; q < nseg * SEG; q += THREADS) {
-                const uint32_t sg = q / SEG;
-                const uint32_t d = segown[sg];
-                const uint32_t e = (sg - segpre[d]) * SEG + q % SEG;
-                const uint32_t k = kc[d];
-                const uint64_t p = pos[d];
-                const OutT x = e < k ? carry[d * SEG + e] : stage[tstart[d] + e - k];
-                if (p != ~0ull) Pack::store(out, ostride, p + e, x);
-            }
-        }
+        scatter_store_segments<THREADS, Pack, Geo>(L, nseg, out, ostride);
         __syncthreads();
         if (own) {
             uint32_t left = T - Eown;
@@ -1365,21 +1605,12 @@
         for (int j = 0; j < ITEMS; j++) v[j] = nv[j];
         __syncthreads();
     }
-    if (own) {
-        const uint32_t d = d0;
-        pos[d] = 0;
-        if (kc[d]) {
-            const uint64_t p = atomicAdd(&cursor[(size_t)d * kShards], (unsigned long long)kc[d]);
-            pos[d] = p + kc[d] <= my_cap ? p : ~0ull;
-        }
-    }
-    __syncthreads();
-    for (uint32_t q = threadIdx.x; q < nbins * SEG; q += THREADS) {
-        const uint32_t d = q / SEG, j = q % SEG;
-        if (j < kc[d] && pos[d] != ~0ull) Pack::store(out, ostride, pos[d] + j, carry[q]);
-    }
+    scatter_flush<THREADS, Pack, Geo>(L, nbins, own, &cursor[coff], own ? cap_end[coff] : 0, out,
+                                      ostride);
+    const uint32_t bad = pk.flags(acc);
     if (bad_flag && bad) atomicOr(bad_flag, bad);
 }
+#endif
 
 template <class Digit>
 __global__ void k_padcopy(const Tup* __restrict__ in, uint64_t n, Digit dig_arg,
@@ -1732,14 +1963,19 @@
 }
 
 template <class Pack>
-static int sampled_items(uint32_t nbins) {
-    constexpr int THREADS = SMJ_SC_THREADS;
-    constexpr int BIG = sizeof(Tup) == 16
+struct SampledTile {
+    static constexpr int BIG = sizeof(Tup) == 16
         ? (sizeof(typename Pack::OutT) <= 8    ? SMJ_SC_ITEMS16P
            : sizeof(typename Pack::OutT) <= 12 ? SMJ_SC_ITEMS16Q
                                                : SMJ_SC_ITEMS16)
         : (sizeof(typename Pack::OutT) <= 4 ? SMJ_SC_ITEMS8W : SMJ_SC_ITEMS8);
-    constexpr int SMALL = sizeof(Tup) == 16 ? 4 : 8;
+    static constexpr int SMALL = sizeof(Tup) == 16 ? 4 : 8;
+};
+
+template <class Pack>
+static int sampled_items(uint32_t nbins) {
+    constexpr int THREADS = SMJ_SC_THREADS;
+    constexpr int BIG = SampledTile<Pack>::BIG, SMALL = SampledTile<Pack>::SMALL;
     typedef typename Pack::OutT O;
     if (ScatterGeom<THREADS, BIG, O, Pack::kStoreBytes>::lds_bytes(nbins) <= 160 * 1024) return BIG;
     if (ScatterGeom<THREADS, SMALL, O, Pack::kStoreBytes>::lds_bytes(nbins) <= 160 * 1024)
@@ -1759,6 +1995,11 @@
     if (lds > 160 * 1024) return false;
     uint32_t nwg = 0;
     const uint64_t chunk = scatter_chunk(n, TILE, &nwg);
+    if ((chunk + TILE) * sizeof(Tup) >= (1ull << 32)) {
+        fprintf(stderr, "[ERROR] smj: sampled scatter chunk of %llu tuples exceeds 4 GiB\n",
+                (unsigned long long)chunk);
+        abort();
+    }
     constexpr bool VEC_OK = sizeof(Tup) == 8 && ITEMS % 2 == 0;
     set_lds_attr((const void*)k_scatter_res<THREADS, ITEMS, PlanDigit1, Pack, false>, 160 * 1024);
     if constexpr (VEC_OK)
@@ -1790,12 +2031,7 @@
         fprintf(stderr, "[ERROR] smj: sampled scatter needs <= %d partitions\n", THREADS);
         abort();
     }
-    constexpr int BIG = sizeof(Tup) == 16
-        ? (sizeof(typename Pack::OutT) <= 8    ? SMJ_SC_ITEMS16P
-           : sizeof(typename Pack::OutT) <= 12 ? SMJ_SC_ITEMS16Q
-                                               : SMJ_SC_ITEMS16)
-        : (sizeof(typename Pack::OutT) <= 4 ? SMJ_SC_ITEMS8W : SMJ_SC_ITEMS8);
-    constexpr int SMALL = sizeof(Tup) == 16 ? 4 : 8;
+    constexpr int BIG = SampledTile<Pack>::BIG, SMALL = SampledTile<Pack>::SMALL;
     const int items = sampled_items<Pack>(nbins);
     if (items == BIG && sampled_scatter_t<BIG>(ws, in, n, out, ostride, dig, nbins, cursor,
                                                cap_end, pk, bad_flag, st))
@@ -1805,6 +2041,43 @@
         return;
     fprintf(stderr, "[ERROR] smj: sampled scatter LDS exceeds 160 KiB (%u partitions)\n", nbins);
     abort();
+}
+
+template <class Pack>
+static int scatter_query_t(uint32_t nbins, int vec, int* regs, int* scratch) {
+    constexpr int THREADS = SMJ_SC_THREADS;
+    constexpr int BIG = SampledTile<Pack>::BIG, SMALL = SampledTile<Pack>::SMALL;
+    const int items = nbins <= (uint32_t)THREADS ? sampled_items<Pack>(nbins) : 0;
+    if (!items || !regs) return items * THREADS;
+    const void* k = nullptr;
+    if (vec) {
+        if (sizeof(Tup) != 8 || items % 2) return 0;
+        if constexpr (sizeof(Tup) == 8 && BIG % 2 == 0 && SMALL % 2 == 0)
+            k = items == BIG ? (const void*)k_scatter_res<THREADS, BIG, PlanDigit1, Pack, true>
+                             : (const void*)k_scatter_res<THREADS, SMALL, PlanDigit1, Pack, true>;
+    } else {
+        k = items == BIG ? (const void*)k_scatter_res<THREADS, BIG, PlanDigit1, Pack, false>
+                         : (const void*)k_scatter_res<THREADS, SMALL, PlanDigit1, Pack, false>;
+    }
+    if (!k) return 0;
+    hipFuncAttributes a;
+    SMJ_CHECK(hipFuncGetAttributes(&a, k));
+    *regs = a.numRegs;
+    *scratch = (int)a.localSizeBytes;
+    return items * THREADS;
+}
+
+int scatter_query(int layout, uint32_t nbins, int vec, int* regs, int* scratch) {
+    switch (layout) {
+    case 0: return scatter_query_t<PackRange>(nbins, vec, regs, scratch);
+#ifdef KEY_8B
+    case 1: return scatter_query_t<LayPacked::Pack>(nbins, vec, regs, scratch);
+    case 4: return scatter_query_t<LayP96::Pack>(nbins, vec, regs, scratch);
+#endif
+    case 2: return scatter_query_t<LayP48::Pack>(nbins, vec, regs, scratch);
+    case 3: return scatter_query_t<LayP32::Pack>(nbins, vec, regs, scratch);
+    }
+    return 0;
 }
 
 void sampled_partition(Workspace* ws, int nrel, const Tup* const* in, const uint64_t* n,
diff --git a/avx-sort-merge-joins_amd/csrc/smj_common.hpp b/avx-sort-merge-joins_amd/csrc/smj_common.hpp
--- a/avx-sort-merge-joins_amd/csrc/smj_common.hpp
+++ b/avx-sort-merge-joins_amd/csrc/smj_common.hpp
@@ -189,6 +189,19 @@
 constexpr uint32_t kBadRange = 2;
 constexpr uint32_t kBadPayload48 = 4;
 constexpr uint32_t kBadPayload32 = 8;
+
+struct PackAcc {
+    uint32_t pay_lo = 0, pay_hi = 0;
+    bool range = false;
+    __device__ __forceinline__ void add_pay(uint64_t p) {
+        pay_lo |= (uint32_t)p;
+        pay_hi |= (uint32_t)(p >> 32);
+    }
+    __device__ __forceinline__ uint64_t pay() const { return ((uint64_t)pay_hi << 32) | pay_lo; }
+};
+__device__ __forceinline__ uint32_t pack_range_flag(const PackAcc& a) {
+    return a.range ? kBadRange : 0u;
+}
 
 struct RangePlan {
     int64_t base;
@@ -313,23 +326,35 @@
         typedef uint64_t OutT;
         uint64_t bu, span;
         uint32_t s1;
-        __device__ __forceinline__ uint64_t operator()(const Tup& t, uint32_t& bad) const {
+        __device__ __forceinline__ uint64_t pack(const Tup& t, PackAcc& a) const {
             const uint64_t ku = key_u(t.key);
             const uint64_t r = ku - bu;
             const uint32_t pb = 64 - s1;
-            bad |= (ku < bu || r > span) ? kBadRange : 0u;
-            bad |= ((uint64_t)t.payload >> pb) != 0 ? kBadPayload : 0u;
+            a.range |= ku < bu || r > span;
+            a.pay_hi |= (uint32_t)((uint64_t)t.payload >> 32);
             return ((r & ((1ull << s1) - 1)) << pb) | (uint64_t)t.payload;
+        }
+        __device__ __forceinline__ uint32_t flags(const PackAcc& a) const {
+            return pack_range_flag(a) | ((a.pay() >> (64 - s1)) != 0 ? kBadPayload : 0u);
+        }
+        __device__ __forceinline__ uint64_t operator()(const Tup& t, uint32_t& bad) const {
+            PackAcc a;
+            const uint64_t w = pack(t, a);
+            bad |= flags(a);
+            return w;
         }
         static constexpr uint32_t kStoreBytes = 8;
         __device__ static __forceinline__ void store(void* out, uint64_t, uint64_t i,
                                                      uint64_t x) {
             static_cast<uint64_t*>(out)[i] = x;
         }
-        static constexpr bool kPairs = false;
-        template <class X>
-        __device__ static __forceinline__ void store2(void*, uint64_t, uint64_t, const X&,
-                                                      const X&) {}
+        static constexpr bool kPairs = true;
+        __device__ static __forceinline__ void store2(void* out, uint64_t, uint64_t i,
+                                                      uint64_t x0, uint64_t x1) {
+            typedef unsigned long long V2 __attribute__((ext_vector_type(2)));
+            const V2 v = {x0, x1};
+            *(__attribute__((address_space(1))) V2*)(static_cast<uint64_t*>(out) + i) = v;
+        }
     };
     __host__ static bool usable(const RangePlan& P) { return P.s1 >= 1 && P.s1 <= 32; }
 };
@@ -435,13 +460,22 @@
     struct Pack {
         typedef P96W OutT;
         uint64_t bu, span;
-        __device__ __forceinline__ P96W operator()(const Tup& t, uint32_t& bad) const {
+        __device__ __forceinline__ P96W pack(const Tup& t, PackAcc& a) const {
             const uint64_t ku = key_u(t.key);
             const uint64_t r = ku - bu;
-            bad |= (ku < bu || r > span) ? kBadRange : 0u;
+            a.range |= ku < bu || r > span;
             P96W w;
             w.pay = t.payload;
             w.rel = (uint32_t)r;
+            return w;
+        }
+        __device__ __forceinline__ uint32_t flags(const PackAcc& a) const {
+            return pack_range_flag(a);
+        }
+        __device__ __forceinline__ P96W operator()(const Tup& t, uint32_t& bad) const {
+            PackAcc a;
+            const P96W w = pack(t, a);
+            bad |= flags(a);
             return w;
         }
         static constexpr uint32_t kStoreBytes = SMJ_P96_SEGB;
@@ -572,7 +606,7 @@
         typedef uint64_t OutT;
         uint64_t bu, span;
         uint32_t s1;
-        __device__ __forceinline__ uint64_t operator()(const Tup& t, uint32_t& bad) const {
+        __device__ __forceinline__ uint64_t pack(const Tup& t, PackAcc& a) const {
             const uint64_t ku = key_u(tup_key(t));
             const uint64_t r = ku - bu;
             const uint32_t pb = 48 - s1;
@@ -581,10 +615,19 @@
 #else
             const uint64_t pay = (uint32_t)t;
 #endif
-            bad |= (ku < bu || r > span) ? kBadRange : 0u;
-            bad |= (pay >> (64 - s1)) != 0 ? kBadPayload : 0u;
-            bad |= (pay >> pb) != 0 ? kBadPayload48 : 0u;
+            a.range |= ku < bu || r > span;
+            a.add_pay(pay);
             return ((r & ((1ull << s1) - 1)) << pb) | (pay & ((1ull << pb) - 1));
+        }
+        __device__ __forceinline__ uint32_t flags(const PackAcc& a) const {
+            return pack_range_flag(a) | ((a.pay() >> (64 - s1)) != 0 ? kBadPayload : 0u) |
+                   ((a.pay() >> (48 - s1)) != 0 ? kBadPayload48 : 0u);
+        }
+        __device__ __forceinline__ uint64_t operator()(const Tup& t, uint32_t& bad) const {
+            PackAcc a;
+            const uint64_t w = pack(t, a);
+            bad |= flags(a);
+            return w;
         }
         static constexpr uint32_t kStoreBytes = 4;
         __device__ static __forceinline__ void store(void* out, uint64_t stride, uint64_t i,
@@ -604,6 +647,25 @@
             *(__attribute__((address_space(1))) U2*)(lo + i) = l;
             *(__attribute__((address_space(1))) H2*)((uint16_t*)(lo + stride) + i) = h;
         }
+        static constexpr bool kQuads = true;
+        __device__ static __forceinline__ void store4(void* out, uint64_t stride, uint64_t i,
+                                                      const uint64_t (&x)[4]) {
+            typedef uint32_t U4 __attribute__((ext_vector_type(4)));
+            typedef uint32_t U2 __attribute__((ext_vector_type(2)));
+            uint32_t* lo = static_cast<uint32_t*>(out);
+            const U4 l = {(uint32_t)x[0], (uint32_t)x[1], (uint32_t)x[2], (uint32_t)x[3]};
+            const uint32_t h0 = (uint32_t)(x[0] >> 32) & 0xffffu, h1 = (uint32_t)(x[1] >> 32);
+            const uint32_t h2 = (uint32_t)(x[2] >> 32) & 0xffffu, h3 = (uint32_t)(x[3] >> 32);
+            const U2 h = {h0 | (h1 << 16), h2 | (h3 << 16)};
+            *(__attribute__((address_space(1))) U4*)(lo + i) = l;
+            uint16_t* hp = (uint16_t*)(lo + stride) + i;
+            if ((stride & 1) == 0) {
+                *(__attribute__((address_space(1))) U2*)hp = h;
+            } else {
+                ((G32)(uint32_t*)hp)[0] = h.x;
+                ((G32)(uint32_t*)hp)[1] = h.y;
+            }
+        }
     };
     __host__ static bool usable(const RangePlan& P) { return P.s1 >= 1 && P.s1 <= 32; }
 };
@@ -692,7 +754,7 @@
         typedef uint32_t OutT;
         uint64_t bu, span;
         uint32_t s1;
-        __device__ __forceinline__ uint32_t operator()(const Tup& t, uint32_t& bad) const {
+        __device__ __forceinline__ uint32_t pack(const Tup& t, PackAcc& a) const {
             const uint64_t ku = key_u(tup_key(t));
             const uint64_t r = ku - bu;
 #ifdef KEY_8B
@@ -700,11 +762,20 @@
 #else
             const uint64_t pay = (uint32_t)t;
 #endif
-            bad |= (ku < bu || r > span) ? kBadRange : 0u;
-            bad |= (pay >> (64 - s1)) != 0 ? kBadPayload : 0u;
-            bad |= (pay >> (48 - s1)) != 0 ? kBadPayload48 : 0u;
-            bad |= (pay >> (32 - s1)) != 0 ? kBadPayload32 : 0u;
+            a.range |= ku < bu || r > span;
+            a.add_pay(pay);
             return ((uint32_t)r << (32 - s1)) | ((uint32_t)pay & (0xffffffffu >> s1));
+        }
+        __device__ __forceinline__ uint32_t flags(const PackAcc& a) const {
+            return pack_range_flag(a) | ((a.pay() >> (64 - s1)) != 0 ? kBadPayload : 0u) |
+                   ((a.pay() >> (48 - s1)) != 0 ? kBadPayload48 : 0u) |
+                   ((a.pay() >> (32 - s1)) != 0 ? kBadPayload32 : 0u);
+        }
+        __device__ __forceinline__ uint32_t operator()(const Tup& t, uint32_t& bad) const {
+            PackAcc a;
+            const uint32_t w = pack(t, a);
+            bad |= flags(a);
+            return w;
         }
         static constexpr uint32_t kStoreBytes = 4;
         __device__ static __forceinline__ void store(void* out, uint64_t, uint64_t i, uint32_t x) {
@@ -797,6 +868,8 @@
 struct PackNone {
     typedef Tup OutT;
     __device__ __forceinline__ Tup operator()(const Tup& t, uint32_t&) const { return t; }
+    __device__ __forceinline__ Tup pack(const Tup& t, PackAcc&) const { return t; }
+    __device__ __forceinline__ uint32_t flags(const PackAcc&) const { return 0u; }
     static constexpr uint32_t kStoreBytes = sizeof(Tup);
     __device__ static __forceinline__ void store(void* out, uint64_t, uint64_t i, const Tup& x) {
         static_cast<Tup*>(out)[i] = x;
@@ -814,6 +887,14 @@
         const uint64_t ku = key_u(tup_key(t));
         bad |= (ku < bu || ku - bu > span) ? kBadRange : 0u;
         return t;
+    }
+    __device__ __forceinline__ Tup pack(const Tup& t, PackAcc& a) const {
+        const uint64_t ku = key_u(tup_key(t));
+        a.range |= ku < bu || ku - bu > span;
+        return t;
+    }
+    __device__ __forceinline__ uint32_t flags(const PackAcc& a) const {
+        return pack_range_flag(a);
     }
     static constexpr uint32_t kStoreBytes = sizeof(Tup);
     __device__ static __forceinline__ void store(void* out, uint64_t, uint64_t i, const Tup& x) {
diff --git a/avx-sort-merge-joins_amd/csrc/smj_internal.hpp b/avx-sort-merge-joins_amd/csrc/smj_internal.hpp
--- a/avx-sort-merge-joins_amd/csrc/smj_internal.hpp
+++ b/avx-sort-merge-joins_amd/csrc/smj_internal.hpp
@@ -318,6 +318,7 @@
 };
 bool bucket_sort(Workspace* ws, const BucketSortArgs& a, hipStream_t st);
 int tilepass_occupancy(bool p32, uint32_t d2);
+int scatter_query(int layout, uint32_t nbins, int vec, int* regs, int* scratch);
 
 void plan_from_sample(Workspace* ws, const Tup* const* rels,
                       const uint64_t* ns, int nrel, uint32_t D1, uint32_t D2,
diff --git a/avx-sort-merge-joins_amd/smj/__init__.py b/avx-sort-merge-joins_amd/smj/__init__.py
--- a/avx-sort-merge-joins_amd/smj/__init__.py
+++ b/avx-sort-merge-joins_amd/smj/__init__.py
@@ -49,6 +49,7 @@
     "smj_mgpu_comm_workspace", "smj_workspace_last_layout", "smj_mgpu_join_slices",
     "smj_mgpu_last_stats", "smj_mgpu_last_sorted", "smj_mgpu_group_workspace",
     "smj_dev_partition_range_shards", "smj_tilepass_occupancy",
+    "smj_scatter_tile", "smj_scatter_resources",
     "smj_dev_join_pairs", "smj_dev_semi_join",
     "smj_dev_band_join", "smj_dev_band_join_count",
 ]
@@ -275,6 +276,8 @@
             "smj_workspace_set_layouts": (None, [_P, _U32]),
             "smj_workspace_last_layout": (C.c_int, [_P]),
             "smj_tilepass_occupancy": (C.c_int, [C.c_int, _U32]),
+            "smj_scatter_tile": (_U32, [C.c_int, _U32]),
+            "smj_scatter_resources": (C.c_int, [C.c_int, _U32, C.c_int, _P, _P]),
             "smj_trace_enable": (None, [_P, C.c_int]),
             "smj_trace_reset": (None, [_P]),
             "smj_trace_only": (None, [_P, C.c_char_p]),
@@ -546,6 +549,15 @@
     def tilepass_occupancy(self, layout: str = "p48", d2_bits: int = 10) -> int:
         return int(self.lib.smj_tilepass_occupancy(LAYOUTS_USED.index(layout), d2_bits))
 
+    def scatter_tile(self, layout: str, nbins: int) -> int:
+        return int(self.lib.smj_scatter_tile(LAYOUTS_USED.index(layout), nbins))
+
+    def scatter_resources(self, layout: str, nbins: int, vec: bool = False):
+        regs, scr = C.c_int(-1), C.c_int(-1)
+        rc = self.lib.smj_scatter_resources(LAYOUTS_USED.index(layout), nbins, int(vec),
+                                            C.byref(regs), C.byref(scr))
+        return None if rc else (regs.value, scr.value)
+
     @staticmethod
     def stream_ptr():
         return torch.cuda.current_stream().cuda_stream
diff --git a/include/smj.h b/include/smj.h
--- a/include/smj.h
+++ b/include/smj.h
@@ -312,6 +312,9 @@
 #define SMJ_LAYOUT_USED_P96    4
 int smj_workspace_last_layout(smj_workspace * ws);
 int smj_tilepass_occupancy(int layout, uint32_t d2_bits);
+uint32_t smj_scatter_tile(int layout, uint32_t nbins);
+int smj_scatter_resources(int layout, uint32_t nbins, int vec, int* num_regs,
+                          int* scratch_bytes);
 
 void smj_dev_partition(smj_workspace * ws, const tuple_t * in, uint64_t n,
                        tuple_t * out, uint32_t nbits, uint32_t shiftbits,
```

Result: slower. 86880 Mtuples/s (-1.5%).
